# ronawho/distributed-lsb

Hardware: AMD Instinct MI355X
Metric: Melem/s (16-byte elems) at 1/2/4/8 GPUs; per-pass HBM GB/s vs roofline (higher is better)
Workload: dtype u64

## Files before the change

distributed-lsb_amd/csrc/lsb_abi.cpp:

```cpp
#include "lsb_rt.h"

using namespace lsb_rt;


extern "C" {

int64_t lsb_per_rank(int64_t n_total, int num_ranks) {
  return (num_ranks > 0 && n_total >= 0) ? div_ceil(n_total, num_ranks) : 0;
}

int64_t lsb_here(int64_t n_total, int num_ranks, int rank) {
  if (num_ranks <= 0 || n_total < 0 || rank < 0 || rank >= num_ranks) return 0;
  return here_of(n_total, num_ranks, rank);
}

const char* lsb_strerror(int code) {
  switch (code) {
    case LSB_OK: return "ok";
    case LSB_ERR_INVALID: return "invalid argument";
    case LSB_ERR_HIP: return last_error().empty() ? "HIP error" : last_error().c_str();
    case LSB_ERR_RCCL: return last_error().empty() ? "RCCL error" : last_error().c_str();
    case LSB_ERR_NOMEM: return "out of memory";
    case LSB_ERR_VERIFY: return "verification failed";
    case LSB_ERR_UNSUPPORTED: return "unsupported";
// ... 122 lines not shown
    else {
      ncclResult_t nr = ncclCommInitRank(&c->comm, num_ranks, uid, rank);
      if (nr != ncclSuccess) {
        c->comm = nullptr;
        rc = fail(LSB_ERR_RCCL, "ncclCommInitRank", ncclGetErrorString(nr));
      }
    }
  }
  if (rc != LSB_OK) {
    lsb_destroy(c);
    return rc;
  }
  *out = c;
  return LSB_OK;
}

int lsb_create_rank_ops(lsb_ctx_t** out, int64_t n_total, int num_ranks, int rank, int dev_id,
                        int radix_bits, const lsb_comm_ops_t* ops) {
  if (!out) return fail(LSB_ERR_INVALID, "lsb_create_rank_ops", "null out");
  *out = nullptr;
  if (n_total < 0 || num_ranks < 1 || num_ranks > 64 || rank < 0 || rank >= num_ranks || !ops ||
      !ops->allgather || !ops->alltoallv || !ops->allreduce_min_i64 || !ops->barrier)
    return fail(LSB_ERR_INVALID, "lsb_create_rank_ops", "n, P, rank or ops");
  if (radix_bits != 8 && radix_bits != 16 && radix_bits != 64)
    return fail(LSB_ERR_UNSUPPORTED, "lsb_create_rank_ops", "radix_bits must be 8, 16 or 64");
  lsb_ctx* c = new_ctx(n_total, num_ranks, radix_bits);
  if (!c) return LSB_ERR_NOMEM;
  c->mode = Mode::kOps;
  c->ops = *ops;
  c->first_rank = rank;
  c->ranks.resize(1);
  const int rc = init_rank(c, c->ranks[0], rank, dev_id);
  if (rc != LSB_OK) {
    lsb_destroy(c);
    return rc;
  }
  *out = c;
  return LSB_OK;
}

void lsb_destroy(lsb_ctx_t* c) {
  if (!c) return;
  (void)resolve_timing(c);
#ifdef LSB_OS_PROFILE
  (void)lsb_sync(c);
  os_profile_report();
#endif
#ifdef LSB_DEBUG
  const bool legacy = getenv("LSB_TEARDOWN_LEGACY") != nullptr;
#else
  const bool legacy = false;
#endif
  for (Rank& r : c->ranks) {
    if (legacy) break;
    (void)hipSetDevice(r.dev);
    if (r.stream) (void)hipStreamSynchronize(r.stream);
    if (r.pstream) (void)hipStreamSynchronize(r.pstream);
    if (r.xstream) (void)hipStreamSynchronize(r.xstream);
  }
  for (Rank& r : c->ranks) free_rank(r, c);
  for (auto& e : c->event_pool) (void)hipEventDestroy(e.second);
  if (c->comm) (void)ncclCommDestroy(c->comm);
  delete c;
}

int lsb_set_option(lsb_ctx_t* c, int option, int64_t value) {
  LSB_TRY(check_ctx(c));
  switch (option) {
    case LSB_OPT_TIMING:
      c->timing = value != 0;
      return LSB_OK;
    case LSB_OPT_FORCE_EXCHANGE:
      c->force_exchange = value != 0;
      return LSB_OK;
    case LSB_OPT_SKIP_CONSTANT_DIGITS:
      c->skip_constant = value != 0;
      return LSB_OK;
    case LSB_OPT_ONESWEEP:
      c->onesweep = value != 0;
      return LSB_OK;
    case LSB_OPT_REGION_FIRST:
      c->region = value != 0;
      return LSB_OK;
    case LSB_OPT_EXCHANGE_PEER:
      c->peer = value != 0;
      return LSB_OK;
    case LSB_OPT_EXCHANGE_P2P:
      c->p2p = value != 0;
      return LSB_OK;
    case LSB_OPT_EXCHANGE_SELF:
      c->self_coll = value != 0;
      return LSB_OK;
    case LSB_OPT_EXCHANGE_GATHER:
      c->gather = value != 0;
      return LSB_OK;
    case LSB_OPT_FAIL_ONESWEEP:
      if (value < 0 || value > (1 << 30)) return fail(LSB_ERR_INVALID, "lsb_set_option", "fail count");
      c->fail_onesweep = (int)value;
      return LSB_OK;
    case LSB_OPT_HYBRID:
      if (value < 0 || value > 2) return fail(LSB_ERR_INVALID, "lsb_set_option", "hybrid must be 0, 1 or 2");
      c->hybrid = (int)value;
      return LSB_OK;
    case LSB_OPT_ONESWEEP_SPLIT:
      if (value < 0 || value > 2) return fail(LSB_ERR_INVALID, "lsb_set_option", "split must be 0..2");
      c->os_split = (int)value;
      return LSB_OK;
    case LSB_OPT_EXCHANGE_CHUNKS:
      if (value != 0 && value != 2 && value != 4 && value != 8)
        return fail(LSB_ERR_INVALID, "lsb_set_option", "exchange chunks must be 0, 2, 4 or 8");
      c->xchunks = (int)value;
      return LSB_OK;
    case LSB_OPT_EXCHANGE_SLICES:
      if (value < 1 || value > 64)
        return fail(LSB_ERR_INVALID, "lsb_set_option", "exchange slices must be 1..64");
      c->slices = (int)value;
      return LSB_OK;
    default:
      return fail(LSB_ERR_INVALID, "lsb_set_option", "unknown option");
  }
}

int lsb_local_ranks(const lsb_ctx_t* c, int* first_rank, int* num_local) {
  LSB_TRY(check_ctx(c));
  if (first_rank) *first_rank = c->first_rank;
  if (num_local) *num_local = (int)c->ranks.size();
  return LSB_OK;
}

int lsb_generate_ex(lsb_ctx_t* c, int dist, double param) {
  LSB_TRY(check_ctx(c));
  lsb::KeyGen g;
  if (dist == LSB_DIST_UNIFORM) {
    g.dist = lsb::kDistUniform;
  } else if (dist == LSB_DIST_ZIPF) {
    if (!(param > 0.0) || param > 16.0) return fail(LSB_ERR_INVALID, "lsb_generate_ex", "zipf s");
    g.dist = lsb::kDistZipf;
    g.zipf_s = param;
    g.zipf_n = 1ull << 30;
  } else {
    return fail(LSB_ERR_INVALID, "lsb_generate_ex", "dist");
  }
  c->keygen = g;
  for (Rank& r : c->ranks) {
    HIP_TRY(hipSetDevice(r.dev));
    HIP_TRY(lsb::launch_pcg_fill(r.A, c->per, (uint64_t)r.rank, (uint64_t)r.rank * c->per, g,
                                 r.stream));
  }
  return lsb_sync(c);
}

int lsb_generate(lsb_ctx_t* c) { return lsb_generate_ex(c, LSB_DIST_UNIFORM, 0.0); }

int lsb_copy_in(lsb_ctx_t* c, int rank, int64_t off, int64_t cnt, const lsb_elem_t* host) {
  LSB_TRY(check_ctx(c));
  Rank* r = local_rank(c, rank);
  if (!r || off < 0 || cnt < 0 || off + cnt > c->per || (cnt > 0 && !host))
    return fail(LSB_ERR_INVALID, "lsb_copy_in", "rank or range");
  if (cnt == 0) return LSB_OK;
  HIP_TRY(hipSetDevice(r->dev));
  HIP_TRY(hipStreamSynchronize(r->stream));
  HIP_TRY(hipMemcpy(r->A + off, host, (size_t)cnt * sizeof(Elem), hipMemcpyHostToDevice));
  return LSB_OK;
}

int lsb_copy_out(lsb_ctx_t* c, int rank, int64_t off, int64_t cnt, lsb_elem_t* host) {
  LSB_TRY(check_ctx(c));
  Rank* r = local_rank(c, rank);
  if (!r || off < 0 || cnt < 0 || off + cnt > c->per || (cnt > 0 && !host))
    return fail(LSB_ERR_INVALID, "lsb_copy_out", "rank or range");
  if (cnt == 0) return LSB_OK;
  HIP_TRY(hipSetDevice(r->dev));
  HIP_TRY(hipStreamSynchronize(r->stream));
  HIP_TRY(hipMemcpy(host, r->A + off, (size_t)cnt * sizeof(Elem), hipMemcpyDeviceToHost));
  return LSB_OK;
}

namespace {

void quiesce(lsb_ctx* c) {
  for (Rank& r : c->ranks) {
    (void)hipSetDevice(r.dev);
    for (hipStream_t s : {r.stream, r.pstream, r.xstream})
      if (s) (void)hipStreamSynchronize(s);
  }
}

}

int lsb_pass(lsb_ctx_t* c, int digit) {
  LSB_TRY(check_ctx(c));
  if (digit < 0 || digit >= 64 / c->bits) return fail(LSB_ERR_INVALID, "lsb_pass", "digit");
  c->pass_cursor = c->bits == 64 ? 0 : digit * (c->bits / lsb::kDigitBits);
  const int rc = do_pass(c, digit);
  if (rc != LSB_OK) quiesce(c);
  return rc;
}

namespace {

int sort_body(lsb_ctx* c) {
  std::vector<Timer> sort_timers;
  sort_timers.reserve(c->ranks.size());
  for (Rank& r : c->ranks) sort_timers.emplace_back(c, &r, LSB_K_SORT);
  const int passes = 64 / c->bits;
  c->last_local_passes = c->last_exchanges = 0;
  c->last_varying = ~0ull;
  c->last_first = LSB_FIRST_COUNT;
  c->pass_cursor = 0;
  c->cur_pass = 0;
  if (c->bits == 64 && exchanging(c)) {
    LSB_TRY(merge_sort(c));
  } else if (onesweep_applies(c)) {
    LSB_TRY(sort_onesweep(c));
  } else if (exchange_onesweep_applies(c)) {
    LSB_TRY(sort_exchange_onesweep(c));
  } else if (!c->skip_constant) {
    for (int d = 0; d < passes; ++d) LSB_TRY(do_pass(c, d));
  } else {
    for (Rank& r : c->ranks) {
      HIP_TRY(hipSetDevice(r.dev));
      HIP_TRY(hipMemsetAsync(r.span, 0, 2 * sizeof(uint64_t), r.stream));
    }
    LSB_TRY(do_pass(c, 0, ~0ull, true));
    uint64_t kor = 0, knor = 0;
    LSB_TRY(gather_span(c, &kor, &knor));
    c->last_varying = kor & knor;
    const uint64_t digit_mask = (1ull << c->bits) - 1;
    for (int d = 1; d < passes; ++d) {
      if (((c->last_varying >> (d * c->bits)) & digit_mask) == 0) continue;
      LSB_TRY(do_pass(c, d, c->last_varying));
    }
  }
  for (Timer& t : sort_timers) t.stop();
  return LSB_OK;
}

}

int lsb_sort(lsb_ctx_t* c) {
  LSB_TRY(check_ctx(c));
  const int rc = sort_body(c);
  if (rc != LSB_OK) quiesce(c);
  return rc;
}

int lsb_get_last_sort(lsb_ctx_t* c, int* local_passes, int* exchanges, uint64_t* varying_bits) {
  LSB_TRY(check_ctx(c));
  if (local_passes) *local_passes = c->last_local_passes;
  if (exchanges) *exchanges = c->last_exchanges;
  if (varying_bits) *varying_bits = c->last_varying;
  return LSB_OK;
}

int lsb_get_first_pass(lsb_ctx_t* c, int* form) {
  LSB_TRY(check_ctx(c));
  if (!form) return fail(LSB_ERR_INVALID, "lsb_get_first_pass", "null");
  *form = c->last_first;
  return LSB_OK;
}

int lsb_sync(lsb_ctx_t* c) {
  LSB_TRY(check_ctx(c));
  for (Rank& r : c->ranks) {
    HIP_TRY(hipSetDevice(r.dev));
    HIP_TRY(hipStreamSynchronize(r.stream));
    LSB_TRY(onesweep_check(r));
  }
  return LSB_OK;
}

int lsb_barrier(lsb_ctx_t* c) {
  LSB_TRY(lsb_sync(c));
  if (c->mode == Mode::kLoopback) return LSB_OK;
  if (c->mode == Mode::kOps)
    return c->ops.barrier(c->ops.user) == 0 ? LSB_OK : ops_fail("barrier");
  Rank& r = c->ranks[0];
  HIP_TRY(hipSetDevice(r.dev));
  RCCL_TRY(ncclAllReduce(r.check, r.check, 1, ncclUint64, ncclSum, c->comm, r.stream));
  HIP_TRY(hipStreamSynchronize(r.stream));
  return LSB_OK;
}

int lsb_verify(lsb_ctx_t* c, int64_t* first_bad) {
  LSB_TRY(check_ctx(c));
  int64_t bad = INT64_MAX;
  for (Rank& r : c->ranks) {
    HIP_TRY(hipSetDevice(r.dev));
    HIP_TRY(hipMemsetAsync(r.check, 0xff, sizeof(unsigned long long), r.stream));
    HIP_TRY(lsb::launch_verify(r.A, r.here, (int64_t)r.rank * c->per, c->n, c->per, c->keygen,
                               r.check, r.stream));
    unsigned long long h = ~0ull;
    HIP_TRY(hipMemcpyAsync(&h, r.check, sizeof h, hipMemcpyDeviceToHost, r.stream));
    HIP_TRY(hipStreamSynchronize(r.stream));
    if (h != ~0ull && (int64_t)h < bad) bad = (int64_t)h;
  }
  std::vector<uint64_t> bnd;
  LSB_TRY(gather_boundaries(c, bnd));
  int prev = -1;
  for (int s = 0; s < c->P; ++s) {
    if (here_of(c->n, c->P, s) == 0) continue;
    if (prev >= 0) {
      const uint64_t lk = bnd[(size_t)prev * 4 + 2], lv = bnd[(size_t)prev * 4 + 3];
      const uint64_t fk = bnd[(size_t)s * 4 + 0], fv = bnd[(size_t)s * 4 + 1];
      if (!(lk < fk || (lk == fk && lv < fv))) {
        const int64_t idx = (int64_t)prev * c->per + here_of(c->n, c->P, prev) - 1;
        if (idx < bad) bad = idx;
      }
    }
    prev = s;
  }
  LSB_TRY(allreduce_min_i64(c, &bad));
  if (first_bad) *first_bad = bad == INT64_MAX ? -1 : bad;
  return bad == INT64_MAX ? LSB_OK : LSB_ERR_VERIFY;
}

int lsb_check_sorted(lsb_ctx_t* c, int* sorted) {
  LSB_TRY(check_ctx(c));
  int local_ok = 1;
  for (Rank& r : c->ranks) {
    HIP_TRY(hipSetDevice(r.dev));
    HIP_TRY(hipMemsetAsync(r.check, 0, sizeof(unsigned int), r.stream));
    HIP_TRY(lsb::launch_check_sorted(r.A, r.here, reinterpret_cast<unsigned int*>(r.check),
                                     r.stream));
    unsigned int h = 0;
    HIP_TRY(hipMemcpyAsync(&h, r.check, sizeof h, hipMemcpyDeviceToHost, r.stream));
    HIP_TRY(hipStreamSynchronize(r.stream));
    if (h) local_ok = 0;
  }
  std::vector<uint64_t> bnd;
  LSB_TRY(gather_boundaries(c, bnd));
  int prev = -1;
  int bounds_ok = 1;
  for (int s = 0; s < c->P; ++s) {
    if (here_of(c->n, c->P, s) == 0) continue;
    if (prev >= 0 && bnd[(size_t)s * 4 + 0] < bnd[(size_t)prev * 4 + 2]) bounds_ok = 0;
    prev = s;
  }
  int64_t ok = (local_ok && bounds_ok) ? 1 : 0;
  LSB_TRY(allreduce_min_i64(c, &ok));
  if (sorted) *sorted = (int)ok;
// ... 249 lines not shown
```

distributed-lsb_amd/csrc/lsb_context.cpp:

```cpp
#include "lsb_rt.h"

namespace lsb_rt {

thread_local std::string g_last_error;

const std::string& last_error() { return g_last_error; }

int fail(int code, const char* what, const char* detail) {
  char buf[512];
  snprintf(buf, sizeof buf, "%s: %s", what, detail ? detail : "");
  g_last_error = buf;
  if (getenv("LSB_DEBUG")) fprintf(stderr, "[lsb] %s\n", buf);
  return code;
}
hipEvent_t take_event(lsb_ctx* c) {
  int dev = 0;
  (void)hipGetDevice(&dev);
  for (size_t i = c->event_pool.size(); i-- > 0;)
    if (c->event_pool[i].first == dev) {
      hipEvent_t e = c->event_pool[i].second;
      c->event_pool.erase(c->event_pool.begin() + (long)i);
      return e;
    }
  hipEvent_t e = nullptr;
// ... 219 lines not shown
  if (k > 1) {
    std::vector<size_t> sc1(P), sd1(P), rc1(P), rd1(P);
    auto cut = [&](size_t n, size_t i) { return (size_t)((unsigned __int128)n * i / k); };
    for (size_t i = 0; i < k; ++i) {
      for (int q = 0; q < P; ++q) {
        sd1[q] = sd[q] + cut(sc[q], i);
        sc1[q] = cut(sc[q], i + 1) - cut(sc[q], i);
        rd1[q] = rd[q] + cut(rc[q], i);
        rc1[q] = cut(rc[q], i + 1) - cut(rc[q], i);
      }
      LSB_TRY(coll_alltoallv_u64(c, r, send, sc1.data(), sd1.data(), recv, rc1.data(), rd1.data(), 0, st));
    }
    return LSB_OK;
  }
  int64_t call_bytes = 0;
  for (int q = 0; q < P; ++q) call_bytes += (int64_t)sc[q] * 8;
  c->coll_calls += 1;
  c->coll_bytes += call_bytes;
  c->coll_max = std::max(c->coll_max, call_bytes);
  c->xs_calls += 1;
  for (int q = 0; q < P && q < LSB_MAX_RANKS; ++q) {
    c->xs_sent[q] += (int64_t)sc[q] * 8;
    c->xs_recv[q] += (int64_t)rc[q] * 8;
  }
  if (c->cur_pass >= 0 && c->cur_pass < LSB_MAX_PASSES) c->pass_xbytes[c->cur_pass] += call_bytes;
  if (c->mode == Mode::kRccl) {
    static const bool dsync = [] { const char* e = getenv("LSB_RCCL_SYNC"); return e && atoi(e); }();
    if (dsync) HIP_TRY(hipDeviceSynchronize());
    if (!c->p2p) {
      RCCL_TRY(ncclAllToAllv(send, sc, sd, recv, rc, rd, ncclUint64, c->comm, st));
    } else {
      RCCL_TRY(ncclGroupStart());
      for (int q = 0; q < P; ++q) {
        if (sc[q] > 0) RCCL_TRY(ncclSend(send + sd[q], sc[q], ncclUint64, q, c->comm, st));
        if (rc[q] > 0) RCCL_TRY(ncclRecv(recv + rd[q], rc[q], ncclUint64, q, c->comm, st));
      }
      RCCL_TRY(ncclGroupEnd());
    }
    if (dsync) HIP_TRY(hipDeviceSynchronize());
    return LSB_OK;
  }
  size_t send_end = 0, recv_end = 0;
  for (int q = 0; q < P; ++q) {
    if (sc[q]) send_end = std::max(send_end, sd[q] + sc[q]);
    if (rc[q]) recv_end = std::max(recv_end, rd[q] + rc[q]);
  }
  std::vector<uint64_t> hs(std::max<size_t>(send_end, 1)), hr(std::max<size_t>(recv_end, 1));
  std::vector<size_t> sb(P), sdb(P), rb(P), rdb(P);
  for (int q = 0; q < P; ++q) {
    if (sc[q])
      HIP_TRY(hipMemcpyAsync(hs.data() + sd[q], send + sd[q], sc[q] * 8, hipMemcpyDeviceToHost,
                             r.stream));
    sb[q] = sc[q] * 8;
    sdb[q] = sd[q] * 8;
    rb[q] = rc[q] * 8;
    rdb[q] = rd[q] * 8;
  }
  HIP_TRY(hipStreamSynchronize(r.stream));
  if (c->ops.alltoallv(c->ops.user, hs.data(), sb.data(), sdb.data(), hr.data(), rb.data(),
                       rdb.data()) != 0)
    return ops_fail("alltoallv");
  for (int q = 0; q < P; ++q)
    if (rc[q])
      HIP_TRY(hipMemcpyAsync(recv + rd[q], hr.data() + rd[q], rc[q] * 8, hipMemcpyHostToDevice,
                             r.stream));
  HIP_TRY(hipStreamSynchronize(r.stream));
  return LSB_OK;
}

int check_ctx(const lsb_ctx* c) {
  if (!c) return fail(LSB_ERR_INVALID, "lsb", "null context");
  return LSB_OK;
}

lsb_ctx* new_ctx(int64_t n_total, int num_ranks, int radix_bits) {
  lsb_ctx* c = new (std::nothrow) lsb_ctx();
  if (!c) return nullptr;
  c->n = n_total;
  c->P = num_ranks;
  c->per = div_ceil(n_total, num_ranks);
  c->bits = radix_bits;
  c->nb = radix_bits == 64 ? lsb::kBuckets : 1 << radix_bits;
  if (const char* e = getenv("LSB_REGION_FIRST")) c->region = atoi(e) != 0;
  if (const char* e = getenv("LSB_EXCHANGE_CHUNKS")) {
    const int v = atoi(e);
    c->xchunks = v == 2 || v == 4 || v == 8 ? v : 0;
  }
  if (const char* e = getenv("LSB_XCHUNK_RESERVE")) c->xchunk_reserve = std::max(0, atoi(e));
  return c;
}

int gather_boundaries(lsb_ctx* c, std::vector<uint64_t>& bnd) {
  const int P = c->P;
  bnd.assign((size_t)P * 4, 0);
  if (c->mode == Mode::kLoopback) {
    for (Rank& r : c->ranks) {
      if (r.here == 0) continue;
      HIP_TRY(hipSetDevice(r.dev));
      HIP_TRY(hipStreamSynchronize(r.stream));
      HIP_TRY(hipMemcpy(&bnd[(size_t)r.rank * 4], r.A, 16, hipMemcpyDeviceToHost));
      HIP_TRY(hipMemcpy(&bnd[(size_t)r.rank * 4 + 2], r.A + (r.here - 1), 16, hipMemcpyDeviceToHost));
    }
    return LSB_OK;
  }
  Rank& r = c->ranks[0];
  HIP_TRY(hipSetDevice(r.dev));
  uint64_t* d = r.gather;
  HIP_TRY(hipMemsetAsync(d, 0, sizeof(uint64_t) * 4 * P, r.stream));
  if (r.here > 0) {
    HIP_TRY(hipMemcpyAsync(d + (size_t)r.rank * 4, r.A, 16, hipMemcpyDeviceToDevice, r.stream));
    HIP_TRY(hipMemcpyAsync(d + (size_t)r.rank * 4 + 2, r.A + (r.here - 1), 16,
                           hipMemcpyDeviceToDevice, r.stream));
  }
  LSB_TRY(coll_allgather_u64(c, r, d + (size_t)r.rank * 4, d, 4));
  HIP_TRY(hipMemcpyAsync(bnd.data(), d, sizeof(uint64_t) * 4 * P, hipMemcpyDeviceToHost, r.stream));
  HIP_TRY(hipStreamSynchronize(r.stream));
  return LSB_OK;
}

int allreduce_min_i64(lsb_ctx* c, int64_t* v) {
  if (c->mode == Mode::kLoopback) return LSB_OK;
  if (c->mode == Mode::kOps)
    return c->ops.allreduce_min_i64(c->ops.user, v) == 0 ? LSB_OK : ops_fail("allreduce_min_i64");
  Rank& r = c->ranks[0];
  HIP_TRY(hipSetDevice(r.dev));
  int64_t* d = reinterpret_cast<int64_t*>(r.check);
  HIP_TRY(hipMemcpyAsync(d, v, sizeof(int64_t), hipMemcpyHostToDevice, r.stream));
  RCCL_TRY(ncclAllReduce(d, d, 1, ncclInt64, ncclMin, c->comm, r.stream));
  HIP_TRY(hipMemcpyAsync(v, d, sizeof(int64_t), hipMemcpyDeviceToHost, r.stream));
  HIP_TRY(hipStreamSynchronize(r.stream));
  return LSB_OK;
}

int gather_span(lsb_ctx* c, uint64_t* kor, uint64_t* knor) {
  *kor = *knor = 0;
  if (c->mode != Mode::kLoopback) {
    Rank& r = c->ranks[0];
    HIP_TRY(hipSetDevice(r.dev));
    LSB_TRY(coll_allgather_u64(c, r, r.span, r.span_gather, 2));
    HIP_TRY(hipMemcpyAsync(r.span_h, r.span_gather, sizeof(uint64_t) * 2 * c->P,
                           hipMemcpyDeviceToHost, r.stream));
    HIP_TRY(hipStreamSynchronize(r.stream));
    for (int q = 0; q < c->P; ++q) {
      *kor |= r.span_h[2 * q];
      *knor |= r.span_h[2 * q + 1];
    }
    return LSB_OK;
  }
  for (Rank& r : c->ranks) {
    HIP_TRY(hipSetDevice(r.dev));
    HIP_TRY(hipMemcpyAsync(r.span_h, r.span, sizeof(uint64_t) * 2, hipMemcpyDeviceToHost, r.stream));
  }
  for (Rank& r : c->ranks) {
    HIP_TRY(hipSetDevice(r.dev));
    HIP_TRY(hipStreamSynchronize(r.stream));
    *kor |= r.span_h[0];
    *knor |= r.span_h[1];
  }
  return LSB_OK;
}

}
```

distributed-lsb_amd/csrc/lsb_kernels.h:

```cpp
#pragma once

#include <hip/hip_runtime.h>
#include <stdint.h>

namespace lsb {

struct alignas(16) Elem {
  uint64_t key;
  uint64_t val;
};
static_assert(sizeof(Elem) == 16, "16-byte records");

constexpr int kDigitBits = 8;
constexpr int kBuckets = 1 << kDigitBits;
#ifndef LSB_SCATTER_BLOCK
#define LSB_SCATTER_BLOCK 256
#define LSB_SCATTER_IPT 16
#endif
constexpr int kScatterBlock = LSB_SCATTER_BLOCK;
constexpr int kScatterIpt = LSB_SCATTER_IPT;
constexpr int kTile = kScatterBlock * kScatterIpt;
#ifndef LSB_OS_BLOCK
#define LSB_OS_BLOCK 512
#endif
constexpr int kOsBlock = LSB_OS_BLOCK;
constexpr int kOsIpt = kTile / kOsBlock;
#ifndef LSB_OS_SPLIT_BLOCK
#define LSB_OS_SPLIT_BLOCK 256
#endif
constexpr int kOsSplitBlock = LSB_OS_SPLIT_BLOCK;
constexpr int kOsSplitIpt = kTile / kOsSplitBlock;
static_assert(kOsBlock % kBuckets == 0 && kOsBlock * kOsIpt == kTile, "onesweep tile shape");
constexpr int kMaxChunks = 65536;

struct Chunking {
  int64_t chunk_elems = 0;
  int num_chunks = 0;
};
Chunking make_chunking(int64_t m, int max_chunks);

constexpr int kDistUniform = 0;
constexpr int kDistZipf = 1;
struct KeyGen {
  int dist = kDistUniform;
  double zipf_s = 1.1;
  uint64_t zipf_n = 1ull << 30;
};

hipError_t launch_pcg_fill(Elem* A, int64_t count, uint64_t seed, uint64_t val0, KeyGen gen,
                           hipStream_t s);

hipError_t launch_digit16_counts(const Elem* A, int64_t m, int shift, int64_t* first,
                                 uint64_t* counts, hipStream_t s);

hipError_t launch_upsweep(const Elem* A, int64_t m, int shift, Chunking ch,
                          uint32_t* chunk_hist, uint64_t* span, hipStream_t s);

hipError_t launch_scan(const uint32_t* chunk_hist, int G, uint64_t* chunk_off,
                       uint64_t* totals, hipStream_t s);

hipError_t launch_scatter(const Elem* in, Elem* out, int64_t m, int shift, Chunking ch,
                          const uint64_t* chunk_off, const uint64_t* totals, int64_t* first16,
                          hipStream_t s);
hipError_t launch_starts_reset(int64_t* first16, hipStream_t s);
hipError_t launch_starts_to_counts(const int64_t* first16, int64_t m, uint64_t* counts,
                                   hipStream_t s);

constexpr int kOnesweepSubs = 8;
constexpr int64_t kOnesweepMaxElems = (int64_t(1) << 33) - (int64_t(1) << 16);
inline int64_t onesweep_tiles(int64_t m) { return (m + kTile - 1) / kTile; }
hipError_t launch_subhist(const Elem* A, int64_t m, int shift, int grid, uint32_t* sub_hist,
                          uint64_t* span, hipStream_t s);
hipError_t onesweep_profile(unsigned long long* out10, bool reset);
constexpr int kSegCap = 256;
struct SegPass {
  uint64_t pmask = 0;
  uint64_t rmask = 0;
  int64_t* base = nullptr;
  uint32_t* err = nullptr;
};
constexpr int kDescPieces = 4;
constexpr int kDescOverflow = 0xFF;
struct alignas(16) TileDesc {
  int32_t n, e0, e1, sel;
  int32_t start[kDescPieces];
  int64_t adj[kDescPieces];
};
constexpr int kMaxExchangeChunks = 8;
struct GatherSrc {
  const Elem* R = nullptr;
  const Elem* A = nullptr;
  int64_t self_adj[kMaxExchangeChunks] = {};
  int chunk_shift = 8;
  const int64_t* place = nullptr;
  const int64_t* gstart = nullptr;
  const int64_t* gadj = nullptr;
  const TileDesc* desc = nullptr;
  int P = 1, nb = 256, me = 0, self_in_a = 1;
  int64_t a_len = 0, r_len = 0;
};
hipError_t launch_gather_desc(const GatherSrc& g, int64_t m, TileDesc* desc, hipStream_t s);
hipError_t launch_count16_chunks(const Elem* B, int64_t m, int shift16, const uint32_t* lo_hist, int cshift,
                                 int grid, uint64_t* count16, uint32_t* chunk_hist, hipStream_t s);
constexpr int64_t kRegionMin = int64_t(1) << 27;
constexpr int kRegions = kBuckets * kOnesweepSubs;
inline int64_t region_mean(int64_t m) { return (m + kRegions - 1) / kRegions; }
#ifndef LSB_REGION_SIGMA
#define LSB_REGION_SIGMA 6
#endif
#ifndef LSB_REGION_DIV
#define LSB_REGION_DIV 64
#endif
inline int64_t region_cap(int64_t m, int64_t min_m = kRegionMin) {
  if (m < min_m || m <= 0) return 0;
  const int64_t mu = region_mean(m);
  int64_t sd = 1;
  while (sd * sd < mu) ++sd;
  const int64_t a = mu / LSB_REGION_DIV, b = LSB_REGION_SIGMA * sd;
  const int64_t slack = a > b ? a : b;
  return (mu + slack + kTile - 1) / kTile * kTile;
}
#ifndef LSB_REGION_STAGGER
#define LSB_REGION_STAGGER 0
#endif
__host__ __device__ inline int64_t region_stride(int64_t cap) { return cap + (LSB_REGION_STAGGER ? kTile : 0); }
__host__ __device__ inline int64_t region_base(int64_t r, int64_t cap) {
  return r * region_stride(cap) + (LSB_REGION_STAGGER ? ((r * 37) & 15) * 256 : 0);
}
inline int64_t region_slots(int64_t m, int64_t min_m = kRegionMin) {
  return region_stride(region_cap(m, min_m)) * kRegions;
}
struct RegionPass {
  int64_t cap = 0;
  uint32_t* counts = nullptr;
  uint32_t* ovf = nullptr;
};
hipError_t launch_sample(const Elem* A, int64_t m, int shift, uint32_t* hist, uint64_t* span,
                         hipStream_t s);
struct OnesweepExtra {
  uint64_t* totals = nullptr;
  uint64_t* count16 = nullptr;
  int halves = 1;
  const SegPass* seg = nullptr;
  const GatherSrc* gather = nullptr;
  bool probe = false;
  const RegionPass* region = nullptr;
  int region_mode = 0;
};
int onesweep_halves_for(const uint32_t* sub_hist_host, int64_t m);
hipError_t launch_onesweep(const Elem* in, Elem* out, int64_t m, int shift, int next_shift,
                           const uint32_t* sub_hist, uint32_t* next_hist, uint32_t* status,
                           uint32_t* tile_ctr, uint32_t epoch, uint32_t* err, int grid,
                           hipStream_t s, OnesweepExtra extra = OnesweepExtra());

constexpr int kSegMax = 64;
hipError_t launch_segsort(const Elem* in, Elem* out, int64_t m, uint64_t pmask, uint32_t* err,
                          int grid, hipStream_t s);
hipError_t launch_segfix(const Elem* in, Elem* out, int64_t m, int shift, const uint32_t* status,
                         const SegPass& seg, int grid, hipStream_t s);

hipError_t launch_place(const Elem* src, Elem* out, int64_t out_len, int64_t k0, int64_t count,
                        int shift, int nbuckets, const int64_t* off_row, hipStream_t s,
                        int next_shift = -1, uint32_t* next_hist = nullptr, bool store = true,
                        bool skew = false);

hipError_t launch_peer_exchange(const Elem* src, int64_t m, int shift, int nbuckets,
                                const uint64_t* hist, int P, int me, int64_t per,
                                Elem* const* dst, int64_t* base, hipStream_t s);
hipError_t launch_system_acquire(hipStream_t s);

hipError_t launch_plan(const uint64_t* hist, int P, int nb, int me, int64_t n, int64_t* work,
                       int64_t* total, int64_t* place, int64_t* counts, hipStream_t s,
                       int64_t* gstart = nullptr, int cshift = 8, int64_t* chunk_counts = nullptr);

constexpr int kSplitCands = 256;
constexpr int kSplitRounds = 8;
constexpr int kMergeMaxCuts = 512;
hipError_t launch_split_init(uint64_t* state, int Q, hipStream_t s);
hipError_t launch_split_cands(const Elem* A, int64_t m, const uint64_t* state, int Q, uint64_t* cnt,
                              hipStream_t s);
hipError_t launch_split_update(const uint64_t* gathered, int P, int Q, const int64_t* targets,
                               uint64_t* state, hipStream_t s);
hipError_t launch_split_final(const Elem* A, int64_t m, const uint64_t* state, int Q, uint64_t* out,
                              hipStream_t s);
constexpr int kMergeTile = 2048;
constexpr int kMergeMaxPairs = 32;
struct MergePair {
  const Elem* a;
  const Elem* b;
  Elem* out;
  int64_t na, nb, tile0;
};
struct MergeLevel {
  MergePair p[kMergeMaxPairs];
  int npairs;
  int64_t tiles;
};
inline int64_t merge_tiles(int64_t n) { return (n + kMergeTile - 1) / kMergeTile; }
hipError_t launch_merge_level(const MergeLevel& level, int64_t* path, int grid, hipStream_t s);

hipError_t launch_copy_records(Elem* dst, const Elem* src, int64_t cnt, hipStream_t s);
hipError_t launch_verify(const Elem* A, int64_t here, int64_t gbase, int64_t n, int64_t per,
                         KeyGen gen, unsigned long long* first_bad, hipStream_t s);

hipError_t launch_check_sorted(const Elem* A, int64_t here, unsigned int* unsorted, hipStream_t s);

}
```

distributed-lsb_amd/csrc/lsb_kernels.hip:

```cpp
#include "lsb_device.h"
#include <type_traits>

#ifdef LSB_DEBUG
#include <cassert>
#define LSB_DASSERT(c) assert(c)
#else
#define LSB_DASSERT(c) ((void)0)
#endif

namespace lsb {
namespace {

typedef unsigned __int128 u128;

constexpr u128 kPcgMult = ((u128)0x2360ED051FC65DA4ULL << 64) | (u128)0x4385DF649FCCF645ULL;
constexpr u128 kPcgInc = ((u128)0x5851F42D4C957F2DULL << 64) | (u128)0x14057B7EF767814FULL;

struct JumpTable {
  uint64_t mul_lo[64], mul_hi[64], add_lo[64], add_hi[64];
};

constexpr JumpTable make_jump_table() {
  JumpTable t{};
  u128 m = kPcgMult, a = kPcgInc;
  for (int k = 0; k < 64; ++k) {
    t.mul_lo[k] = (uint64_t)m;
    t.mul_hi[k] = (uint64_t)(m >> 64);
    t.add_lo[k] = (uint64_t)a;
    t.add_hi[k] = (uint64_t)(a >> 64);
    a = a * (m + 1);
    m = m * m;
  }
  return t;
}

__constant__ JumpTable kJump = make_jump_table();

__device__ __forceinline__ uint64_t pcg_output(u128 s) {
  const uint64_t x = (uint64_t)(s >> 64) ^ (uint64_t)s;
  const unsigned rot = (unsigned)(s >> 122);
  return (x >> rot) | (x << ((64u - rot) & 63u));
}

__device__ __forceinline__ u128 pcg_seed(uint64_t seed) {
  return ((u128)seed + kPcgInc) * kPcgMult + kPcgInc;
}

__device__ __forceinline__ u128 pcg_jump(u128 s, uint64_t delta) {
  while (delta) {
    const int k = __builtin_ctzll(delta);
    const u128 m = ((u128)kJump.mul_hi[k] << 64) | kJump.mul_lo[k];
    const u128 a = ((u128)kJump.add_hi[k] << 64) | kJump.add_lo[k];
    s = s * m + a;
    delta &= delta - 1;
  }
  return s;
}

__device__ __forceinline__ uint32_t lane_id() { return __lane_id(); }

__device__ __forceinline__ uint32_t mbcnt(uint64_t mask) {
  return __builtin_amdgcn_mbcnt_hi((uint32_t)(mask >> 32),
                                   __builtin_amdgcn_mbcnt_lo((uint32_t)mask, 0u));
}

__device__ __forceinline__ uint64_t match_digit8(uint32_t d, uint64_t active) {
  uint32_t lo = (uint32_t)active, hi = (uint32_t)(active >> 32);
#pragma unroll
  for (int bit = 0; bit < 8; ++bit) {
    const uint32_t t = (uint32_t)__builtin_amdgcn_sbfe((int)d, bit, 1);
    const uint64_t bal = __builtin_amdgcn_uicmp(t, 0u, 33);
    lo = __builtin_amdgcn_bitop3_b32(lo, (uint32_t)bal, t, 0x90);
    hi = __builtin_amdgcn_bitop3_b32(hi, (uint32_t)(bal >> 32), t, 0x90);
  }
  return ((uint64_t)hi << 32) | lo;
}

__device__ __forceinline__ Elem load_elem(const Elem* p) {
  const ulonglong2 v = *reinterpret_cast<const ulonglong2*>(p);
  return Elem{v.x, v.y};
}

__device__ __forceinline__ Elem load_elem_nt(const Elem* p) {
  typedef unsigned long long u64x2 __attribute__((ext_vector_type(2)));
  const u64x2 v = __builtin_nontemporal_load(reinterpret_cast<const u64x2*>(p));
  return Elem{v.x, v.y};
}

__device__ __forceinline__ void store_elem(Elem* p, const Elem& e) {
  *reinterpret_cast<ulonglong2*>(p) = make_ulonglong2(e.key, e.val);
}

template <typename T>
__device__ __forceinline__ T wave_inclusive_scan(T v) {
  const uint32_t lane = lane_id();
#pragma unroll
  for (int off = 1; off < 64; off <<= 1) {
    const T u = __shfl_up(v, off, 64);
    if (lane >= (uint32_t)off) v += u;
  }
  return v;
}

template <>
__device__ __forceinline__ uint32_t wave_inclusive_scan<uint32_t>(uint32_t v) {
  const uint32_t lane = lane_id(), rl = lane & 15u;
  uint32_t t;
  t = (uint32_t)__builtin_amdgcn_mov_dpp((int)v, 0x111, 0xf, 0xf, false);
  if (rl >= 1) v += t;
  t = (uint32_t)__builtin_amdgcn_mov_dpp((int)v, 0x112, 0xf, 0xf, false);
  if (rl >= 2) v += t;
  t = (uint32_t)__builtin_amdgcn_mov_dpp((int)v, 0x114, 0xf, 0xf, false);
  if (rl >= 4) v += t;
  t = (uint32_t)__builtin_amdgcn_mov_dpp((int)v, 0x118, 0xf, 0xf, false);
  if (rl >= 8) v += t;
  t = (uint32_t)__builtin_amdgcn_mov_dpp((int)v, 0x142, 0xf, 0xf, false);
  if ((lane & 31u) >= 16) v += t;
  t = (uint32_t)__builtin_amdgcn_mov_dpp((int)v, 0x143, 0xf, 0xf, false);
  if (lane >= 32) v += t;
  return v;
}

__device__ __forceinline__ uint32_t pair_swap(uint32_t v) {
  return (uint32_t)__builtin_amdgcn_mov_dpp((int)v, 0xB1, 0xf, 0xf, false);
}

template <int BLOCK, typename T>
__device__ __forceinline__ T block_exclusive_scan(T v, T* tmp, T* total) {
  constexpr int W = BLOCK / 64;
  const int w = threadIdx.x >> 6;
  const T inc = wave_inclusive_scan(v);
  if (lane_id() == 63) tmp[w] = inc;
  __syncthreads();
  T pre = 0, tot = 0;
#pragma unroll
  for (int i = 0; i < W; ++i) {
    const T x = tmp[i];
    pre += (i < w) ? x : T(0);
    tot += x;
  }
  __syncthreads();
  *total = tot;
  return pre + inc - v;
}

constexpr int kFillPerThread = 16;

__device__ __forceinline__ uint64_t mix64(uint64_t z) {
  z = (z ^ (z >> 30)) * 0xBF58476D1CE4E5B9ull;
  z = (z ^ (z >> 27)) * 0x94D049BB133111EBull;
  return z ^ (z >> 31);
}

__device__ __forceinline__ uint64_t make_key(uint64_t draw, const KeyGen& g) {
  if (g.dist == kDistUniform) return draw;
  const double u = (double)(draw >> 11) * 0x1.0p-53;
  const double n1 = (double)g.zipf_n + 1.0;
  double x;
  if (g.zipf_s == 1.0) {
    x = exp(u * log(n1));
  } else {
    const double e = 1.0 - g.zipf_s;
    x = pow(1.0 - u * (1.0 - pow(n1, e)), 1.0 / e);
  }
  uint64_t k = (uint64_t)x;
  if (k < 1) k = 1;
  if (k > g.zipf_n) k = g.zipf_n;
  return mix64(k);
}

__global__ __launch_bounds__(256) void k_pcg_fill(Elem* __restrict__ A, int64_t count,
                                                  uint64_t seed, uint64_t val0, KeyGen g) {
  const int64_t first = ((int64_t)blockIdx.x * 256 + threadIdx.x) * kFillPerThread;
// ... 419 lines not shown
  __syncthreads();
  if (t <= C) {
    int64_t a = 0;
    for (int l = 0; l < (t << cshift) && l < kBuckets; ++l) a += tot[l];
    cstart[t] = a;
  }
  __syncthreads();
  const uint64_t* __restrict__ keys = reinterpret_cast<const uint64_t*>(B);
  const int64_t TT = (m + T - 1) / T;
  const int64_t t0 = (int64_t)blockIdx.x * tiles_per_wg;
  const int64_t t1 = t0 + tiles_per_wg < TT ? t0 + tiles_per_wg : TT;
  auto target = [&](int64_t p, uint32_t l) -> uint32_t {
    const uint32_t k = l >> cshift;
    const int64_t len = cstart[k + 1] - cstart[k];
    const int64_t TTk = (len + T - 1) / T;
    return k * kSub + (uint32_t)sub_of_tile((p - cstart[k]) / T, TTk);
  };
  uint32_t cur_l = 0xFFFFFFFFu, cur_s = 0xFFFFFFFFu;
  uint32_t acc_l = 0, acc_s = 0;
  auto flush_l = [&]() {
    if (cur_l != 0xFFFFFFFFu && acc_l) atomicAdd(&count16[((uint32_t)t << 8) | cur_l], (unsigned long long)acc_l);
    acc_l = 0;
  };
  auto flush_s = [&]() {
    if (cur_s != 0xFFFFFFFFu && acc_s) atomicAdd(&chunk_hist[cur_s * kBuckets + t], acc_s);
    acc_s = 0;
  };
  for (int64_t tile = t0; tile < t1; ++tile) {
    const int64_t tb = tile * T;
    const int64_t end = tb + T < m ? tb + T : m;
    const uint32_t lf = (uint32_t)(keys[2 * tb] >> shift16) & 0xFFu;
    const uint32_t ll = (uint32_t)(keys[2 * (end - 1)] >> shift16) & 0xFFu;
    const uint32_t sf = target(tb, lf), sl = target(end - 1, ll);
    const bool uniform = lf == ll && sf == sl;
    uint64_t k[IPT];
#pragma unroll
    for (int i = 0; i < IPT; ++i) {
      const int64_t idx = tb + (int64_t)i * BLOCK + t;
      k[i] = idx < end ? __builtin_nontemporal_load(keys + 2 * idx) : 0ull;
    }
    if (uniform) {
#pragma unroll
      for (int i = 0; i < IPT; ++i) {
        const int64_t idx = tb + (int64_t)i * BLOCK + t;
        if (idx < end) atomicAdd(&th[w][(uint32_t)(k[i] >> (shift16 + 8)) & 0xFFu], 1u);
      }
      __syncthreads();
      uint32_t v = 0;
#pragma unroll
      for (int ww = 0; ww < W; ++ww) {
        v += th[ww][t];
        th[ww][t] = 0;
      }
      if (lf != cur_l) {
        flush_l();
        cur_l = lf;
      }
      if (sf != cur_s) {
        flush_s();
        cur_s = sf;
      }
      acc_l += v;
      acc_s += v;
      __syncthreads();
    } else {
#pragma unroll
      for (int i = 0; i < IPT; ++i) {
        const int64_t idx = tb + (int64_t)i * BLOCK + t;
        if (idx >= end) continue;
        const uint32_t l = (uint32_t)(k[i] >> shift16) & 0xFFu, h = (uint32_t)(k[i] >> (shift16 + 8)) & 0xFFu;
        atomicAdd(&count16[(h << 8) | l], 1ull);
        atomicAdd(&chunk_hist[target(idx, l) * kBuckets + h], 1u);
      }
    }
  }
  flush_l();
  flush_s();
}

constexpr int kSampleBlock = 256;
constexpr int kSampleTiles = 256;
__global__ __launch_bounds__(kSampleBlock) void k_sample(const Elem* __restrict__ A, int64_t m, int shift,
                                                         uint32_t* __restrict__ hist,
                                                         unsigned long long* __restrict__ span) {
  constexpr int IPT = kTile / kSampleBlock;
  __shared__ uint32_t h[kBuckets];
  h[threadIdx.x] = 0;
  __syncthreads();
  const int64_t TT = (m + kTile - 1) / kTile;
  const int64_t tb = (int64_t)blockIdx.x * TT / gridDim.x * kTile;
  const uint64_t* __restrict__ keys = reinterpret_cast<const uint64_t*>(A);
  uint64_t kor = 0, knor = 0;
#pragma unroll
  for (int i = 0; i < IPT; ++i) {
    const int64_t idx = tb + (int64_t)i * kSampleBlock + threadIdx.x;
    if (idx < m) {
      const uint64_t k = __builtin_nontemporal_load(keys + 2 * idx);
      kor |= k;
      knor |= ~k;
      atomicAdd(&h[(uint32_t)(k >> shift) & (kBuckets - 1)], 1u);
    }
  }
#pragma unroll
  for (int off = 32; off > 0; off >>= 1) {
    kor |= __shfl_xor(kor, off, 64);
    knor |= __shfl_xor(knor, off, 64);
  }
  if (lane_id() == 0) {
    atomicOr(&span[0], (unsigned long long)kor);
    atomicOr(&span[1], (unsigned long long)knor);
  }
  __syncthreads();
  if (h[threadIdx.x]) atomicAdd(&hist[threadIdx.x], h[threadIdx.x]);
}

#ifdef LSB_OS_PROFILE
__device__ unsigned long long g_os_prof[10];
#define OS_MARK(k)                                                       \
  do {                                                                   \
    if (t == 0) {                                                        \
      const uint64_t now = __builtin_amdgcn_s_memtime();                 \
      prof[k] += now - prof_last;                                        \
      prof_last = now;                                                   \
    }                                                                    \
  } while (0)
#else
#define OS_MARK(k) ((void)0)
#endif

#ifndef LSB_SEG_WIN
#define LSB_SEG_WIN 2
#endif
constexpr int kSegWin = LSB_SEG_WIN;
#ifndef LSB_SEG_LDSNB
#define LSB_SEG_LDSNB 0
#endif
#ifndef LSB_SEG_BATCH
#define LSB_SEG_BATCH 4
#endif
#ifndef LSB_GATHER_PF
#define LSB_GATHER_PF 64
#endif

template <int BLOCK, int IPT, bool NEXT, bool C16, int HALVES, bool SEG, bool GATHER, int RG>
__device__ __forceinline__ void onesweep_body(
    const Elem* __restrict__ in, Elem* __restrict__ out, int64_t m, int shift, int next_shift,
    const uint32_t* __restrict__ sub_hist, uint32_t* __restrict__ next_hist,
    uint32_t* __restrict__ status, uint32_t* __restrict__ tile_ctr, uint32_t epoch,
    uint32_t* __restrict__ err, uint64_t* __restrict__ totals,
    unsigned long long* __restrict__ count16, SegPass seg, GatherSrc gs, RegionPass rg) {
  constexpr int W = BLOCK / 64;
  constexpr int T = BLOCK * IPT;
  static_assert(!SEG || (!NEXT && !C16 && HALVES == 1), "the segment pass: last pass, whole stage");
  static_assert(RG == 0 || (!C16 && HALVES == 1 && !SEG && !GATHER), "regional passes: plain whole stage");
  static_assert(RG != 1 || NEXT, "the regional first pass counts the next digit");
  static_assert(BLOCK % kBuckets == 0, "bucket threads");
  using WC = typename std::conditional<(W > 4), uint16_t, uint32_t>::type;

  constexpr int HT = T / HALVES;
  __shared__ Elem stage[HT];
  __shared__ WC wcnt[W][kBuckets];
  __shared__ int64_t delta[kBuckets];
  __shared__ uint32_t cut[NEXT ? kBuckets : 1];
  __shared__ uint32_t nh[NEXT ? kSub * kBuckets : 1];
  __shared__ uint64_t scan64[W];
  __shared__ uint32_t scan32[W];
  __shared__ int32_t s_tile, s_sub;
  __shared__ uint32_t tile_lo[2];
  __shared__ TileDesc s_desc;

  const int t = threadIdx.x;
  const bool bkt = BLOCK == kBuckets || t < kBuckets;
  const int w = t >> 6;
  const uint32_t lane = lane_id();
  const int64_t TT = RG == 2 ? rg.cap / T * kRegions : (m + T - 1) / T;
  const int64_t TTn = RG == 1 ? rg.cap / T * kRegions : (m + T - 1) / T;
  const int64_t mcap = RG == 1 ? region_stride(rg.cap) * kRegions : m;
  uint32_t racc = 0;
  constexpr uint32_t kValMask = kStatusValMask, kPreBit = 1u << 30;
  const uint32_t tag_agg = (epoch & 1u) << 31, tag_pre = tag_agg | kPreBit;
  const int shift16 = shift - 8;
  uint32_t acc_lo = 0xFFFFFFFFu;
  uint64_t acc = 0;
  auto c16_flush = [&]() {
    if (acc) atomicAdd(count16 + (((uint32_t)t << 8) | acc_lo), (unsigned long long)acc);
    acc = 0;
  };

  uint32_t col[HALVES == 1 ? kSub : 1];
  uint64_t tot = 0;
#pragma unroll
  for (int x = 0; x < kSub; ++x) {
    const uint32_t v = bkt && RG != 1 ? sub_hist[x * kBuckets + t] : 0u;
    if (HALVES == 1) col[x] = v;
    tot += v;
  }
  uint64_t all;
  const uint64_t bstart = block_exclusive_scan<BLOCK>(tot, scan64, &all);
  if (totals != nullptr && blockIdx.x == 0 && bkt) totals[t] = tot;
  if (SEG && blockIdx.x == 0 && bkt) {
    uint64_t pre = bstart;
#pragma unroll
    for (int x = 0; x < kSub; ++x) {
      seg.base[x * kBuckets + t] = (int64_t)pre;
      pre += col[x];
    }
  }
  const bool skewed = NEXT && __syncthreads_or(tot > (uint64_t)(m >> 5)) != 0;
  if (NEXT)
    for (int i = t; i < kSub * kBuckets; i += BLOCK) nh[i] = 0;

#ifdef LSB_OS_PROFILE
  uint64_t prof[10] = {};
  uint64_t prof_last = __builtin_amdgcn_s_memtime();
#endif
  int sub = (int)(blockIdx.x % kSub);
  int tries = 0;
  int cur_sub = -1;
  uint64_t base = 0;
  auto grab = [&](int& tile_out, int& sub_out) {
    int tile = -1;
    while (tries < kSub) {
      const int64_t f0 = sub_first_tile(sub, TT), f1 = sub_first_tile(sub + 1, TT);
      if (f1 > f0) {
        const uint32_t jj = atomicAdd(&tile_ctr[sub], 1u);
        if ((int64_t)jj < f1 - f0) {
          tile = (int)(f0 + jj);
          break;
        }
      }
      sub = sub + 1 == kSub ? 0 : sub + 1;
      ++tries;
    }
    tile_out = tile;
    sub_out = sub;
  };
  int nxt_tile = -1, nxt_sub = 0;
  if (t == 0) grab(nxt_tile, nxt_sub);
  uint4 dreg = make_uint4(0u, 0u, 0u, 0u);
  auto fetch_desc = [&]() {
    if (GATHER && w == 0) {
      const int nt = __builtin_amdgcn_readfirstlane(nxt_tile);
      if (nt >= 0 && lane < 4) dreg = reinterpret_cast<const uint4*>(gs.desc + nt)[lane];
    }
  };
  fetch_desc();

  for (;;) {
    if (t == 0) {
      s_tile = nxt_tile;
      s_sub = nxt_sub;
    }
    if (GATHER && w == 0 && lane < 4) {
      uint32_t l;
      asm volatile("v_mbcnt_lo_u32_b32 %0, -1, 0" : "=v"(l));
      *reinterpret_cast<uint4*>(reinterpret_cast<char*>(&s_desc) + l * 16u) = dreg;
    }
#pragma unroll
    for (int j = 0; j < kBuckets / 64; ++j) wcnt[w][lane + 64 * j] = 0;
    __syncthreads();
    OS_MARK(0);
    const int tile = s_tile;
    if (tile < 0) break;
    const int x = s_sub;
    if (x != cur_sub) {
      if (RG == 1) {
        if (bkt && cur_sub >= 0 && racc) atomicAdd(&rg.counts[t * kSub + cur_sub], racc);
        racc = 0;
        base = (uint64_t)region_base((bkt ? t : 0) * kSub + x, rg.cap);
      } else {
        uint64_t pre = 0;
#pragma unroll
        for (int xx = 0; xx < kSub; ++xx)
          pre += xx < x ? (HALVES == 1 ? col[xx] : (bkt ? sub_hist[xx * kBuckets + t] : 0u)) : 0u;
        base = bstart + pre;
      }
      cur_sub = x;
    }
    int64_t tb = (int64_t)tile * T;
    int nvalid = (int)((m - tb) < T ? (m - tb) : T);
    uint32_t rg_reg = 0, rg_k = 0;
    if (RG == 2) {
      const uint32_t tu = (uint32_t)__builtin_amdgcn_readfirstlane(tile);
      const uint32_t ct = (uint32_t)(rg.cap / T);
      rg_reg = tu / ct;
      rg_k = tu - rg_reg * ct;
      tb = region_base(rg_reg, rg.cap) + (int64_t)rg_k * T;
    }

    Elem e[IPT];
    const int wbase = w * 64 * IPT + (int)lane;
    if (GATHER) {
      const int dn = __builtin_amdgcn_readfirstlane(s_desc.n);
      if (dn != kDescOverflow) {
        const uint32_t sel = (uint32_t)__builtin_amdgcn_readfirstlane(s_desc.sel);
        const Elem* pb[kDescPieces];
        int st[kDescPieces];
#pragma unroll
        for (int k = 0; k < kDescPieces; ++k) {
          st[k] = __builtin_amdgcn_readfirstlane(s_desc.start[k]);
          const uint64_t a = s_desc.adj[k];
          const int64_t adj = (int64_t)(((uint64_t)(uint32_t)__builtin_amdgcn_readfirstlane((int)(a >> 32)) << 32) |
                                        (uint32_t)__builtin_amdgcn_readfirstlane((int)(uint32_t)a));
          pb[k] = ((sel >> k) & 1u ? gs.A : gs.R) + (tb + adj);
        }
        const int wu = __builtin_amdgcn_readfirstlane(w);
#pragma unroll
        for (int i = 0; i < IPT; ++i) {
          const int li = wbase + i * 64;
          const int g0 = wu * 64 * IPT + i * 64;
          int ka = 0, kb = 0;
#pragma unroll
          for (int k = 1; k < kDescPieces; ++k) {
            ka += g0 >= st[k] ? 1 : 0;
            kb += g0 + 63 >= st[k] ? 1 : 0;
          }
          const Elem* src = pb[0];
          if (ka == kb) {
#pragma unroll
            for (int k = 1; k < kDescPieces; ++k) src = ka >= k ? pb[k] : src;
          } else {
#pragma unroll
            for (int k = 1; k < kDescPieces; ++k) src = li >= st[k] ? pb[k] : src;
          }
          LSB_DASSERT(li >= nvalid || gather_in(gs, src + li));
          e[i] = li < nvalid ? load_elem_nt(src + li) : Elem{0ull, 0ull};
        }
      } else {
        const int e0 = s_desc.e0, e1 = s_desc.e1;
#pragma unroll
        for (int i = 0; i < IPT; ++i) {
          const int li = wbase + i * 64;
          LSB_DASSERT(li >= nvalid || gather_in(gs, gather_search(gs, e0, e1, tb + li)));
          e[i] = li < nvalid ? load_elem_nt(gather_search(gs, e0, e1, tb + li)) : Elem{0ull, 0ull};
          __builtin_amdgcn_sched_barrier(0);
        }
      }
#if LSB_GATHER_PF
      if (w == 1 && lane == 0) {
        const int pf = tile + LSB_GATHER_PF;
        if (pf < sub_first_tile(x + 1, TT))
          (void)__hip_atomic_load(const_cast<int32_t*>(&gs.desc[pf].n), __ATOMIC_RELAXED, __HIP_MEMORY_SCOPE_AGENT);
      }
#endif
    } else {
#pragma unroll
      for (int i = 0; i < IPT; ++i) {
        const int li = wbase + i * 64;
        e[i] = RG == 2 || li < nvalid ? load_elem_nt(in + tb + li) : Elem{0ull, 0ull};
      }
      if (RG == 2) {
        __builtin_amdgcn_sched_barrier(0);
        const int64_t v = (int64_t)rg.counts[rg_reg] - (int64_t)rg_k * T;
        nvalid = (int)(v < 0 ? 0 : (v < T ? v : T));
      }
    }
#ifdef LSB_OS_PROFILE
    asm volatile("s_waitcnt vmcnt(0)" ::: "memory");
    OS_MARK(6);
#endif
    const int64_t first = sub_first_tile(x, TT);
    const int64_t last = sub_first_tile(x + 1, TT);
    const bool head = tile == first;
    const bool even = (lane & 1u) == 0;
    const __amdgpu_buffer_rsrc_t rs = __builtin_amdgcn_make_buffer_rsrc(
        status + first * kBuckets, 0, (int)((last - first) * kBuckets * 4), 0x00020000);
    constexpr uint32_t kRowBytes = kBuckets * 4;
    const uint32_t my_off = (uint32_t)(tile - first) * kRowBytes + (uint32_t)t * 4u;
    uint32_t prow = (uint32_t)(tile - first) - 1u;
    v2u g[kLookW];
    auto load_window = [&]() {
#pragma unroll
      for (int r = 0; r < kLookW; ++r)
        g[r] = __builtin_amdgcn_raw_buffer_load_b64(rs, (prow - (uint32_t)r) * kRowBytes + (uint32_t)t * 4u, 0, 16);
    };
    uint32_t cnt = 0, lstart;
    uint32_t rk[IPT];
#pragma unroll
    for (int i = 0; i < IPT; ++i) {
      const bool valid = wbase + i * 64 < nvalid;
      const uint32_t d = (uint32_t)(e[i].key >> shift) & (kBuckets - 1);
      const uint64_t mt = match_digit8(d, __ballot(valid));
      const uint32_t below = mbcnt(mt);
      const uint32_t pre = wcnt[w][d];
      rk[i] = pre + below;
      if (valid && below == 0) wcnt[w][d] = (WC)(pre + (uint32_t)__popcll(mt));
      if (C16) {
        const int li = wbase + i * 64;
        if (li == 0) tile_lo[0] = (uint32_t)(e[i].key >> shift16) & 0xFFu;
        if (li == nvalid - 1) tile_lo[1] = (uint32_t)(e[i].key >> shift16) & 0xFFu;
      }
    }
    __syncthreads();
    OS_MARK(1);
    if (bkt) {
#pragma unroll
      for (int ww = 0; ww < W; ++ww) {
        const uint32_t v = wcnt[ww][t];
        wcnt[ww][t] = (WC)cnt;
        cnt += v;
      }
      if (RG == 1) racc += cnt;
    }
    bool mixed16 = false;
    if (C16) {
      const uint32_t l0 = tile_lo[0];
      mixed16 = l0 != tile_lo[1];
      if (!mixed16 && cnt > 0) {
        if (l0 != acc_lo) {
          c16_flush();
          acc_lo = l0;
        }
        acc += cnt;
      }
    }
    const uint32_t cnt_b = pair_swap(cnt);
    if (even && bkt) {
      const uint32_t tg = head ? tag_pre : tag_agg;
      __builtin_amdgcn_raw_buffer_store_b64(v2u{cnt | tg, cnt_b | tg}, rs, my_off, 0, kStPol);
      if (!head) load_window();
    }
    {
      uint32_t tile_total;
      lstart = block_exclusive_scan<BLOCK>(cnt, scan32, &tile_total);
      if (bkt) {
#pragma unroll
        for (int ww = 0; ww < W; ++ww) wcnt[ww][t] = (WC)(wcnt[ww][t] + lstart);
      }
    }
    __syncthreads();
    OS_MARK(2);
    auto stage_half = [&](int h) {
#pragma unroll
      for (int i = 0; i < IPT; ++i) {
        if (wbase + i * 64 < nvalid) {
          const uint32_t d = (uint32_t)(e[i].key >> shift) & (kBuckets - 1);
          if (HALVES == 1) {
            stage[wcnt[w][d] + rk[i]] = e[i];
          } else {
            if (h == 0) rk[i] += wcnt[w][d];
            if ((int)(rk[i] / HT) == h) stage[rk[i] - h * HT] = e[i];
          }
        }
      }
    };
    stage_half(0);

    OS_MARK(3);
    uint32_t ea = 0, eb = 0;
    if (even && bkt && !head) {
      uint32_t spins = 0;
      for (;;) {
        uint32_t used = 0;
        bool done = false;
#pragma unroll
        for (int r = 0; r < kLookW; ++r) {
          if (done || used != (uint32_t)r) continue;
          if (((g[r].x ^ g[r].y) >> 30) == 0 && (g[r].x & ~kValMask & ~kPreBit) == tag_agg) {
            ea += g[r].x & kValMask;
            eb += g[r].y & kValMask;
            ++used;
            done = (g[r].x & kPreBit) != 0;
          }
        }
#ifdef LSB_OS_PROFILE
        if (t == 0) prof[7] += used;
#endif
        if (done) break;
        if (used == 0) {
          __builtin_amdgcn_s_sleep(kPollSleep);
          if ((++spins & 1023u) == 0 &&
              (spins > kSpinLimit ||
               __hip_atomic_load((gu32*)err, __ATOMIC_RELAXED, __HIP_MEMORY_SCOPE_AGENT) != 0)) {
            atomicOr(err, 1u);
            break;
          }
        }
        prow -= used;
        load_window();
      }
      __builtin_amdgcn_raw_buffer_store_b64(v2u{(ea + cnt) | tag_pre, (eb + cnt_b) | tag_pre}, rs,
                                            my_off, 0, kStPol);
    }
    const uint32_t eb_left = pair_swap(eb);
    const uint64_t excl = even ? ea : eb_left;
    int64_t R = (int64_t)(base + excl);
    if (RG == 1 && bkt && excl + cnt > (uint64_t)rg.cap) {
      atomicOr(rg.ovf, 1u);
      R = R < mcap - (int64_t)cnt ? R : mcap - (int64_t)cnt;
    }
    if (bkt) delta[t] = R - (int64_t)lstart;
    if (NEXT && bkt) {
      uint32_t c = 0xFFFFu;
      if (RG == 1) {
        c = 0xFFFFu | ((uint32_t)(t >> 5) << 16) | ((uint32_t)(t >> 5) << 24);
      } else if (cnt > 0) {
        const int x0 = sub_of_tile(R / T, TTn);
        const int64_t bnd = x0 + 1 < kSub ? sub_first_tile(x0 + 1, TTn) * T : mcap;
        if (R + cnt > bnd) {
          const int x1 = sub_of_tile(bnd / T, TTn);
          c = (uint32_t)(lstart + (bnd - R)) | ((uint32_t)x0 << 16) | ((uint32_t)x1 << 24);
        } else {
          c = 0xFFFFu | ((uint32_t)x0 << 16) | ((uint32_t)x0 << 24);
        }
      }
      cut[t] = c;
    }
    __syncthreads();
    OS_MARK(5);
#ifdef LSB_OS_PROFILE
    if (t == 0) ++prof[8];
#endif
    if (t == 0) {
      grab(nxt_tile, nxt_sub);
    }

    auto emit = [&](auto skew_tag, const Elem& v, int j, int64_t g, uint32_t c) {
      constexpr bool kSkew = decltype(skew_tag)::value;
      LSB_DASSERT(g >= 0 && g < mcap);
      const uint64_t gs = (uint64_t)g < (uint64_t)(mcap - 1) ? (uint64_t)g : (uint64_t)(mcap - 1);
      store_elem(out + gs, v);
      if (NEXT) {
        const uint32_t xs = (uint32_t)j >= (c & 0xFFFFu) ? (c >> 24) : ((c >> 16) & 0xFFu);
        const uint32_t dn = (uint32_t)(v.key >> next_shift) & (kBuckets - 1);
        const uint32_t slot = xs * kBuckets + dn;
        if (kSkew) {
          const uint64_t act = __ballot(1);
          const uint32_t prev =
              (uint32_t)__builtin_amdgcn_update_dpp((int)~slot, (int)slot, 0x138, 0xf, 0xf, false);
          const bool head = prev != slot;
          const uint64_t heads = __ballot(head);
          if (head) {
            const uint64_t above = heads & ~((2ull << lane) - 1ull);
            const uint32_t end = above ? (uint32_t)__builtin_ctzll(above) : (uint32_t)__popcll(act);
            atomicAdd(&nh[slot], end - lane);
          }
        } else {
          atomicAdd(&nh[slot], 1u);
        }
      }
    };
    auto seg_pos = [&](const Elem& v, int j, int jend) -> int {
      int pos = j;
#if LSB_SEG_LDSNB
      const uint64_t pv = j > 0 ? stage[j - 1].key : ~v.key;
      const uint64_t nx = j + 1 < nvalid ? stage[j + 1].key : ~v.key;
#else
      const uint32_t kl = (uint32_t)v.key, kh = (uint32_t)(v.key >> 32);
      uint64_t pv = ((uint64_t)(uint32_t)__builtin_amdgcn_update_dpp(0, (int)kh, 0x138, 0xf, 0xf, false) << 32) |
                    (uint32_t)__builtin_amdgcn_update_dpp(0, (int)kl, 0x138, 0xf, 0xf, false);
      uint64_t nx = ((uint64_t)(uint32_t)__builtin_amdgcn_update_dpp(0, (int)kh, 0x130, 0xf, 0xf, false) << 32) |
                    (uint32_t)__builtin_amdgcn_update_dpp(0, (int)kl, 0x130, 0xf, 0xf, false);
      if (lane == 0 && j > 0) pv = stage[j - 1].key;
      if ((lane == 63 || j + 1 == jend) && j + 1 < nvalid) nx = stage[j + 1].key;
#endif
      const uint64_t pk = v.key & seg.pmask;
      const bool sp = j > 0 && (pv & seg.pmask) == pk;
      const bool sn = j + 1 < nvalid && (nx & seg.pmask) == pk;
      if (sp || sn) {
        uint32_t less = 0, eqb = 0;
        const int klo = j - kSegMax > 0 ? j - kSegMax : 0;
        const int khi = j + 1 + kSegMax < nvalid ? j + 1 + kSegMax : nvalid;
        uint64_t wb[kSegWin > 0 ? kSegWin : 1], wf[kSegWin > 0 ? kSegWin : 1];
#pragma unroll
        for (int q = 0; q < kSegWin; ++q) {
          wb[q] = q == 0 && j - 1 >= klo ? pv : j - 1 - q >= klo ? stage[j - 1 - q].key : ~v.key;
          wf[q] = q == 0 && j + 1 < khi ? nx : j + 1 + q < khi ? stage[j + 1 + q].key : ~v.key;
        }
        int k = j - 1;
        bool on = true;
#pragma unroll
        for (int q = 0; q < kSegWin; ++q) {
          on = on && (wb[q] & seg.pmask) == pk;
          if (on) {
            less += wb[q] < v.key ? 1u : 0u;
            eqb += wb[q] == v.key ? 1u : 0u;
            --k;
          }
        }
        while (on && k >= klo) {
          const uint64_t kk = stage[k].key;
          if ((kk & seg.pmask) != pk) break;
          less += kk < v.key ? 1u : 0u;
          eqb += kk == v.key ? 1u : 0u;
          --k;
        }
        const int sfirst = k + 1;
        bool too_long = k < klo && klo > 0;
        k = j + 1;
        on = true;
#pragma unroll
        for (int q = 0; q < kSegWin; ++q) {
          on = on && (wf[q] & seg.pmask) == pk;
          if (on) {
            less += wf[q] < v.key ? 1u : 0u;
            ++k;
          }
        }
        while (on && k < khi) {
          const uint64_t kk = stage[k].key;
          if ((kk & seg.pmask) != pk) break;
          less += kk < v.key ? 1u : 0u;
          ++k;
        }
        too_long |= k == khi && khi < nvalid;
        if (too_long) atomicOr(seg.err, 2u);
        pos = sfirst + (int)(less + eqb);
      }
      return pos;
    };
    auto write_out = [&](auto skew_tag, int h) {
      const int jend = HALVES == 1 || (h + 1) * HT >= nvalid ? nvalid : (h + 1) * HT;
      if ((!SEG || LSB_SEG_BATCH) && HALVES == 1 && !C16 && !GATHER && jend == HT) {
        constexpr int G = SEG && LSB_SEG_BATCH > 0 && LSB_SEG_BATCH < HT / BLOCK ? LSB_SEG_BATCH : HT / BLOCK;
#pragma unroll
        for (int k0 = 0; k0 < HT / BLOCK; k0 += G) {
          Elem v[G];
          int64_t dl[G];
          uint32_t ct[G];
#pragma unroll
          for (int k = 0; k < G; ++k) v[k] = stage[(k0 + k) * BLOCK + t];
#pragma unroll
          for (int k = 0; k < G; ++k) {
            const uint32_t d = (uint32_t)(v[k].key >> shift) & (kBuckets - 1);
            dl[k] = delta[d];
            ct[k] = NEXT ? cut[d] : 0u;
          }
#pragma unroll
          for (int k = 0; k < G; ++k) {
            const int j = (k0 + k) * BLOCK + t;
            emit(skew_tag, v[k], j, dl[k] + (SEG ? seg_pos(v[k], j, jend) : j), ct[k]);
          }
        }
        return;
      }
      for (int j = h * HT + t; j < jend; j += BLOCK) {
        const Elem v = stage[j - h * HT];
        int pos = j;
        if (SEG) pos = seg_pos(v, j, jend);
        const uint32_t d = (uint32_t)(v.key >> shift) & (kBuckets - 1);
        emit(skew_tag, v, j, delta[d] + pos, NEXT ? cut[d] : 0u);
        if (C16 && mixed16) {
          const uint32_t s16 = (d << 8) | ((uint32_t)(v.key >> shift16) & 0xFFu);
          const uint64_t act = __ballot(1);
          const uint32_t prev = (uint32_t)__builtin_amdgcn_update_dpp((int)~s16, (int)s16, 0x138, 0xf, 0xf, false);
          const bool head = prev != s16;
          const uint64_t heads = __ballot(head);
          if (head) {
            const uint64_t above = heads & ~((2ull << lane) - 1ull);
            const uint32_t end = above ? (uint32_t)__builtin_ctzll(above) : (uint32_t)__popcll(act);
            atomicAdd(count16 + s16, (unsigned long long)(end - lane));
          }
        }
      }
    };
    for (int h = 0; h < HALVES; ++h) {
      if (h > 0) {
        stage_half(h);
        __syncthreads();
      }
      if (skewed) write_out(std::true_type{}, h);
      else write_out(std::false_type{}, h);
      if (h == HALVES - 1) fetch_desc();
      __syncthreads();
    }
    OS_MARK(4);
  }
  if (C16) c16_flush();
#ifdef LSB_OS_PROFILE
  if (t == 0)
    for (int k = 0; k < 10; ++k) atomicAdd(&g_os_prof[k], (unsigned long long)prof[k]);
#endif
  if (NEXT) {
    for (int i = t; i < kSub * kBuckets; i += BLOCK)
      if (nh[i]) atomicAdd(&next_hist[i], nh[i]);
  }
  if (RG == 1 && bkt && cur_sub >= 0 && racc) atomicAdd(&rg.counts[t * kSub + cur_sub], racc);
}

template <int BLOCK, int IPT, bool NEXT, bool C16, int HALVES, bool SEG = false, bool GATHER = false, int RG = 0>
__global__ __launch_bounds__(BLOCK, (HALVES == 1 ? 2 : 3) * BLOCK / 256) void k_onesweep(
    const Elem* __restrict__ in, Elem* __restrict__ out, int64_t m, int shift, int next_shift,
    const uint32_t* __restrict__ sub_hist, uint32_t* __restrict__ next_hist,
    uint32_t* __restrict__ status, uint32_t* __restrict__ tile_ctr, uint32_t epoch,
    uint32_t* __restrict__ err, uint64_t* __restrict__ totals,
    unsigned long long* __restrict__ count16, SegPass seg, GatherSrc gs, RegionPass rg) {
  onesweep_body<BLOCK, IPT, NEXT, C16, HALVES, SEG, GATHER, RG>(in, out, m, shift, next_shift, sub_hist,
                                                                next_hist, status, tile_ctr, epoch, err, totals,
                                                                count16, seg, gs, rg);
}

__global__ __launch_bounds__(kOsBlock, 2 * kOsBlock / 256) void k_onesweep_probe(
    const Elem* __restrict__ in, Elem* __restrict__ out, int64_t m, int shift, int next_shift,
    const uint32_t* __restrict__ sub_hist, uint32_t* __restrict__ next_hist,
    uint32_t* __restrict__ status, uint32_t* __restrict__ tile_ctr, uint32_t epoch,
    uint32_t* __restrict__ err, uint64_t* __restrict__ totals,
    unsigned long long* __restrict__ count16, SegPass seg, GatherSrc gs) {
  onesweep_body<kOsBlock, kOsIpt, true, false, 1, false, false, 0>(in, out, m, shift, next_shift, sub_hist,
                                                                   next_hist, status, tile_ctr, epoch, err,
                                                                   totals, count16, seg, gs, RegionPass());
}

constexpr int kPlaceBlock = 256;
constexpr int kPlaceIpt = 8;
constexpr int kPlaceLdsBuckets = 4096;
constexpr int kPlaceNextGrid = 1024;

template <bool kLds, bool kNext, bool kStore = true>
__global__ __launch_bounds__(kPlaceBlock) void k_place(const Elem* __restrict__ src,
                                                       Elem* __restrict__ out, int64_t k0,
                                                       int64_t count, int shift, uint32_t mask,
                                                       const int64_t* __restrict__ off_row,
                                                       int64_t out_len, int next_shift,
                                                       uint32_t* __restrict__ next_hist, uint32_t skew) {
  __shared__ int64_t lds_off[kLds ? kPlaceLdsBuckets : 1];
  __shared__ uint32_t nh[kNext ? kSub * kBuckets : 1];
  const int nb = (int)mask + 1;
  const int64_t* off = off_row;
  const int64_t TT = (out_len + kTile - 1) / kTile;
  if (kNext)
    for (int i = threadIdx.x; i < kSub * kBuckets; i += kPlaceBlock) nh[i] = 0;
  if (kLds) {
    for (int i = threadIdx.x; i < nb; i += kPlaceBlock) lds_off[i] = off_row[i];
    off = lds_off;
  }
  if (kLds || kNext) __syncthreads();
  const int64_t step = (int64_t)gridDim.x * kPlaceBlock * kPlaceIpt;
  for (int64_t base = (int64_t)blockIdx.x * kPlaceBlock * kPlaceIpt + threadIdx.x; base < count;
       base += step) {
    Elem x[kPlaceIpt];
#pragma unroll
    for (int i = 0; i < kPlaceIpt; ++i) {
      const int64_t k = base + (int64_t)i * kPlaceBlock;
      x[i] = k < count ? load_elem(src + k) : Elem{0ull, 0ull};
    }
#pragma unroll
    for (int i = 0; i < kPlaceIpt; ++i) {
      const int64_t k = base + (int64_t)i * kPlaceBlock;
      if (k < count) {
        const uint32_t d = (uint32_t)(x[i].key >> shift) & mask;
        const int64_t g = off[d] + k0 + k;
        LSB_DASSERT(g >= 0 && g < out_len);
        if (kStore) store_elem(out + g, x[i]);
        if (kNext) {
          const uint32_t xs = (uint32_t)sub_of_tile(g / kTile, TT);
          const uint32_t slot = xs * kBuckets + ((uint32_t)(x[i].key >> next_shift) & (kBuckets - 1));
          if (skew) {
            const uint64_t act = __ballot(1);
            const uint32_t lane = lane_id();
            const uint32_t prev =
                (uint32_t)__builtin_amdgcn_update_dpp((int)~slot, (int)slot, 0x138, 0xf, 0xf, false);
            const bool head = prev != slot;
            const uint64_t heads = __ballot(head);
            if (head) {
              const uint64_t above = heads & ~((2ull << lane) - 1ull);
              const uint32_t end = above ? (uint32_t)__builtin_ctzll(above) : (uint32_t)__popcll(act);
              atomicAdd(&nh[slot], end - lane);
            }
          } else {
            atomicAdd(&nh[slot], 1u);
          }
        }
      }
    }
  }
  if (kNext) {
    __syncthreads();
    for (int i = threadIdx.x; i < kSub * kBuckets; i += kPlaceBlock)
      if (nh[i]) atomicAdd(&next_hist[i], nh[i]);
  }
}

struct PeerDests {
  Elem* dst[64];
};

constexpr int kPeerBaseBlock = 1024;
constexpr int kWaitVmcnt0 = 0x0F70;

__global__ __launch_bounds__(kPeerBaseBlock) void k_peer_base(const uint64_t* __restrict__ hist,
                                                              int P, int nb, int me,
                                                              int64_t* __restrict__ base) {
  __shared__ uint64_t tmp_t[kPeerBaseBlock / 64], tmp_m[kPeerBaseBlock / 64];
// ... 238 lines not shown
      return (h << 8) | l;
    });
    __syncthreads();
    const int C = kBuckets >> cshift;
    if ((int)threadIdx.x < C) {
      const int k = threadIdx.x;
      const int64_t a = row[k << cshift];
      const int64_t e = k + 1 < C ? row[(k + 1) << cshift] : tot;
      chunk_recv[(int64_t)s * C + k] = e - a;
    }
  }
  if (threadIdx.x == 0) recv_counts[s] = tot;
}

__global__ __launch_bounds__(256) void k_plan_finish(int P, int nb, int64_t lo,
                                                     const int64_t* __restrict__ work,
                                                     const int64_t* __restrict__ recv_counts,
                                                     int64_t* __restrict__ place) {
  const int64_t i = (int64_t)blockIdx.x * 256 + threadIdx.x;
  if (i < P) {
    int64_t acc = 0;
    for (int s = 0; s <= (int)i; ++s) acc += recv_counts[s];
    place[(int64_t)P * nb + i] = acc;
  }
  if (i >= (int64_t)P * nb) return;
  const int s = (int)(i / nb);
  int64_t displ = 0;
  for (int q = 0; q < s; ++q) displ += recv_counts[q];
  place[i] = (place[i] - lo) - (displ + work[i]);
}

__global__ __launch_bounds__(256) void k_gather_adj(GatherSrc g, int64_t* __restrict__ gadj) {
  const int64_t e = (int64_t)blockIdx.x * 256 + threadIdx.x;
  if (e < (int64_t)g.P * g.nb) gadj[e] = gather_adj(g, (int)e);
}

__global__ __launch_bounds__(256) void k_gather_desc(GatherSrc g, int64_t m, int64_t TT,
                                                     TileDesc* __restrict__ desc) {
  const int64_t t = (int64_t)blockIdx.x * 256 + threadIdx.x;
  if (t >= TT) return;
  const int cells = g.P * g.nb;
  const int64_t tb = t * kTile;
  const int64_t te = (tb + kTile < m ? tb + kTile : m) - 1;
  const int e0 = gather_piece(g, 0, cells - 1, tb);
  const int e1 = gather_piece(g, e0, cells - 1, te);
  TileDesc d;
  d.e0 = e0;
  d.e1 = e1;
  d.sel = 0;
  int n = 0;
#pragma unroll
  for (int k = 0; k < kDescPieces; ++k) {
    d.start[k] = 0x7FFFFFFF;
    d.adj[k] = 0;
  }
  if (e1 - e0 < 64) {
    for (int e = e0; e <= e1; ++e) {
      const int64_t st = g.gstart[e], en = e + 1 < cells ? g.gstart[e + 1] : m;
      if (en <= st) continue;
      if (n == kDescPieces) {
        n = kDescOverflow;
        break;
      }
      const int64_t v = gather_adj(g, e);
      d.start[n] = st > tb ? (int32_t)(st - tb) : 0;
      d.adj[n] = v >> 1;
      d.sel |= (int)(v & 1) << n;
      ++n;
    }
  } else {
    n = kDescOverflow;
  }
  d.n = n;
  desc[t] = d;
}

__global__ __launch_bounds__(256) void k_copy_records(Elem* __restrict__ dst, const Elem* __restrict__ src,
                                                      int64_t cnt) {
  const int64_t stride = (int64_t)gridDim.x * 256;
  for (int64_t i = (int64_t)blockIdx.x * 256 + threadIdx.x; i < cnt; i += stride)
    store_elem(dst + i, load_elem_nt(src + i));
}

__global__ __launch_bounds__(256) void k_verify(const Elem* __restrict__ A, int64_t here,
                                                int64_t gbase, int64_t n, int64_t per, KeyGen gen,
                                                unsigned long long* first_bad) {
  const int64_t stride = (int64_t)gridDim.x * 256;
  for (int64_t i = (int64_t)blockIdx.x * 256 + threadIdx.x; i < here; i += stride) {
    const Elem x = load_elem(A + i);
    bool bad = x.val >= (uint64_t)n;
    if (!bad) {
      const uint64_t r = x.val / (uint64_t)per;
      const uint64_t idx = x.val - r * (uint64_t)per;
      bad = make_key(pcg_output(pcg_jump(pcg_seed(r), idx + 1)), gen) != x.key;
    }
    if (i + 1 < here) {
      const Elem y = load_elem(A + i + 1);
      bad |= !(x.key < y.key || (x.key == y.key && x.val < y.val));
    }
    if (bad) atomicMin(first_bad, (unsigned long long)(gbase + i));
  }
}

__global__ __launch_bounds__(256) void k_check_sorted(const Elem* __restrict__ A, int64_t here,
                                                      unsigned int* unsorted) {
  const int64_t stride = (int64_t)gridDim.x * 256;
  for (int64_t i = (int64_t)blockIdx.x * 256 + threadIdx.x; i + 1 < here; i += stride) {
    if (A[i + 1].key < A[i].key) *unsorted = 1u;
  }
}

int grid_for(int64_t work, int block, int cap) {
  const int64_t g = (work + block - 1) / block;
  return (int)(g < 1 ? 1 : (g > cap ? cap : g));
}

}

Chunking make_chunking(int64_t m, int max_chunks) {
  Chunking ch;
  if (m <= 0) return ch;
  if (max_chunks > kMaxChunks) max_chunks = kMaxChunks;
  if (max_chunks < 1) max_chunks = 1;
  const int64_t tiles = (m + kTile - 1) / kTile;
  const int64_t tiles_per_chunk = (tiles + max_chunks - 1) / max_chunks;
  ch.chunk_elems = tiles_per_chunk * kTile;
  ch.num_chunks = (int)((m + ch.chunk_elems - 1) / ch.chunk_elems);
  return ch;
}

hipError_t launch_pcg_fill(Elem* A, int64_t count, uint64_t seed, uint64_t val0, KeyGen gen,
                           hipStream_t s) {
  if (count <= 0) return hipSuccess;
  const int64_t threads = (count + kFillPerThread - 1) / kFillPerThread;
  const int64_t blocks = (threads + 255) / 256;
  hipLaunchKernelGGL(k_pcg_fill, dim3((unsigned)blocks), dim3(256), 0, s, A, count, seed, val0,
                     gen);
  return hipGetLastError();
}

hipError_t launch_digit16_counts(const Elem* A, int64_t m, int shift, int64_t* first,
                                 uint64_t* counts, hipStream_t s) {
  hipError_t e = hipMemsetAsync(first, 0xff, sizeof(int64_t) * 65536, s);
  if (e != hipSuccess) return e;
  if (m > 0)
    hipLaunchKernelGGL(k_digit_starts, dim3(grid_for(m, 256, 8192)), dim3(256), 0, s, A, m, shift,
                       first);
  hipLaunchKernelGGL(k_starts_to_counts, dim3(1), dim3(kStartsBlock), 0, s, first, m, counts);
  return hipGetLastError();
}

hipError_t launch_starts_reset(int64_t* first, hipStream_t s) {
  return hipMemsetAsync(first, 0x7f, sizeof(int64_t) * 65536, s);
}

hipError_t launch_starts_to_counts(const int64_t* first, int64_t m, uint64_t* counts,
                                   hipStream_t s) {
  hipLaunchKernelGGL(k_starts_to_counts, dim3(1), dim3(kStartsBlock), 0, s, first, m, counts);
  return hipGetLastError();
}

hipError_t launch_upsweep(const Elem* A, int64_t m, int shift, Chunking ch, uint32_t* chunk_hist,
                          uint64_t* span, hipStream_t s) {
  if (m <= 0) return hipSuccess;
  if (span)
    hipLaunchKernelGGL((k_upsweep<256, 16, true>), dim3(ch.num_chunks), dim3(256), 0, s, A, m,
                       shift, ch.chunk_elems, ch.num_chunks, chunk_hist,
                       reinterpret_cast<unsigned long long*>(span));
  else
    hipLaunchKernelGGL((k_upsweep<256, 16, false>), dim3(ch.num_chunks), dim3(256), 0, s, A, m,
                       shift, ch.chunk_elems, ch.num_chunks, chunk_hist, nullptr);
  return hipGetLastError();
}

hipError_t launch_scan(const uint32_t* chunk_hist, int G, uint64_t* chunk_off, uint64_t* totals,
                       hipStream_t s) {
  if (G <= 0) return hipSuccess;
  if (G > kMaxChunks) return hipErrorInvalidValue;
  hipLaunchKernelGGL(k_scan, dim3(kBuckets), dim3(kScanBlock), 0, s, chunk_hist, G, chunk_off,
                     totals);
  return hipGetLastError();
}

hipError_t launch_scatter(const Elem* in, Elem* out, int64_t m, int shift, Chunking ch,
                          const uint64_t* chunk_off, const uint64_t* totals, int64_t* first16,
                          hipStream_t s) {
  if (m <= 0) return hipSuccess;
  if (first16) {
    if (shift < 8) return hipErrorInvalidValue;
    hipLaunchKernelGGL((k_scatter<kScatterBlock, kScatterIpt, true>), dim3(ch.num_chunks),
                       dim3(kScatterBlock), 0, s, in, out, m, shift, ch.chunk_elems, ch.num_chunks,
                       chunk_off, totals, reinterpret_cast<long long*>(first16));
  } else {
    hipLaunchKernelGGL((k_scatter<kScatterBlock, kScatterIpt, false>), dim3(ch.num_chunks),
                       dim3(kScatterBlock), 0, s, in, out, m, shift, ch.chunk_elems, ch.num_chunks,
                       chunk_off, totals, nullptr);
  }
  return hipGetLastError();
}

hipError_t onesweep_profile(unsigned long long* out10, bool reset) {
#ifdef LSB_OS_PROFILE
  hipError_t e = hipMemcpyFromSymbol(out10, HIP_SYMBOL(g_os_prof), 10 * sizeof(unsigned long long));
  if (e != hipSuccess || !reset) return e;
  const unsigned long long z[10] = {};
  return hipMemcpyToSymbol(HIP_SYMBOL(g_os_prof), z, sizeof z);
#else
  for (int k = 0; k < 10; ++k) out10[k] = 0;
  (void)reset;
  return hipErrorNotSupported;
#endif
}

hipError_t launch_subhist(const Elem* A, int64_t m, int shift, int grid, uint32_t* sub_hist,
                          uint64_t* span, hipStream_t s) {
  hipError_t e = hipMemsetAsync(sub_hist, 0, sizeof(uint32_t) * kSub * kBuckets, s);
  if (e != hipSuccess || m <= 0) return e;
  const int64_t TT = (m + kTile - 1) / kTile;
  if (grid < 1) grid = 1;
  const int64_t tpw = (TT + grid - 1) / grid;
  const dim3 g((unsigned)((TT + tpw - 1) / tpw));
  if (span)
    hipLaunchKernelGGL((k_subhist<kScatterBlock, kScatterIpt, true>), g, dim3(kScatterBlock), 0, s,
                       A, m, shift, tpw, sub_hist, reinterpret_cast<unsigned long long*>(span));
  else
    hipLaunchKernelGGL((k_subhist<kScatterBlock, kScatterIpt, false>), g, dim3(kScatterBlock), 0, s,
                       A, m, shift, tpw, sub_hist, nullptr);
  return hipGetLastError();
}

hipError_t launch_count16_chunks(const Elem* B, int64_t m, int shift16, const uint32_t* lo_hist, int cshift,
                                 int grid, uint64_t* count16, uint32_t* chunk_hist, hipStream_t s) {
  if (shift16 < 0 || shift16 > 48 || cshift < 5 || cshift > 7 || !lo_hist) return hipErrorInvalidValue;
  hipError_t e = hipMemsetAsync(count16, 0, sizeof(uint64_t) * 65536, s);
  if (e == hipSuccess)
    e = hipMemsetAsync(chunk_hist, 0, sizeof(uint32_t) * (kBuckets >> cshift) * kSub * kBuckets, s);
  if (e != hipSuccess || m <= 0) return e;
  const int64_t TT = (m + kTile - 1) / kTile;
  if (grid < 1) grid = 1;
  const int64_t tpw = (TT + grid - 1) / grid;
  hipLaunchKernelGGL((k_count16c<kScatterBlock, kScatterIpt>), dim3((unsigned)((TT + tpw - 1) / tpw)),
                     dim3(kScatterBlock), 0, s, B, m, shift16, lo_hist, cshift, tpw,
                     reinterpret_cast<unsigned long long*>(count16), chunk_hist);
  return hipGetLastError();
}

hipError_t launch_sample(const Elem* A, int64_t m, int shift, uint32_t* hist, uint64_t* span, hipStream_t s) {
  if (shift < 0 || shift > 56) return hipErrorInvalidValue;
  hipError_t e = hipMemsetAsync(hist, 0, sizeof(uint32_t) * kBuckets, s);
  if (e == hipSuccess) e = hipMemsetAsync(span, 0, 2 * sizeof(uint64_t), s);
  if (e != hipSuccess || m <= 0) return e;
  const int64_t TT = (m + kTile - 1) / kTile;
  const unsigned g = (unsigned)(TT < kSampleTiles ? TT : kSampleTiles);
  hipLaunchKernelGGL(k_sample, dim3(g), dim3(kSampleBlock), 0, s, A, m, shift, hist,
                     reinterpret_cast<unsigned long long*>(span));
  return hipGetLastError();
}

int onesweep_halves_for(const uint32_t* h, int64_t m) {
  for (int b = 0; b < kBuckets; ++b) {
    uint64_t tot = 0;
    for (int x = 0; x < kSub; ++x) tot += h[x * kBuckets + b];
    if (tot > (uint64_t)(m >> 5) && tot < (uint64_t)m) return 2;
  }
  return 1;
}

hipError_t launch_onesweep(const Elem* in, Elem* out, int64_t m, int shift, int next_shift,
                           const uint32_t* sub_hist, uint32_t* next_hist, uint32_t* status,
                           uint32_t* tile_ctr, uint32_t epoch, uint32_t* err, int grid,
                           hipStream_t s, OnesweepExtra extra) {
  if (m <= 0) return hipSuccess;
  if (m > kOnesweepMaxElems || epoch == 0 || epoch >= (1u << 31) || shift < 0 || shift > 56 ||
      next_shift > 56 || (extra.halves != 1 && extra.halves != 2))
    return hipErrorInvalidValue;
  hipError_t e = hipMemsetAsync(tile_ctr, 0, sizeof(uint32_t) * kSub, s);
  if (e != hipSuccess) return e;
  const int rm = extra.region_mode;
  const RegionPass rp = extra.region ? *extra.region : RegionPass();
  if (rm < 0 || rm > 2 || (rm != 0 && (!extra.region || rp.cap <= 0 || rp.cap % kTile != 0 ||
                                       rp.cap * kRegions < m || !rp.counts)))
    return hipErrorInvalidValue;
  const int64_t TT = rm == 2 ? rp.cap / kTile * kRegions : (m + kTile - 1) / kTile;
  auto* c16 = reinterpret_cast<unsigned long long*>(extra.count16);
  const bool gat = extra.gather != nullptr;
  if (extra.halves == 2 && gat) return hipErrorInvalidValue;
  const bool split = extra.halves == 2 && c16 == nullptr;
  int64_t g = split ? (int64_t)grid * 3 / 2 : grid;
  if (g < kSub) g = kSub;
  if (g > (TT + kSub - 1) / kSub * kSub) g = (TT + kSub - 1) / kSub * kSub;
  const dim3 gd((unsigned)g), bd(split ? kOsSplitBlock : kOsBlock);
  uint32_t* st = status;
  const GatherSrc gsrc = extra.gather ? *extra.gather : GatherSrc();
  auto go = [&](auto kplain, auto kgather, int nshift, uint32_t* nhist, unsigned long long* cnt16,
                SegPass sp) {
    hipLaunchKernelGGL(gat ? kgather : kplain, gd, bd, 0, s, in, out, m, shift, nshift, sub_hist, nhist,
                       st, tile_ctr, epoch, err, extra.totals, cnt16, sp, gsrc, RegionPass());
  };
  if (rm != 0) {
    if (c16 || extra.halves != 1 || extra.seg || gat || extra.probe || extra.totals) return hipErrorInvalidValue;
    if (rm == 1 && (next_shift < 0 || !rp.ovf)) return hipErrorInvalidValue;
    if (next_shift >= 0) {
      e = hipMemsetAsync(next_hist, 0, sizeof(uint32_t) * kSub * kBuckets, s);
      if (e != hipSuccess) return e;
    }
    if (rm == 1) {
      e = hipMemsetAsync(rp.counts, 0, sizeof(uint32_t) * kRegions, s);
      if (e == hipSuccess) e = hipMemsetAsync(rp.ovf, 0, sizeof(uint32_t), s);
      if (e != hipSuccess) return e;
      hipLaunchKernelGGL((k_onesweep<kOsBlock, kOsIpt, true, false, 1, false, false, 1>), gd, bd, 0, s, in, out,
                         m, shift, next_shift, sub_hist, next_hist, st, tile_ctr, epoch, err, nullptr, nullptr,
                         SegPass(), gsrc, rp);
    } else if (next_shift >= 0) {
      hipLaunchKernelGGL((k_onesweep<kOsBlock, kOsIpt, true, false, 1, false, false, 2>), gd, bd, 0, s, in, out,
                         m, shift, next_shift, sub_hist, next_hist, st, tile_ctr, epoch, err, nullptr, nullptr,
                         SegPass(), gsrc, rp);
    } else {
      hipLaunchKernelGGL((k_onesweep<kOsBlock, kOsIpt, false, false, 1, false, false, 2>), gd, bd, 0, s, in, out,
                         m, shift, 0, sub_hist, nullptr, st, tile_ctr, epoch, err, nullptr, nullptr, SegPass(),
                         gsrc, rp);
    }
  } else if (extra.probe) {
    if (next_shift < 0 || !next_hist || c16 || extra.halves != 1 || extra.seg || gat) return hipErrorInvalidValue;
    e = hipMemsetAsync(next_hist, 0, sizeof(uint32_t) * kSub * kBuckets, s);
    if (e != hipSuccess) return e;
    hipLaunchKernelGGL(k_onesweep_probe, gd, bd, 0, s, in, out, m, shift, next_shift, sub_hist, next_hist, st,
                       tile_ctr, epoch, err, nullptr, nullptr, SegPass(), gsrc);
  } else if (extra.seg) {
    if (next_shift >= 0 || c16 || extra.halves != 1 || !extra.seg->base ||
        !extra.seg->err || gat)
      return hipErrorInvalidValue;
    hipLaunchKernelGGL((k_onesweep<kOsBlock, kOsIpt, false, false, 1, true>), gd, bd, 0, s, in, out, m,
                       shift, 0, sub_hist, nullptr, st, tile_ctr, epoch, err, extra.totals, nullptr,
                       *extra.seg, gsrc, RegionPass());
  } else if (c16) {
    if (shift < 8 || next_shift >= 0) return hipErrorInvalidValue;
    e = hipMemsetAsync(c16, 0, sizeof(uint64_t) * 65536, s);
    if (e != hipSuccess) return e;
    go(k_onesweep<kOsBlock, kOsIpt, false, true, 1>, k_onesweep<kOsBlock, kOsIpt, false, true, 1, false, true>,
       0, nullptr, c16, SegPass());
  } else if (next_shift >= 0) {
    e = hipMemsetAsync(next_hist, 0, sizeof(uint32_t) * kSub * kBuckets, s);
    if (e != hipSuccess) return e;
    if (split)
      go(k_onesweep<kOsSplitBlock, kOsSplitIpt, true, false, 2>,
         k_onesweep<kOsSplitBlock, kOsSplitIpt, true, false, 2>, next_shift, next_hist, nullptr, SegPass());
    else
      go(k_onesweep<kOsBlock, kOsIpt, true, false, 1>, k_onesweep<kOsBlock, kOsIpt, true, false, 1, false, true>,
         next_shift, next_hist, nullptr, SegPass());
  } else if (split) {
    go(k_onesweep<kOsSplitBlock, kOsSplitIpt, false, false, 2>,
       k_onesweep<kOsSplitBlock, kOsSplitIpt, false, false, 2>, 0, nullptr, nullptr, SegPass());
  } else {
    go(k_onesweep<kOsBlock, kOsIpt, false, false, 1>, k_onesweep<kOsBlock, kOsIpt, false, false, 1, false, true>,
       0, nullptr, nullptr, SegPass());
  }
  return hipGetLastError();
}

hipError_t launch_place(const Elem* src, Elem* out, int64_t out_len, int64_t k0, int64_t count,
                        int shift, int nbuckets, const int64_t* off_row, hipStream_t s,
                        int next_shift, uint32_t* next_hist, bool store, bool skew) {
  if (count <= 0) return hipSuccess;
  if (nbuckets != 256 && nbuckets != 65536) return hipErrorInvalidValue;
  if (k0 < 0 || k0 + count > out_len) return hipErrorInvalidValue;
  const uint32_t mask = (uint32_t)nbuckets - 1;
  const bool lds = nbuckets <= kPlaceLdsBuckets;
  if (next_shift >= 0) {
    if (next_shift > 56 || !next_hist || out_len > kOnesweepMaxElems) return hipErrorInvalidValue;
    const dim3 grid(grid_for(count, kPlaceBlock * kPlaceIpt, kPlaceNextGrid));
    if (!store) {
      if (lds)
        hipLaunchKernelGGL((k_place<true, true, false>), grid, dim3(kPlaceBlock), 0, s, src, out, k0,
                           count, shift, mask, off_row, out_len, next_shift, next_hist, skew ? 1u : 0u);
      else
        hipLaunchKernelGGL((k_place<false, true, false>), grid, dim3(kPlaceBlock), 0, s, src, out, k0,
                           count, shift, mask, off_row, out_len, next_shift, next_hist, skew ? 1u : 0u);
      return hipGetLastError();
    }
    if (lds)
      hipLaunchKernelGGL((k_place<true, true>), grid, dim3(kPlaceBlock), 0, s, src, out, k0, count,
                         shift, mask, off_row, out_len, next_shift, next_hist, skew ? 1u : 0u);
    else
      hipLaunchKernelGGL((k_place<false, true>), grid, dim3(kPlaceBlock), 0, s, src, out, k0, count,
                         shift, mask, off_row, out_len, next_shift, next_hist, skew ? 1u : 0u);
    return hipGetLastError();
  }
  if (!store) return hipErrorInvalidValue;
  const dim3 grid(grid_for(count, kPlaceBlock * kPlaceIpt, 4096));
  if (lds)
    hipLaunchKernelGGL((k_place<true, false>), grid, dim3(kPlaceBlock), 0, s, src, out, k0, count,
                       shift, mask, off_row, out_len, 0, nullptr, 0u);
  else
    hipLaunchKernelGGL((k_place<false, false>), grid, dim3(kPlaceBlock), 0, s, src, out, k0, count,
                       shift, mask, off_row, out_len, 0, nullptr, 0u);
  return hipGetLastError();
}

hipError_t launch_peer_exchange(const Elem* src, int64_t m, int shift, int nbuckets,
                                const uint64_t* hist, int P, int me, int64_t per,
                                Elem* const* dst, int64_t* base, hipStream_t s) {
  if (P < 1 || P > 64 || me < 0 || me >= P || (nbuckets != 256 && nbuckets != 65536))
    return hipErrorInvalidValue;
  hipLaunchKernelGGL(k_peer_base, dim3(1), dim3(kPeerBaseBlock), 0, s, hist, P, nbuckets, me, base);
  if (m <= 0) return hipGetLastError();
  PeerDests d{};
  for (int q = 0; q < P; ++q) d.dst[q] = dst[q];
  const dim3 grid(grid_for(m, kPlaceBlock * kPlaceIpt, 4096));
  const uint32_t mask = (uint32_t)nbuckets - 1;
  if (nbuckets <= kPlaceLdsBuckets)
    hipLaunchKernelGGL(k_peer_scatter<true>, grid, dim3(kPlaceBlock), 0, s, src, m, shift, mask,
                       base, per, P, d);
  else
    hipLaunchKernelGGL(k_peer_scatter<false>, grid, dim3(kPlaceBlock), 0, s, src, m, shift, mask,
                       base, per, P, d);
  return hipGetLastError();
}

hipError_t launch_system_acquire(hipStream_t s) {
  hipLaunchKernelGGL(k_system_acquire, dim3(64), dim3(64), 0, s);
  return hipGetLastError();
}

hipError_t launch_plan(const uint64_t* hist, int P, int nb, int me, int64_t n, int64_t* work,
                       int64_t* total, int64_t* place, int64_t* counts, hipStream_t s,
                       int64_t* gstart, int cshift, int64_t* chunk_counts) {
  if (P < 1 || me < 0 || me >= P || nb < 1 || n < 0) return hipErrorInvalidValue;
  if (cshift < 8 && (nb != 65536 || cshift < 5 || !chunk_counts || P > 64)) return hipErrorInvalidValue;
  const int C = cshift < 8 ? kBuckets >> cshift : 1;
  if (cshift < 8) {
    hipError_t e = hipMemsetAsync(chunk_counts, 0, sizeof(int64_t) * 2 * P * C, s);
    if (e != hipSuccess) return e;
  }
  const int64_t per = (n + P - 1) / P;
  const int64_t lo = (int64_t)me * per;
  int64_t here = n - lo;
  if (here > per) here = per;
  if (here < 0) here = 0;
  const int64_t hi = lo + here;
  hipError_t e = hipMemsetAsync(counts, 0, sizeof(int64_t) * 2 * P, s);
  if (e != hipSuccess) return e;
  const int64_t cells = (int64_t)P * nb;
  hipLaunchKernelGGL(k_plan_cols, dim3((nb + 255) / 256), dim3(256), 0, s, hist, P, nb, work, total);
  hipLaunchKernelGGL(k_plan_base, dim3(1), dim3(kPlanScanBlock), 0, s, total, nb);
  hipLaunchKernelGGL(k_plan_pieces, dim3((unsigned)((cells + 255) / 256)), dim3(256), 0, s, hist, P,
                     nb, me, per, lo, hi, total, work, place,
                     reinterpret_cast<unsigned long long*>(counts), gstart, cshift < 8 ? cshift : 8,
                     cshift < 8 ? reinterpret_cast<unsigned long long*>(chunk_counts) : nullptr);
  hipLaunchKernelGGL(k_plan_rows, dim3(P), dim3(kPlanScanBlock), 0, s, work, nb, counts + P, cshift < 8 ? cshift : 8,
                     cshift < 8 ? chunk_counts + (size_t)P * C : nullptr);
  hipLaunchKernelGGL(k_plan_finish, dim3((unsigned)((cells + 255) / 256)), dim3(256), 0, s, P, nb,
                     lo, work, counts + P, place);
  return hipGetLastError();
}

hipError_t launch_gather_desc(const GatherSrc& g, int64_t m, TileDesc* desc, hipStream_t s) {
  if (m <= 0) return hipSuccess;
  if (!g.R || !g.A || !g.place || !g.gstart || !g.gadj || !desc || g.P < 1 || g.me < 0 || g.me >= g.P ||
      (g.nb != 256 && g.nb != 65536) || (int64_t)g.P * g.nb > (int64_t(1) << 30))
    return hipErrorInvalidValue;
  const int64_t TT = (m + kTile - 1) / kTile;
  const int64_t cells = (int64_t)g.P * g.nb;
  hipLaunchKernelGGL(k_gather_adj, dim3((unsigned)((cells + 255) / 256)), dim3(256), 0, s, g,
                     const_cast<int64_t*>(g.gadj));
  hipLaunchKernelGGL(k_gather_desc, dim3((unsigned)((TT + 255) / 256)), dim3(256), 0, s, g, m, TT, desc);
  return hipGetLastError();
}

hipError_t launch_copy_records(Elem* dst, const Elem* src, int64_t cnt, hipStream_t s) {
  if (cnt <= 0) return hipSuccess;
  hipLaunchKernelGGL(k_copy_records, dim3(grid_for(cnt, 256, 8192)), dim3(256), 0, s, dst, src, cnt);
  return hipGetLastError();
}

hipError_t launch_verify(const Elem* A, int64_t here, int64_t gbase, int64_t n, int64_t per,
                         KeyGen gen, unsigned long long* first_bad, hipStream_t s) {
  if (here <= 0) return hipSuccess;
  hipLaunchKernelGGL(k_verify, dim3(grid_for(here, 256, 8192)), dim3(256), 0, s, A, here, gbase, n,
                     per, gen, first_bad);
  return hipGetLastError();
}

hipError_t launch_check_sorted(const Elem* A, int64_t here, unsigned int* unsorted, hipStream_t s) {
  if (here <= 1) return hipSuccess;
  hipLaunchKernelGGL(k_check_sorted, dim3(grid_for(here, 256, 8192)), dim3(256), 0, s, A, here,
                     unsorted);
  return hipGetLastError();
}

}
```

distributed-lsb_amd/csrc/lsb_passes.cpp:

```cpp
#include "lsb_rt.h"

#include <cmath>

#include <deque>

namespace lsb_rt {

int local_pass(lsb_ctx* c, Rank& r, int shift, bool want_span, bool starts16) {
  HIP_TRY(hipSetDevice(r.dev));
  r.starts_fused = starts16;
  if (r.here == 0) {
    HIP_TRY(hipMemsetAsync(r.totals, 0, sizeof(uint64_t) * lsb::kBuckets, r.stream));
    return LSB_OK;
  }
  if (starts16) HIP_TRY(lsb::launch_starts_reset(r.first16, r.stream));
  const lsb::Chunking& ch = r.chunking;
  {
    Timer t(c, &r, LSB_K_UPSWEEP);
    HIP_TRY(lsb::launch_upsweep(r.A, r.here, shift, ch, r.chunk_hist,
                                want_span ? r.span : nullptr, r.stream));
  }
  {
    Timer t(c, &r, LSB_K_SCAN);
    HIP_TRY(lsb::launch_scan(r.chunk_hist, ch.num_chunks, r.chunk_off, r.totals, r.stream));
  }
  {
    Timer t(c, &r, LSB_K_SCATTER);
    HIP_TRY(lsb::launch_scatter(r.A, r.B, r.here, shift, ch, r.chunk_off, r.totals,
                                starts16 ? r.first16 : nullptr, r.stream));
    count_pass_elems(c, r.here);
  }
  std::swap(r.A, r.B);
  return LSB_OK;
}


int do_pass(lsb_ctx* c, int digit, uint64_t varying, bool want_span) {
  if (c->bits == 64 && exchanging(c)) return merge_sort(c);
  for (Rank& r : c->ranks) r.starts_fused = false;
  const int subs = c->bits / lsb::kDigitBits;
  for (int sub = 0; sub < subs; ++sub) {
    const int shift = digit * c->bits + sub * lsb::kDigitBits;
    if (!want_span && ((varying >> shift) & (lsb::kBuckets - 1)) == 0) continue;
    const bool starts16 = exchanging(c) && subs == 2 && sub == 1;
    begin_pass(c, shift);
    for (Rank& r : c->ranks) LSB_TRY(local_pass(c, r, shift, want_span && sub == 0, starts16));
    ++c->last_local_passes;
  }
  if (!exchanging(c)) return LSB_OK;
  ++c->last_exchanges;
  return exchange_digit(c, digit);
}

bool onesweep_applies(const lsb_ctx* c) {
  return c->onesweep && !exchanging(c) && c->ranks.size() == 1 && c->ranks[0].here > 0 &&
         c->ranks[0].here <= lsb::kOnesweepMaxElems;
}

constexpr int kRgCounts = 0, kRgHist = lsb::kRegions, kRgOvf = kRgHist + lsb::kBuckets,
              kRgSpan = kRgOvf + 2, kRgWords = kRgSpan + 4;

int onesweep_ensure(Rank& r) {
  if (r.os_status) return LSB_OK;
  const size_t tiles = (size_t)lsb::onesweep_tiles(r.here);
  LSB_TRY(dev_alloc(&r.os_status, tiles * lsb::kBuckets));
  LSB_TRY(dev_alloc(&r.os_hist, 2 * lsb::kOnesweepSubs * lsb::kBuckets));
  LSB_TRY(dev_alloc(&r.os_ctr, 2 * lsb::kOnesweepSubs));
  LSB_TRY(host_alloc(&r.os_err_h, 2));
  r.os_err_h[0] = r.os_err_h[1] = 0;
  LSB_TRY(host_alloc(&r.os_hist_h, (size_t)lsb::kOnesweepSubs * lsb::kBuckets));
  HIP_TRY(hipMemsetAsync(r.os_status, 0, tiles * lsb::kBuckets * sizeof(uint32_t), r.stream));
  HIP_TRY(hipMemsetAsync(r.os_ctr, 0, 2 * lsb::kOnesweepSubs * sizeof(uint32_t), r.stream));
  r.os_epoch = 0;
  r.os_grid = max_chunks_for_device(r.dev);
  if (r.rg_cap > 0) {
    const size_t rows = (size_t)lsb::onesweep_tiles(r.rg_cap * lsb::kRegions) * lsb::kBuckets;
    LSB_TRY(dev_alloc(&r.rg_buf, (size_t)kRgWords));
    LSB_TRY(host_alloc(&r.rg_h, (size_t)kRgWords));
    LSB_TRY(dev_alloc(&r.os_status2, rows));
    HIP_TRY(hipMemsetAsync(r.os_status2, 0, rows * sizeof(uint32_t), r.stream));
    r.os_epoch2 = 0;
  }
  return LSB_OK;
}

void zero_status(Rank& r) {
  (void)hipMemsetAsync(r.os_status, 0, (size_t)lsb::onesweep_tiles(r.here) * lsb::kBuckets * sizeof(uint32_t),
                       r.stream);
  if (r.os_status2)
    (void)hipMemsetAsync(r.os_status2, 0,
                         (size_t)lsb::onesweep_tiles(r.rg_cap * lsb::kRegions) * lsb::kBuckets * sizeof(uint32_t),
                         r.stream);
  r.os_epoch = 0;
  r.os_epoch2 = 0;
}

int onesweep_launch(lsb_ctx* c, Rank& r, int shift, int next, const uint32_t* hist,
                    uint32_t* next_hist, lsb::OnesweepExtra x) {
  if (r.os_dirty) {
    zero_status(r);
    HIP_TRY(hipGetLastError());
    r.os_dirty = false;
  }
  const bool track2 = x.region_mode == 2;
  uint32_t* status = track2 ? r.os_status2 : r.os_status;
  uint32_t& last_epoch = track2 ? r.os_epoch2 : r.os_epoch;
  if (!status) return fail(LSB_ERR_INVALID, "onesweep_launch", "regional layout's look-back rows");
  uint32_t epoch = last_epoch + 1;
  if (epoch >= (1u << 30)) epoch = 2;
  hipError_t e;
  if (c->fail_onesweep > 0 && --c->fail_onesweep == 0) {
    r.os_dirty = true;
    return fail(LSB_ERR_HIP, "launch_onesweep", "injected launch failure (LSB_OPT_FAIL_ONESWEEP)");
  }
  {
    Timer t(c, &r, LSB_K_SCATTER);
    e = lsb::launch_onesweep(r.A, r.B, r.here, shift, next, hist, next_hist, status, r.os_ctr,
                             epoch, r.os_ctr + lsb::kOnesweepSubs, r.os_grid, r.stream, x);
  }
  if (e != hipSuccess) {
    (void)hipGetLastError();
    r.os_dirty = true;
    return fail(LSB_ERR_HIP, "launch_onesweep", hipGetErrorString(e));
  }
  last_epoch = epoch;
  count_pass_elems(c, r.here);
  std::swap(r.A, r.B);
  return LSB_OK;
}

int queue_halves(lsb_ctx* c, Rank& r, const uint32_t* hist) {
  if (c->os_split != 0 || r.here == 0) return LSB_OK;
  HIP_TRY(hipMemcpyAsync(r.os_hist_h, hist, sizeof(uint32_t) * lsb::kOnesweepSubs * lsb::kBuckets,
                         hipMemcpyDeviceToHost, r.stream));
  return LSB_OK;
}

int choose_halves(lsb_ctx* c, Rank& r, bool synced) {
  if (c->os_split != 0 || r.here == 0) {
    r.os_halves = c->os_split == 2 ? 2 : 1;
    return LSB_OK;
  }
  if (!synced) HIP_TRY(hipStreamSynchronize(r.stream));
  r.os_halves = lsb::onesweep_halves_for(r.os_hist_h, r.here);
  return LSB_OK;
}

int count_byte(lsb_ctx* c, Rank& r, int byte, bool span) {
  Timer t(c, &r, LSB_K_UPSWEEP);
  HIP_TRY(lsb::launch_subhist(r.A, r.here, byte * lsb::kDigitBits, r.os_grid, r.os_hist,
                              span ? r.span : nullptr, r.stream));
  return LSB_OK;
}

std::vector<int> varying_bytes(uint64_t varying) {
  std::vector<int> d;
  for (int b = 0; b < 64 / lsb::kDigitBits; ++b)
    if (((varying >> (b * lsb::kDigitBits)) & (lsb::kBuckets - 1)) != 0) d.push_back(b);
  return d;
}

int onesweep_digits(lsb_ctx* c, Rank& r, const std::vector<int>& digits, int* passes, size_t from = 0,
                    const lsb::RegionPass* rp = nullptr, bool* disarm = nullptr) {
  uint32_t* hist[2] = {r.os_hist, r.os_hist + lsb::kOnesweepSubs * lsb::kBuckets};
  for (size_t i = from; i < digits.size(); ++i) {
    const int shift = digits[i] * lsb::kDigitBits;
    const int next = i + 1 < digits.size() ? digits[i + 1] * lsb::kDigitBits : -1;
    begin_pass(c, shift);
    lsb::OnesweepExtra x;
    x.halves = r.os_halves;
    if (rp && i == from) {
      x.region = rp;
      x.region_mode = 2;
    }
    LSB_TRY(onesweep_launch(c, r, shift, next, hist[i & 1], hist[(i + 1) & 1], x));
    ++*passes;
    if (disarm) *disarm = false;
  }
  return LSB_OK;
}


bool region_applies(const lsb_ctx* c, const Rank& r) {
  return c->region && !exchanging(c) && c->onesweep && c->os_split == 0 && r.rg_cap > 0 &&
         r.here == c->per && r.cap >= lsb::region_stride(r.rg_cap) * lsb::kRegions &&
         r.here <= lsb::kOnesweepMaxElems;
}

lsb::RegionPass region_pass(Rank& r) {
  lsb::RegionPass rp;
  rp.cap = r.rg_cap;
  rp.counts = r.rg_buf + kRgCounts;
  rp.ovf = r.rg_buf + kRgOvf;
  return rp;
}

int region_sample(lsb_ctx* c, Rank& r, int byte, bool* go, uint64_t* seen) {
  *go = false;
  if (!r.os_status2) return LSB_OK;
  {
    Timer t(c, &r, LSB_K_UPSWEEP);
    HIP_TRY(lsb::launch_sample(r.A, r.here, byte * lsb::kDigitBits, r.rg_buf + kRgHist,
                               reinterpret_cast<uint64_t*>(r.rg_buf + kRgSpan), r.stream));
  }
  HIP_TRY(hipMemcpyAsync(r.rg_h + kRgHist, r.rg_buf + kRgHist, (size_t)(kRgWords - kRgHist) * sizeof(uint32_t),
                         hipMemcpyDeviceToHost, r.stream));
  HIP_TRY(hipStreamSynchronize(r.stream));
  uint64_t S = 0, top = 0;
  for (int b = 0; b < lsb::kBuckets; ++b) {
    S += r.rg_h[kRgHist + b];
    top = std::max<uint64_t>(top, r.rg_h[kRgHist + b]);
  }
  uint64_t sp[2];
  memcpy(sp, r.rg_h + kRgSpan, sizeof sp);
  *seen = sp[0] & sp[1];
  bool every_byte = true;
  for (int b = 0; b < 64 / lsb::kDigitBits; ++b)
    every_byte = every_byte && ((*seen >> (b * lsb::kDigitBits)) & (lsb::kBuckets - 1)) != 0;
  const double mean = (double)S / lsb::kBuckets, sd = std::sqrt(mean);
  const double slack = (double)r.rg_cap / (double)lsb::region_mean(r.here);
  const double gate = std::min(mean + std::max(0.1 * mean, 6.0 * sd), mean * slack + 4.0 * sd);
  *go = every_byte && S > 0 && (double)top <= gate;
  return LSB_OK;
}

int region_first(lsb_ctx* c, Rank& r, int shift, int next_shift, int* passes) {
  const lsb::RegionPass rp = region_pass(r);
  begin_pass(c, shift);
  lsb::OnesweepExtra x;
  x.region = &rp;
  x.region_mode = 1;
  LSB_TRY(onesweep_launch(c, r, shift, next_shift, nullptr, r.os_hist + lsb::kOnesweepSubs * lsb::kBuckets, x));
  ++*passes;
  HIP_TRY(hipMemcpyAsync(r.rg_h + kRgOvf, r.rg_buf + kRgOvf, sizeof(uint32_t), hipMemcpyDeviceToHost, r.stream));
  return LSB_OK;
}

std::vector<int> hybrid_bytes(uint64_t varying, int64_t m) {
  int need = 0;
  while ((int64_t(1) << need) < m) ++need;
  std::vector<int> top;
  int bits = 0;
  for (int b = 64 / lsb::kDigitBits - 1; b >= 0 && bits < need; --b) {
    const uint64_t v = (varying >> (b * lsb::kDigitBits)) & (lsb::kBuckets - 1);
    if (!v) continue;
    top.insert(top.begin(), b);
    bits += __builtin_popcountll(v);
  }
  return top;
}

namespace {

struct LocalSort {
  lsb_ctx* c;
  Rank& r;
  int passes = 0;
  uint64_t varying = 0;
  enum Kind { kDone, kLsd, kHybrid } kind = kDone;
  int cursor = 0, cur = 0;
  int counted = -1;
  bool hist_queued = false;
  std::vector<int> digits, msd;
  bool fuse = false;
  bool region = false;
  Elem *X0 = nullptr, *X1 = nullptr, *X2 = nullptr;
  bool armed = false;
  uint64_t pmask = 0;
  lsb::SegPass sp;
  const Elem* seg_in = nullptr;
  uint32_t* err = nullptr;

  LocalSort(lsb_ctx* c_, Rank& r_) : c(c_), r(r_) {}
  LocalSort(const LocalSort&) = delete;
  ~LocalSort() {
    if (armed) {
      r.A = X0;
      r.B = X1;
      r.R = X2;
    }
  }
  struct Step {
    LocalSort& s;
    explicit Step(LocalSort& s_) : s(s_) {
      s.c->pass_cursor = s.cursor;
      s.c->cur_pass = s.cur;
    }
    ~Step() {
      s.cursor = s.c->pass_cursor;
      s.cur = s.c->cur_pass;
    }
  };

  int begin();
  int queue();
  int finish();
  int hybrid_passes(size_t from);
  int classic();
  int first_hist(int byte, bool* skewed, bool* constant);
  int queue_err_word() {
    HIP_TRY(hipMemcpyAsync(r.os_err_h, r.os_ctr + lsb::kOnesweepSubs, sizeof(uint32_t),
                           hipMemcpyDeviceToHost, r.stream));
    return LSB_OK;
  }
};

int LocalSort::classic() {
  HIP_TRY(hipMemsetAsync(r.span, 0, 2 * sizeof(uint64_t), r.stream));
  c->pass_cursor = 0;
  begin_pass(c, 0);
  LSB_TRY(local_pass(c, r, 0, c->skip_constant));
  passes = 1;
  varying = ~0ull;
  if (c->skip_constant) {
    HIP_TRY(hipMemcpyAsync(r.span_h, r.span, 2 * sizeof(uint64_t), hipMemcpyDeviceToHost, r.stream));
    HIP_TRY(hipStreamSynchronize(r.stream));
    varying = r.span_h[0] & r.span_h[1];
  }
  for (int d = 1; d < 64 / lsb::kDigitBits; ++d) {
    if (((varying >> (d * lsb::kDigitBits)) & (lsb::kBuckets - 1)) == 0) continue;
    begin_pass(c, d * lsb::kDigitBits);
    LSB_TRY(local_pass(c, r, d * lsb::kDigitBits));
    ++passes;
  }
  return LSB_OK;
}

int LocalSort::begin() {
  Step step(*this);
  kind = kDone;
  if (r.here == 0) return LSB_OK;
  HIP_TRY(hipSetDevice(r.dev));
  if (!c->onesweep || r.here > lsb::kOnesweepMaxElems) return classic();
  LSB_TRY(onesweep_ensure(r));
  c->pass_cursor = 0;
  c->cur_pass = 0;
  varying = ~0ull;
  HIP_TRY(hipMemsetAsync(r.span, 0, 2 * sizeof(uint64_t), r.stream));
  if (c->hybrid) {
    kind = kHybrid;
    LSB_TRY(ensure_recv(c, r));
    const std::vector<int> guess = hybrid_bytes(~0ull, r.here);
    region = false;
    if (guess.size() >= 3 && region_applies(c, r)) LSB_TRY(region_sample(c, r, guess[0], &region, &varying));
    if (region) {
      c->last_first = LSB_FIRST_REGIONAL;
      msd = guess;
      X0 = r.A;
      X1 = r.B;
      X2 = r.R;
      armed = true;
      LSB_TRY(region_first(c, r, guess[0] * lsb::kDigitBits, guess[1] * lsb::kDigitBits, &passes));
      r.B = X2;
      r.R = X0;
      return LSB_OK;
    }
    varying = ~0ull;
    counted = guess.empty() ? 0 : guess[0];
    LSB_TRY(count_byte(c, r, counted, c->skip_constant));
    HIP_TRY(hipMemcpyAsync(r.os_hist_h, r.os_hist, sizeof(uint32_t) * lsb::kOnesweepSubs * lsb::kBuckets,
                           hipMemcpyDeviceToHost, r.stream));
    hist_queued = true;
  } else {
    kind = kLsd;
    region = false;
    if (region_applies(c, r)) LSB_TRY(region_sample(c, r, 0, &region, &varying));
    if (region) {
      c->last_first = LSB_FIRST_REGIONAL;
      X0 = r.A;
      X1 = r.B;
      X2 = r.R;
      armed = true;
      return region_first(c, r, 0, lsb::kDigitBits, &passes);
    }
    varying = ~0ull;
    LSB_TRY(count_byte(c, r, 0, c->skip_constant));
    LSB_TRY(queue_halves(c, r, r.os_hist));
  }
  if (c->skip_constant)
    HIP_TRY(hipMemcpyAsync(r.span_h, r.span, 2 * sizeof(uint64_t), hipMemcpyDeviceToHost, r.stream));
  return LSB_OK;
}

int LocalSort::first_hist(int byte, bool* skewed, bool* constant) {
  if (byte != counted) {
    LSB_TRY(count_byte(c, r, byte, false));
    counted = byte;
    hist_queued = false;
  }
  if (!hist_queued)
    HIP_TRY(hipMemcpyAsync(r.os_hist_h, r.os_hist, sizeof(uint32_t) * lsb::kOnesweepSubs * lsb::kBuckets,
                           hipMemcpyDeviceToHost, r.stream));
  hist_queued = false;
  HIP_TRY(hipStreamSynchronize(r.stream));
  const int64_t m = r.here;
  const int h = lsb::onesweep_halves_for(r.os_hist_h, m);
  r.os_halves = c->os_split == 0 ? h : (c->os_split == 2 ? 2 : 1);
  *skewed = h == 2;
  *constant = false;
  for (int b = 0; b < lsb::kBuckets && !*constant; ++b) {
    uint64_t tot = 0;
    for (int x = 0; x < lsb::kOnesweepSubs; ++x) tot += r.os_hist_h[x * lsb::kBuckets + b];
    *constant = tot == (uint64_t)m;
  }
  return LSB_OK;
}

int LocalSort::queue() {
  if (kind == kDone) return LSB_OK;
  Step step(*this);
  HIP_TRY(hipSetDevice(r.dev));
  const int64_t m = r.here;
  if (kind == kLsd && region) {
    region = false;
    HIP_TRY(hipStreamSynchronize(r.stream));
    digits = varying_bytes(~0ull);
    if (r.rg_h[kRgOvf] == 0) {
      r.os_halves = 1;
      const lsb::RegionPass rp = region_pass(r);
      LSB_TRY(onesweep_digits(c, r, digits, &passes, 1, &rp, &armed));
      kind = kDone;
      return queue_err_word();
    }
    c->last_first = LSB_FIRST_REGIONAL_REDONE;
    std::swap(r.A, r.B);
    armed = false;
    passes = 0;
    c->pass_cursor = 0;
    c->cur_pass = 0;
    HIP_TRY(hipMemsetAsync(r.span, 0, 2 * sizeof(uint64_t), r.stream));
    LSB_TRY(count_byte(c, r, 0, c->skip_constant));
    LSB_TRY(queue_halves(c, r, r.os_hist));
    HIP_TRY(hipMemcpyAsync(r.span_h, r.span, 2 * sizeof(uint64_t), hipMemcpyDeviceToHost, r.stream));
    HIP_TRY(hipStreamSynchronize(r.stream));
    varying = c->skip_constant ? r.span_h[0] & r.span_h[1] : ~0ull;
    digits = varying_bytes(varying);
    LSB_TRY(choose_halves(c, r, true));
    LSB_TRY(onesweep_digits(c, r, digits, &passes));
    kind = kDone;
    return queue_err_word();
  }
  if (kind == kHybrid && region) {
    region = false;
    HIP_TRY(hipStreamSynchronize(r.stream));
    if (r.rg_h[kRgOvf] == 0) {
      digits = varying_bytes(~0ull);
      r.os_halves = 1;
      return hybrid_passes(1);
    }
    r.A = X0;
    r.B = X1;
    r.R = X2;
    armed = false;
    passes = 0;
    c->pass_cursor = 0;
    c->cur_pass = 0;
    c->last_first = LSB_FIRST_REGIONAL_REDONE;
    HIP_TRY(hipMemsetAsync(r.span, 0, 2 * sizeof(uint64_t), r.stream));
    counted = msd[0];
    LSB_TRY(count_byte(c, r, counted, c->skip_constant));
    HIP_TRY(hipMemcpyAsync(r.os_hist_h, r.os_hist, sizeof(uint32_t) * lsb::kOnesweepSubs * lsb::kBuckets,
                           hipMemcpyDeviceToHost, r.stream));
    hist_queued = true;
    if (c->skip_constant)
      HIP_TRY(hipMemcpyAsync(r.span_h, r.span, 2 * sizeof(uint64_t), hipMemcpyDeviceToHost, r.stream));
    varying = ~0ull;
  }
  if (c->skip_constant) HIP_TRY(hipStreamSynchronize(r.stream));
  if (c->skip_constant) varying = r.span_h[0] & r.span_h[1];
  digits = varying_bytes(varying);
  if (kind == kLsd) {
    if (!digits.empty() && digits[0] != 0) {
      LSB_TRY(count_byte(c, r, digits[0], false));
      LSB_TRY(queue_halves(c, r, r.os_hist));
      LSB_TRY(choose_halves(c, r, false));
    } else {
      LSB_TRY(choose_halves(c, r, c->skip_constant));
    }
    LSB_TRY(onesweep_digits(c, r, digits, &passes));
    kind = kDone;
    return queue_err_word();
  }
  msd = hybrid_bytes(c->skip_constant ? varying : ~0ull, m);
  bool hybrid = msd.size() < digits.size();
  bool skewed = false, constant = false;
  if (hybrid && !msd.empty()) {
    LSB_TRY(first_hist(msd[0], &skewed, &constant));
    if (skewed || constant) hybrid = false;
  }
  if (!hybrid) {
    if (!digits.empty()) LSB_TRY(first_hist(digits[0], &skewed, &constant));
    LSB_TRY(onesweep_digits(c, r, digits, &passes));
    kind = kDone;
    return queue_err_word();
  }
  return hybrid_passes(0);
}

int LocalSort::hybrid_passes(size_t from) {
  const int64_t m = r.here;
  if (from == 0) {
    X0 = r.A;
    X1 = r.B;
    X2 = r.R;
    armed = true;
  }
  for (int b : msd) pmask |= (uint64_t)(lsb::kBuckets - 1) << (b * lsb::kDigitBits);
  err = r.os_ctr + lsb::kOnesweepSubs + 1;
  fuse = c->hybrid == 1 && r.os_halves == 1 && !msd.empty();
  if (fuse) {
    if (!r.seg_base) LSB_TRY(dev_alloc(&r.seg_base, (size_t)lsb::kOnesweepSubs * lsb::kBuckets));
    sp.pmask = pmask;
    sp.rmask = pmask & ~((uint64_t)(lsb::kBuckets - 1) << (msd.back() * lsb::kDigitBits));
    sp.base = r.seg_base;
    sp.err = err;
  }
  HIP_TRY(hipMemsetAsync(err, 0, sizeof(uint32_t), r.stream));
  uint32_t* hist[2] = {r.os_hist, r.os_hist + lsb::kOnesweepSubs * lsb::kBuckets};
  const lsb::RegionPass rp = from == 1 ? region_pass(r) : lsb::RegionPass();
  for (size_t i = from; i < msd.size(); ++i) {
    const int shift = msd[i] * lsb::kDigitBits;
    const int next = i + 1 < msd.size() ? msd[i + 1] * lsb::kDigitBits : -1;
    begin_pass(c, shift);
    lsb::OnesweepExtra x;
    x.halves = r.os_halves;
    if (from == 1 && i == 1) {
      x.region = &rp;
      x.region_mode = 2;
    }
    if (fuse && i + 1 == msd.size()) {
      x.seg = &sp;
      seg_in = r.A;
    }
    LSB_TRY(onesweep_launch(c, r, shift, next, hist[i & 1], hist[(i + 1) & 1], x));
    ++passes;
    if (i == 0) {
      r.B = X2;
      r.R = X0;
    }
  }
  if (msd.empty()) {
    r.B = X1;
    r.R = X2;
  }
  if (fuse) {
    {
      Timer t(c, &r, LSB_K_SEGSORT);
      HIP_TRY(lsb::launch_segfix(seg_in, r.A, m, msd.back() * lsb::kDigitBits, r.os_status, sp,
                                 16 * r.os_grid, r.stream));
    }
    HIP_TRY(hipMemcpyAsync(r.os_err_h + 1, err, sizeof(uint32_t), hipMemcpyDeviceToHost, r.stream));
  }
  return LSB_OK;
}

int LocalSort::finish() {
  if (kind != kHybrid) return LSB_OK;
  Step step(*this);
  HIP_TRY(hipSetDevice(r.dev));
  auto sync_err = [&](uint32_t* v) -> int {
    HIP_TRY(hipStreamSynchronize(r.stream));
    *v = r.os_err_h[1];
    return LSB_OK;
  };
  bool sorted = false, a_valid = true;
  if (fuse) {
    uint32_t e = 0;
    LSB_TRY(sync_err(&e));
    sorted = e == 0;
    a_valid = (e & 2u) == 0;
  }
  if (!sorted && a_valid) {
    HIP_TRY(hipMemsetAsync(err, 0, sizeof(uint32_t), r.stream));
    begin_pass(c, 64);
    {
      Timer t(c, &r, LSB_K_SEGSORT);
      HIP_TRY(lsb::launch_segsort(r.A, r.B, r.here, pmask, err, 3 * r.os_grid / 2, r.stream));
    }
    count_pass_elems(c, r.here, false);
    ++passes;
    HIP_TRY(hipMemcpyAsync(r.os_err_h + 1, err, sizeof(uint32_t), hipMemcpyDeviceToHost, r.stream));
// ... 79 lines not shown
```

distributed-lsb_amd/csrc/lsb_rt.h:

```cpp
#pragma once
#include <hip/hip_runtime.h>
#include <rccl/rccl.h>

#include <algorithm>
#include <cstdio>
#include <cstdlib>
#include <cstring>
#include <new>
#include <string>
#include <vector>

#include "../../include/lsb.h"
#include "lsb_kernels.h"
#include "lsb_xgeom.h"

namespace lsb_rt {

using lsb::Elem;

enum class Mode { kLoopback, kRccl, kOps };

struct PendingEvent {
  int kid;
  int dev;
// ... 32 lines not shown
  int64_t* counts_h = nullptr;
  lsb::Chunking chunking;
  Elem* buf[2] = {nullptr, nullptr};
  std::vector<Elem*> peer0, peer1;
  std::vector<void*> ipc_opened;
  int64_t* peer_base = nullptr;
  uint32_t* os_status = nullptr;
  uint32_t* os_hist = nullptr;
  uint32_t* os_ctr = nullptr;
  uint32_t* os_err_h = nullptr;
  uint32_t* os_hist_h = nullptr;
  int os_halves = 1;
  uint32_t os_epoch = 0;
  bool os_dirty = false;
  int64_t* seg_base = nullptr;
  int os_grid = 0;
  int64_t cap = 0;
  int64_t rg_cap = 0;
  uint32_t* os_status2 = nullptr;
  uint32_t os_epoch2 = 0;
  uint32_t* rg_buf = nullptr;
  uint32_t* rg_h = nullptr;
  int os_cur = 0;
  int os_valid = -1;
  int place_next = -1;
  uint32_t* place_hist = nullptr;
  bool counts_ready = false;
  bool gather_next = false;
  bool gather_pending = false;
  int64_t* gstart = nullptr;
  lsb::TileDesc* gdesc = nullptr;
  lsb::GatherSrc gsrc;
  hipStream_t xstream = nullptr;
  hipEvent_t ck_hi[lsb::kMaxExchangeChunks] = {};
  hipEvent_t ck_wire[lsb::kMaxExchangeChunks] = {};
  hipEvent_t xdone = nullptr;
  uint32_t* ck_hist = nullptr;
  int64_t* ck_counts = nullptr;
  int64_t* ck_counts_h = nullptr;
  uint32_t* lo_hist_h = nullptr;
  uint64_t* split_state = nullptr;
  int64_t* split_targets = nullptr;
  uint64_t* split_cnt = nullptr;
  uint64_t* split_gather = nullptr;
  uint64_t* split_fin = nullptr;
  uint64_t* split_fin_gather = nullptr;
  uint64_t* split_h = nullptr;
  int64_t* merge_path = nullptr;
  int split_q = 0, split_S = 0;
  std::vector<int64_t> mcut;
  std::vector<int64_t> send_counts, send_displs, recv_counts, recv_displs;
};

}

struct lsb_ctx {
  lsb_rt::Mode mode = lsb_rt::Mode::kLoopback;
  int64_t n = 0;
  int64_t per = 0;
  int P = 1;
  int bits = 8;
  int nb = 256;
  int first_rank = 0;
  std::vector<lsb_rt::Rank> ranks;
  ncclComm_t comm = nullptr;
  lsb_comm_ops_t ops = {};
  bool timing = false;
  bool shared_device = false;
  std::vector<int> access_devs;
  bool force_exchange = false;
  bool skip_constant = true;
  int slices = 0;
  int xchunks = 0;
  int xchunk_reserve = 0;
  bool p2p = false;
  bool peer = false;
  bool peer_ready = false;
  bool onesweep = true;
  bool region = true;
  bool self_coll = false;
  bool gather = true;
  int os_split = 0;
  int fail_onesweep = 0;
  int hybrid = 0;
  int64_t coll_calls = 0, coll_bytes = 0, coll_max = 0;
  int last_local_passes = 0;
  int last_exchanges = 0;
  uint64_t last_varying = 0;
  int last_first = 0;
  lsb::KeyGen keygen;
  std::vector<lsb_rt::PendingEvent> pending;
  std::vector<std::pair<int, hipEvent_t>> event_pool;
  int64_t launches[LSB_K_COUNT] = {};
  double total_ms[LSB_K_COUNT] = {};
  int64_t scatter_elems = 0;
  int cur_pass = 0;
  int pass_cursor = 0;
  int pass_shift[LSB_MAX_PASSES] = {};
  int64_t pass_launches[LSB_MAX_PASSES][LSB_K_COUNT] = {};
  double pass_ms[LSB_MAX_PASSES][LSB_K_COUNT] = {};
  int64_t pass_elems[LSB_MAX_PASSES] = {};
  int64_t xs_exchanges = 0, xs_calls = 0;
  int64_t xs_sent[LSB_MAX_RANKS] = {}, xs_recv[LSB_MAX_RANKS] = {};
  int64_t xs_place_bytes = 0, xs_placed = 0, xs_counted = 0;
  int64_t pass_xbytes[LSB_MAX_PASSES] = {};
};

#define HIP_TRY(expr)                                                    \
  do {                                                                   \
    hipError_t _e = (expr);                                              \
    if (_e != hipSuccess) return fail(LSB_ERR_HIP, #expr, hipGetErrorString(_e)); \
  } while (0)

#define RCCL_TRY(expr)                                                   \
  do {                                                                   \
    ncclResult_t _r = (expr);                                            \
    if (_r != ncclSuccess) return fail(LSB_ERR_RCCL, #expr, ncclGetErrorString(_r)); \
  } while (0)

#define LSB_TRY(expr)              \
  do {                             \
    int _c = (expr);               \
    if (_c != LSB_OK) return _c;   \
  } while (0)

namespace lsb_rt {

const std::string& last_error();

inline int64_t div_ceil(int64_t x, int64_t y) { return (x + y - 1) / y; }

inline int64_t here_of(int64_t n, int P, int r) {
  const int64_t per = P > 0 ? div_ceil(n, P) : 0;
  int64_t h = per;
  if (per * r + h > n) h = n - per * r;
  return h < 0 ? 0 : h;
}

inline bool exchanging(const lsb_ctx* c) { return c->P > 1 || c->force_exchange; }

hipEvent_t take_event(lsb_ctx* c);

struct Timer {
  lsb_ctx* c;
  Rank* r;
  int kid;
  int pass;
  hipStream_t stream;
  hipEvent_t start = nullptr;
  Timer(lsb_ctx* c_, Rank* r_, int kid_, hipStream_t s = nullptr)
      : c(c_), r(r_), kid(kid_), pass(kid_ == LSB_K_SORT ? -1 : c_->cur_pass),
        stream(s ? s : r_->stream) {
    if (!c->timing) return;
    start = take_event(c);
    if (start) (void)hipEventRecord(start, stream);
  }
  void stop() {
    if (!start) return;
    hipEvent_t e = take_event(c);
    if (!e) return;
    (void)hipEventRecord(e, stream);
    c->pending.push_back({kid, r->dev, pass, start, e});
    start = nullptr;
  }
  ~Timer() { stop(); }
};

void begin_pass(lsb_ctx* c, int shift);
void count_pass_elems(lsb_ctx* c, int64_t m, bool scatter = true);
int resolve_timing(lsb_ctx* c);

template <typename T>
// ... 113 lines not shown
```

distributed-lsb_amd/lsbsort/__init__.py:

```python
from __future__ import annotations

import ctypes
import os
import sys
from typing import Optional, Sequence

import numpy as np

PKG_DIR = os.path.dirname(os.path.abspath(__file__))
ROOT_DIR = os.path.dirname(PKG_DIR)
LIB_PATH = os.environ.get("LSB_LIBRARY") or os.path.join(ROOT_DIR, "build", "liblsb.so")
HARNESS_PATH = os.path.join(ROOT_DIR, "build", "hip_lsbsort")
HEADER_PATH = os.path.join(os.path.dirname(ROOT_DIR), "include", "lsb.h")

ELEM_DTYPE = np.dtype([("key", "<u8"), ("val", "<u8")])
UNIQUE_ID_BYTES = 128

LSB_OK = 0
LSB_ERR_VERIFY = 5
DIST_UNIFORM, DIST_ZIPF = 0, 1
K_UPSWEEP, K_SCAN, K_SCATTER, K_EXCHANGE, K_PLACE, K_SORT, K_SEGSORT, K_WIRE, K_PLACE_TAIL = range(9)
KERNEL_NAMES = ("upsweep", "scan", "scatter", "exchange", "place", "sort", "segsort", "wire", "place_tail")
MAX_RANKS = 64
OPT_TIMING, OPT_FORCE_EXCHANGE, OPT_SKIP_CONSTANT_DIGITS, OPT_EXCHANGE_SLICES, OPT_EXCHANGE_P2P = 0, 1, 2, 3, 4
OPT_EXCHANGE_PEER = 5
OPT_ONESWEEP = 6
OPT_EXCHANGE_SELF = 7
OPT_ONESWEEP_SPLIT = 8
OPT_HYBRID = 9
OPT_EXCHANGE_GATHER = 10
OPT_FAIL_ONESWEEP = 11
OPT_REGION_FIRST = 12
OPT_EXCHANGE_CHUNKS = 13
FIRST_COUNT, FIRST_REGIONAL, FIRST_REGIONAL_REDONE = 0, 1, 2
MAX_PASSES = 16


class LsbError(RuntimeError):
    def __init__(self, code: int, where: str):
        msg = _lib().lsb_strerror(code).decode()
        super().__init__(f"{where}: lsb error {code}: {msg}")
        self.code = code


_L = None


_ALLGATHER = ctypes.CFUNCTYPE(ctypes.c_int, ctypes.c_void_p, ctypes.c_void_p, ctypes.c_void_p,
                              ctypes.c_size_t)
_ALLTOALLV = ctypes.CFUNCTYPE(ctypes.c_int, ctypes.c_void_p, ctypes.c_void_p,
                              ctypes.POINTER(ctypes.c_size_t), ctypes.POINTER(ctypes.c_size_t),
                              ctypes.c_void_p, ctypes.POINTER(ctypes.c_size_t),
                              ctypes.POINTER(ctypes.c_size_t))
_ALLREDUCE_MIN = ctypes.CFUNCTYPE(ctypes.c_int, ctypes.c_void_p, ctypes.POINTER(ctypes.c_int64))
_BARRIER = ctypes.CFUNCTYPE(ctypes.c_int, ctypes.c_void_p)


class ExchangeStats(ctypes.Structure):
    _fields_ = [("exchanges", ctypes.c_int64), ("calls", ctypes.c_int64),
                ("sent_bytes", ctypes.c_int64 * 64), ("recv_bytes", ctypes.c_int64 * 64),
                ("wire_ms", ctypes.c_double), ("plan_ms", ctypes.c_double), ("place_ms", ctypes.c_double),
                ("place_tail_ms", ctypes.c_double), ("place_bytes", ctypes.c_int64),
                ("placed_records", ctypes.c_int64), ("counted_records", ctypes.c_int64)]


class CommOps(ctypes.Structure):
    _fields_ = [("user", ctypes.c_void_p), ("allgather", _ALLGATHER), ("alltoallv", _ALLTOALLV),
                ("allreduce_min_i64", _ALLREDUCE_MIN), ("barrier", _BARRIER)]


def _bytes_at(ptr, n):
    if n == 0:
        return np.zeros(0, dtype=np.uint8)
    return np.ctypeslib.as_array((ctypes.c_uint8 * n).from_address(ptr))


def _make_comm_ops(comm, P):
    def guard(fn):
        def wrapped(*a):
            try:
                fn(*a)
                return 0
            except Exception as e:
                print(f"lsbsort comm callback failed: {e!r}", file=sys.stderr)
                return 1
        return wrapped

    def allgather(_u, send, recv, nbytes):
        _bytes_at(recv, nbytes * P)[:] = comm.allgather(_bytes_at(send, nbytes).copy())

    def alltoallv(_u, send, sc, sd, recv, rc, rd):
        scn = [sc[i] for i in range(P)]
        sdn = [sd[i] for i in range(P)]
        rcn = [rc[i] for i in range(P)]
        rdn = [rd[i] for i in range(P)]
        send_len = max([d + c for d, c in zip(sdn, scn) if c] or [0])
        recv_len = max([d + c for d, c in zip(rdn, rcn) if c] or [0])
        comm.alltoallv(_bytes_at(send, send_len), scn, sdn, _bytes_at(recv, recv_len), rcn, rdn)

    def allreduce_min(_u, v):
        v[0] = int(comm.allreduce_min(int(v[0])))

    def barrier(_u):
        comm.barrier()

    keep = (_ALLGATHER(guard(allgather)), _ALLTOALLV(guard(alltoallv)),
            _ALLREDUCE_MIN(guard(allreduce_min)), _BARRIER(guard(barrier)))
    ops = CommOps(None, *keep)
    return ops, keep


def _lib() -> ctypes.CDLL:
    global _L
    if _L is None:
        if not os.path.exists(LIB_PATH):
            raise RuntimeError(
                f"HIP library {LIB_PATH} is not built; run `make -C distributed-lsb_amd` "
                "(or __graft_entry__.build())")
        L = ctypes.CDLL(LIB_PATH)
        i64, i32, vp, cp = ctypes.c_int64, ctypes.c_int, ctypes.c_void_p, ctypes.c_char_p
        P64 = ctypes.POINTER(ctypes.c_int64)
        sig = {
            "lsb_per_rank": (i64, [i64, i32]),
            "lsb_here": (i64, [i64, i32, i32]),
            "lsb_create": (i32, [ctypes.POINTER(vp), i64, i32, ctypes.POINTER(ctypes.c_int), i32]),
            "lsb_get_unique_id": (i32, [ctypes.c_char_p]),
            "lsb_device_count": (i32, [ctypes.POINTER(ctypes.c_int)]),
            "lsb_create_rank": (i32, [ctypes.POINTER(vp), i64, i32, i32, i32, i32, ctypes.c_char_p]),
            "lsb_create_rank_ops": (i32, [ctypes.POINTER(vp), i64, i32, i32, i32, i32,
                                          ctypes.POINTER(CommOps)]),
            "lsb_destroy": (None, [vp]),
            "lsb_set_option": (i32, [vp, i32, i64]),
            "lsb_get_last_sort": (i32, [vp, vp, vp, vp]),
            "lsb_get_first_pass": (i32, [vp, vp]),
            "lsb_local_ranks": (i32, [vp, ctypes.POINTER(ctypes.c_int), ctypes.POINTER(ctypes.c_int)]),
            "lsb_generate": (i32, [vp]),
            "lsb_generate_ex": (i32, [vp, i32, ctypes.c_double]),
            "lsb_copy_in": (i32, [vp, i32, i64, i64, vp]),
            "lsb_copy_out": (i32, [vp, i32, i64, i64, vp]),
            "lsb_sort": (i32, [vp]),
            "lsb_pass": (i32, [vp, i32]),
            "lsb_sync": (i32, [vp]),
            "lsb_barrier": (i32, [vp]),
            "lsb_verify": (i32, [vp, P64]),
            "lsb_check_sorted": (i32, [vp, ctypes.POINTER(ctypes.c_int)]),
            "lsb_get_kernel_stats": (i32, [vp, i32, P64, ctypes.POINTER(ctypes.c_double)]),
            "lsb_reset_kernel_stats": (i32, [vp]),
            "lsb_get_scatter_elems": (i32, [vp, P64]),
            "lsb_get_pass_stats": (i32, [vp, i32, ctypes.POINTER(ctypes.c_int), P64, P64,
                                         ctypes.POINTER(ctypes.c_double), ctypes.POINTER(ctypes.c_double),
                                         ctypes.POINTER(ctypes.c_double), ctypes.POINTER(ctypes.c_double)]),
            "lsb_get_exchange_bytes": (i32, [vp, P64, P64, P64]),
            "lsb_get_exchange_stats": (i32, [vp, ctypes.POINTER(ExchangeStats)]),
            "lsb_get_placement": (i32, [vp, i32, ctypes.POINTER(ctypes.c_int), ctypes.POINTER(ctypes.c_double),
                                        ctypes.POINTER(ctypes.c_double), ctypes.POINTER(ctypes.c_double)]),
            "lsb_get_pass_exchange": (i32, [vp, i32, P64, ctypes.POINTER(ctypes.c_double),
                                            ctypes.POINTER(ctypes.c_double)]),
            "lsb_build_info": (cp, []),
            "lsb_rank_footprint": (i32, [i64, i32, i32, i32, P64, P64]),
            "lsb_device_memory": (i32, [i32, P64, P64]),
            "lsb_plan_exchange": (i32, [i64, i32, i32, i32, vp, vp, vp, vp, vp, vp]),
            "lsb_plan_exchange_device": (i32, [i32, i64, i32, i32, i32, vp, vp, vp, vp, vp, vp]),
            "lsb_plan_merge": (i32, [i64, i32, i32, vp, vp, vp, vp, vp, vp]),
            "lsb_strerror": (cp, [i32]),
        }
        for name, (res, args) in sig.items():
            fn = getattr(L, name)
            fn.restype = res
            fn.argtypes = args
        _L = L
    return _L


def _check(code: int, where: str) -> None:
    if code != LSB_OK:
        raise LsbError(code, where)


def per_rank(n: int, P: int) -> int:
    return int(_lib().lsb_per_rank(n, P))


def here(n: int, P: int, r: int) -> int:
    return int(_lib().lsb_here(n, P, r))


def rank_footprint(n: int, P: int, radix_bits: int = 8, with_recv: bool = False) -> dict:
    b, pb = ctypes.c_int64(), ctypes.c_int64()
    _check(_lib().lsb_rank_footprint(n, P, radix_bits, int(with_recv), ctypes.byref(b), ctypes.byref(pb)),
           "lsb_rank_footprint")
    return {"bytes": b.value, "probe_bytes": pb.value}


def device_memory(dev: int = 0) -> tuple:
    f, t = ctypes.c_int64(), ctypes.c_int64()
    _check(_lib().lsb_device_memory(dev, ctypes.byref(f), ctypes.byref(t)), "lsb_device_memory")
    return f.value, t.value


def build_info() -> dict:
    info = _lib().lsb_build_info().decode()
    return dict(kv.split("=", 1) for kv in info.split())


def source_files() -> list:
    import re
    mk = open(os.path.join(ROOT_DIR, "Makefile")).read()
    rt = re.search(r"^RT\s*:=\s*(.*)$", mk, re.M).group(1).split()
    files = []
    for tok in re.search(r"^SOURCES\s*:=\s*(.*)$", mk, re.M).group(1).split():
        if tok.startswith("$(RT:"):
            files += [f"csrc/{u}.cpp" for u in rt]
        else:
            files.append(tok)
    return files


# ... 124 lines not shown

    def copy_out(self, rank: int, off: int = 0, cnt: Optional[int] = None) -> np.ndarray:
        if cnt is None:
            cnt = self.here(rank) - off
        out = np.empty(cnt, dtype=ELEM_DTYPE)
        _check(_lib().lsb_copy_out(self._h, rank, off, cnt, out.ctypes.data if cnt else None),
               "lsb_copy_out")
        return out

    def scatter_global(self, arr: np.ndarray) -> None:
        arr = np.ascontiguousarray(arr, dtype=ELEM_DTYPE)
        if arr.size != self.n:
            raise ValueError("need exactly n records")
        for r in self.local_ranks:
            h = self.here(r)
            if h:
                self.copy_in(r, arr[r * self.per: r * self.per + h])

    def gather_global(self) -> np.ndarray:
        if len(self.local_ranks) != self.P:
            raise RuntimeError("gather_global needs all ranks in this process")
        parts = [self.copy_out(r) for r in range(self.P)]
        return np.concatenate(parts) if parts else np.empty(0, dtype=ELEM_DTYPE)

    def my_sort(self) -> None:
        _check(_lib().lsb_sort(self._h), "lsb_sort")

    def global_shuffle(self, digit: int) -> None:
        _check(_lib().lsb_pass(self._h, digit), "lsb_pass")

    mySort = my_sort
    globalShuffle = global_shuffle

    def sync(self) -> None:
        _check(_lib().lsb_sync(self._h), "lsb_sync")

    def barrier(self) -> None:
        _check(_lib().lsb_barrier(self._h), "lsb_barrier")

    def verify(self):
        bad = ctypes.c_int64(-1)
        rc = _lib().lsb_verify(self._h, ctypes.byref(bad))
        if rc not in (LSB_OK, LSB_ERR_VERIFY):
            _check(rc, "lsb_verify")
        return rc == LSB_OK, int(bad.value)

    def check_sorted(self) -> bool:
        s = ctypes.c_int(0)
        _check(_lib().lsb_check_sorted(self._h, ctypes.byref(s)), "lsb_check_sorted")
        return bool(s.value)

    checkSorted = check_sorted

    def print_lines(self, name: str = "A", n_per_rank: int = 10):
        lines = []
        if n_per_rank * self.P >= self.n:
            lines.append(f"{name}: displaying all {self.n} elements")
        else:
            lines.append(f"{name}: displaying first {n_per_rank} elements on each rank"
                         f" out of {self.n} elements")
        for r in self.local_ranks:
            h = self.here(r)
            k = min(n_per_rank, h)
            for i, e in enumerate(self.copy_out(r, 0, k)):
                lines.append(f"{name}[{r * self.per + i}] = ({int(e['key']):016x},{int(e['val'])})")
            if k < h:
                lines.append("...")
        return lines

    def set_timing(self, on: bool = True) -> None:
        self.set_option(OPT_TIMING, 1 if on else 0)

    def last_sort(self) -> tuple:
        lp, ex, vb = ctypes.c_int(), ctypes.c_int(), ctypes.c_uint64()
        _check(_lib().lsb_get_last_sort(self._h, ctypes.byref(lp), ctypes.byref(ex), ctypes.byref(vb)),
               "lsb_get_last_sort")
        return int(lp.value), int(ex.value), int(vb.value)

    def first_pass(self) -> int:
        f = ctypes.c_int()
        _check(_lib().lsb_get_first_pass(self._h, ctypes.byref(f)), "lsb_get_first_pass")
        return int(f.value)

    def kernel_stats(self) -> dict:
        out = {}
        for kid, name in enumerate(KERNEL_NAMES):
            n = ctypes.c_int64()
            ms = ctypes.c_double()
            _check(_lib().lsb_get_kernel_stats(self._h, kid, ctypes.byref(n), ctypes.byref(ms)),
                   "lsb_get_kernel_stats")
            out[name] = (int(n.value), float(ms.value))
        return out

    def pass_stats(self) -> list:
        out = []
        for p in range(MAX_PASSES):
            sh, la, el = ctypes.c_int(), ctypes.c_int64(), ctypes.c_int64()
            ms = [ctypes.c_double() for _ in range(4)]
            _check(_lib().lsb_get_pass_stats(self._h, p, ctypes.byref(sh), ctypes.byref(la), ctypes.byref(el),
                                             *[ctypes.byref(x) for x in ms]), "lsb_get_pass_stats")
            if sh.value < 0:
                continue
            xb, wire, tail = ctypes.c_int64(), ctypes.c_double(), ctypes.c_double()
            _check(_lib().lsb_get_pass_exchange(self._h, p, ctypes.byref(xb), ctypes.byref(wire),
                                                ctypes.byref(tail)), "lsb_get_pass_exchange")
            out.append({"pass": p, "shift": int(sh.value), "launches": int(la.value), "elems": int(el.value),
                        "ms_count": ms[0].value, "ms_scatter": ms[1].value, "ms_exchange": ms[2].value,
                        "ms_place": ms[3].value, "exchange_bytes": int(xb.value), "ms_wire": wire.value,
                        "ms_place_tail": tail.value})
        return out

    def placement(self, rank: Optional[int] = None) -> dict:
        r = self.local_ranks[0] if rank is None else rank
        k = ctypes.c_int()
        ms = [ctypes.c_double() for _ in range(3)]
        _check(_lib().lsb_get_placement(self._h, r, ctypes.byref(k), *[ctypes.byref(x) for x in ms]),
               "lsb_get_placement")
        return {"candidates": int(k.value), "chosen_ms": round(ms[0].value, 4),
                "first_pair_ms": round(ms[1].value, 4), "worst_ms": round(ms[2].value, 4)}

    def exchange_stats(self) -> dict:
        st = ExchangeStats()
        _check(_lib().lsb_get_exchange_stats(self._h, ctypes.byref(st)), "lsb_get_exchange_stats")
        return {"exchanges": int(st.exchanges), "calls": int(st.calls),
                "sent_bytes": [int(x) for x in st.sent_bytes[:self.P]],
                "recv_bytes": [int(x) for x in st.recv_bytes[:self.P]],
                "wire_ms": st.wire_ms, "plan_ms": st.plan_ms, "place_ms": st.place_ms,
                "place_tail_ms": st.place_tail_ms, "place_bytes": int(st.place_bytes),
                "placed_records": int(st.placed_records), "counted_records": int(st.counted_records)}

    def reset_kernel_stats(self) -> None:
        _check(_lib().lsb_reset_kernel_stats(self._h), "lsb_reset_kernel_stats")

    def scatter_elems(self) -> int:
        e = ctypes.c_int64()
        _check(_lib().lsb_get_scatter_elems(self._h, ctypes.byref(e)), "lsb_get_scatter_elems")
        return int(e.value)

    def exchange_bytes(self) -> tuple:
        c, b, mx = ctypes.c_int64(), ctypes.c_int64(), ctypes.c_int64()
        _check(_lib().lsb_get_exchange_bytes(self._h, ctypes.byref(c), ctypes.byref(b), ctypes.byref(mx)),
               "lsb_get_exchange_bytes")
        return int(c.value), int(b.value), int(mx.value)


def mySort(world: World) -> None:
    world.my_sort()


def globalShuffle(world: World, digit: int) -> None:
    world.global_shuffle(digit)
```

include/lsb.h:

```cpp
#ifndef LSB_H
#define LSB_H

#include <stddef.h>
#include <stdint.h>

#ifdef __cplusplus
extern "C" {
#endif

#define LSB_OK                 0
#define LSB_ERR_INVALID        1
#define LSB_ERR_HIP            2
#define LSB_ERR_RCCL           3
#define LSB_ERR_NOMEM          4
#define LSB_ERR_VERIFY         5
#define LSB_ERR_UNSUPPORTED    6
#define LSB_ERR_STATE          7

#define LSB_UNIQUE_ID_BYTES  128

typedef struct lsb_elem {
  uint64_t key;
  uint64_t val;
} lsb_elem_t;

typedef struct lsb_ctx lsb_ctx_t;

#define LSB_K_UPSWEEP   0
#define LSB_K_SCAN      1
#define LSB_K_SCATTER   2
#define LSB_K_EXCHANGE  3
#define LSB_K_PLACE     4
#define LSB_K_SORT      5
#define LSB_K_SEGSORT   6
#define LSB_K_WIRE      7
#define LSB_K_PLACE_TAIL 8
#define LSB_K_COUNT     9
#define LSB_MAX_RANKS  64

#define LSB_OPT_TIMING          0
#define LSB_OPT_FORCE_EXCHANGE  1
#define LSB_OPT_SKIP_CONSTANT_DIGITS 2
#define LSB_OPT_EXCHANGE_SLICES 3
#define LSB_OPT_EXCHANGE_P2P    4
#define LSB_OPT_EXCHANGE_PEER   5
#define LSB_OPT_ONESWEEP        6
#define LSB_OPT_EXCHANGE_SELF   7
#define LSB_OPT_ONESWEEP_SPLIT  8
#define LSB_OPT_HYBRID          9
#define LSB_OPT_EXCHANGE_GATHER 10
#define LSB_OPT_FAIL_ONESWEEP   11
#define LSB_OPT_REGION_FIRST    12
#define LSB_OPT_EXCHANGE_CHUNKS 13

int64_t lsb_per_rank(int64_t n_total, int num_ranks);
int64_t lsb_here(int64_t n_total, int num_ranks, int rank);

int  lsb_create(lsb_ctx_t** ctx, int64_t n_total, int num_ranks,
                const int* dev_ids, int radix_bits);
int  lsb_device_count(int* count);
int  lsb_get_unique_id(unsigned char id[LSB_UNIQUE_ID_BYTES]);
int  lsb_create_rank(lsb_ctx_t** ctx, int64_t n_total, int num_ranks, int rank,
                     int dev_id, int radix_bits,
                     const unsigned char id[LSB_UNIQUE_ID_BYTES]);
typedef struct lsb_comm_ops {
  void* user;
  int (*allgather)(void* user, const void* send, void* recv, size_t bytes);
  int (*alltoallv)(void* user, const void* send, const size_t* send_bytes,
                   const size_t* send_displs, void* recv, const size_t* recv_bytes,
                   const size_t* recv_displs);
  int (*allreduce_min_i64)(void* user, int64_t* value);
  int (*barrier)(void* user);
} lsb_comm_ops_t;
int  lsb_create_rank_ops(lsb_ctx_t** ctx, int64_t n_total, int num_ranks, int rank,
                         int dev_id, int radix_bits, const lsb_comm_ops_t* ops);
void lsb_destroy(lsb_ctx_t* ctx);
int  lsb_set_option(lsb_ctx_t* ctx, int option, int64_t value);
int  lsb_local_ranks(const lsb_ctx_t* ctx, int* first_rank, int* num_local);

int  lsb_generate(lsb_ctx_t* ctx);
#define LSB_DIST_UNIFORM 0
#define LSB_DIST_ZIPF    1
int  lsb_generate_ex(lsb_ctx_t* ctx, int dist, double param);
int  lsb_copy_in(lsb_ctx_t* ctx, int rank, int64_t off, int64_t cnt, const lsb_elem_t* host);
int  lsb_copy_out(lsb_ctx_t* ctx, int rank, int64_t off, int64_t cnt, lsb_elem_t* host);

int  lsb_sort(lsb_ctx_t* ctx);
int  lsb_get_last_sort(lsb_ctx_t* ctx, int* local_passes, int* exchanges,
                       uint64_t* varying_bits);
#define LSB_FIRST_COUNT           0
#define LSB_FIRST_REGIONAL        1
#define LSB_FIRST_REGIONAL_REDONE 2
int  lsb_get_first_pass(lsb_ctx_t* ctx, int* form);
int  lsb_pass(lsb_ctx_t* ctx, int digit);
int  lsb_sync(lsb_ctx_t* ctx);
int  lsb_barrier(lsb_ctx_t* ctx);

int  lsb_verify(lsb_ctx_t* ctx, int64_t* first_bad);
int  lsb_check_sorted(lsb_ctx_t* ctx, int* sorted);

int  lsb_get_kernel_stats(lsb_ctx_t* ctx, int kernel_id, int64_t* launches, double* total_ms);
int  lsb_reset_kernel_stats(lsb_ctx_t* ctx);
int  lsb_get_scatter_elems(lsb_ctx_t* ctx, int64_t* elems);
#define LSB_MAX_PASSES 16
int  lsb_get_pass_stats(lsb_ctx_t* ctx, int pass, int* shift, int64_t* launches, int64_t* elems,
                        double* ms_count, double* ms_scatter, double* ms_exchange, double* ms_place);
int  lsb_get_exchange_bytes(lsb_ctx_t* ctx, int64_t* calls, int64_t* bytes, int64_t* max_call_bytes);
typedef struct lsb_exchange_stats {
  int64_t exchanges;
  int64_t calls;
  int64_t sent_bytes[LSB_MAX_RANKS];
  int64_t recv_bytes[LSB_MAX_RANKS];
  double wire_ms, plan_ms, place_ms, place_tail_ms;
  int64_t place_bytes;
  int64_t placed_records;
  int64_t counted_records;
} lsb_exchange_stats_t;
int  lsb_get_exchange_stats(lsb_ctx_t* ctx, lsb_exchange_stats_t* out);
int  lsb_get_pass_exchange(lsb_ctx_t* ctx, int pass, int64_t* bytes, double* wire_ms,
                           double* place_tail_ms);

int  lsb_get_placement(lsb_ctx_t* ctx, int rank, int* candidates, double* chosen_ms,
                       double* first_pair_ms, double* worst_ms);

int  lsb_rank_footprint(int64_t n_total, int num_ranks, int radix_bits, int with_recv,
                        int64_t* bytes, int64_t* probe_bytes);

int  lsb_device_memory(int dev, int64_t* free_bytes, int64_t* total_bytes);

const char* lsb_build_info(void);

int  lsb_plan_exchange(int64_t n_total, int num_ranks, int rank, int nbuckets,
                       const int64_t* hist,
                       int64_t* send_counts, int64_t* send_displs,
                       int64_t* recv_counts, int64_t* recv_displs,
                       int64_t* place_off);

int  lsb_plan_exchange_device(int dev_id, int64_t n_total, int num_ranks, int rank, int nbuckets,
                              const int64_t* hist,
                              int64_t* send_counts, int64_t* send_displs,
                              int64_t* recv_counts, int64_t* recv_displs,
                              int64_t* place_off);

int  lsb_plan_merge(int64_t n_total, int num_ranks, int rank, const int64_t* below,
                    const int64_t* upto, int64_t* send_counts, int64_t* send_displs,
                    int64_t* recv_counts, int64_t* recv_displs);

const char* lsb_strerror(int code);

#ifdef __cplusplus
}
#endif

#endif
```

Before: 19970.

## Pack records to 12 bytes in intermediate onesweep passes when values fit 32 bits

The sample kernel and the first regional pass now check whether any value uses its high 32 bits. When none do (on by default with pack_values=1), the intermediate onesweep passes read and write 12-byte packed records instead of 16-byte ones, and the last pass unpacks back to full records. This is meant to cut HBM traffic per pass by about a quarter. In exchange it adds a wide-value detection path that falls back to a counted restart, recovery logic for failed packed passes, and a broken-state flag, all of which add complexity and risk.

```diff
diff --git a/distributed-lsb_amd/csrc/lsb_abi.cpp b/distributed-lsb_amd/csrc/lsb_abi.cpp
--- a/distributed-lsb_amd/csrc/lsb_abi.cpp
+++ b/distributed-lsb_amd/csrc/lsb_abi.cpp
@@ -228,6 +228,10 @@
     case LSB_OPT_REGION_FIRST:
       c->region = value != 0;
       return LSB_OK;
+    case LSB_OPT_PACK_VALUES:
+      if (value < 0 || value > 2) return fail(LSB_ERR_INVALID, "lsb_set_option", "pack values must be 0, 1 or 2");
+      c->pack_values = (int)value;
+      return LSB_OK;
     case LSB_OPT_EXCHANGE_PEER:
       c->peer = value != 0;
       return LSB_OK;
@@ -293,6 +297,7 @@
     HIP_TRY(lsb::launch_pcg_fill(r.A, c->per, (uint64_t)r.rank, (uint64_t)r.rank * c->per, g,
                                  r.stream));
   }
+  c->broken = false;
   return lsb_sync(c);
 }
 
@@ -353,6 +358,7 @@
   c->last_local_passes = c->last_exchanges = 0;
   c->last_varying = ~0ull;
   c->last_first = LSB_FIRST_COUNT;
+  c->last_records = LSB_RECORDS_FULL;
   c->pass_cursor = 0;
   c->cur_pass = 0;
   if (c->bits == 64 && exchanging(c)) {
@@ -386,6 +392,8 @@
 
 int lsb_sort(lsb_ctx_t* c) {
   LSB_TRY(check_ctx(c));
+  if (c->broken)
+    return fail(LSB_ERR_STATE, "lsb_sort", "an earlier sort failed and left packed records in A; load the input again");
   const int rc = sort_body(c);
   if (rc != LSB_OK) quiesce(c);
   return rc;
@@ -403,6 +411,13 @@
   LSB_TRY(check_ctx(c));
   if (!form) return fail(LSB_ERR_INVALID, "lsb_get_first_pass", "null");
   *form = c->last_first;
+  return LSB_OK;
+}
+
+int lsb_get_last_records(lsb_ctx_t* c, int* form) {
+  LSB_TRY(check_ctx(c));
+  if (!form) return fail(LSB_ERR_INVALID, "lsb_get_last_records", "null");
+  *form = c->last_records;
   return LSB_OK;
 }
 
diff --git a/distributed-lsb_amd/csrc/lsb_context.cpp b/distributed-lsb_amd/csrc/lsb_context.cpp
--- a/distributed-lsb_amd/csrc/lsb_context.cpp
+++ b/distributed-lsb_amd/csrc/lsb_context.cpp
@@ -325,6 +325,10 @@
   c->bits = radix_bits;
   c->nb = radix_bits == 64 ? lsb::kBuckets : 1 << radix_bits;
   if (const char* e = getenv("LSB_REGION_FIRST")) c->region = atoi(e) != 0;
+  if (const char* e = getenv("LSB_PACK_VALUES")) {
+    const int v = atoi(e);
+    if (v >= 0 && v <= 2) c->pack_values = v;
+  }
   if (const char* e = getenv("LSB_EXCHANGE_CHUNKS")) {
     const int v = atoi(e);
     c->xchunks = v == 2 || v == 4 || v == 8 ? v : 0;
diff --git a/distributed-lsb_amd/csrc/lsb_kernels.h b/distributed-lsb_amd/csrc/lsb_kernels.h
--- a/distributed-lsb_amd/csrc/lsb_kernels.h
+++ b/distributed-lsb_amd/csrc/lsb_kernels.h
@@ -10,6 +10,11 @@
   uint64_t val;
 };
 static_assert(sizeof(Elem) == 16, "16-byte records");
+struct alignas(4) Packed {
+  uint32_t klo, khi;
+  uint32_t val;
+};
+static_assert(sizeof(Packed) == 12, "12-byte packed records");
 
 constexpr int kDigitBits = 8;
 constexpr int kBuckets = 1 << kDigitBits;
@@ -134,8 +139,9 @@
   int64_t cap = 0;
   uint32_t* counts = nullptr;
   uint32_t* ovf = nullptr;
-};
-hipError_t launch_sample(const Elem* A, int64_t m, int shift, uint32_t* hist, uint64_t* span,
+  uint32_t* wide = nullptr;
+};
+hipError_t launch_sample(const Elem* A, int64_t m, int shift, uint32_t* hist, uint64_t* span, uint32_t* wide,
                          hipStream_t s);
 struct OnesweepExtra {
   uint64_t* totals = nullptr;
@@ -146,6 +152,7 @@
   bool probe = false;
   const RegionPass* region = nullptr;
   int region_mode = 0;
+  bool pack_in = false, pack_out = false;
 };
 int onesweep_halves_for(const uint32_t* sub_hist_host, int64_t m);
 hipError_t launch_onesweep(const Elem* in, Elem* out, int64_t m, int shift, int next_shift,
@@ -200,6 +207,7 @@
 hipError_t launch_merge_level(const MergeLevel& level, int64_t* path, int grid, hipStream_t s);
 
 hipError_t launch_copy_records(Elem* dst, const Elem* src, int64_t cnt, hipStream_t s);
+hipError_t launch_unpack(Elem* dst, const Packed* src, int64_t cnt, hipStream_t s);
 hipError_t launch_verify(const Elem* A, int64_t here, int64_t gbase, int64_t n, int64_t per,
                          KeyGen gen, unsigned long long* first_bad, hipStream_t s);
 
diff --git a/distributed-lsb_amd/csrc/lsb_kernels.hip b/distributed-lsb_amd/csrc/lsb_kernels.hip
--- a/distributed-lsb_amd/csrc/lsb_kernels.hip
+++ b/distributed-lsb_amd/csrc/lsb_kernels.hip
@@ -89,6 +89,28 @@
 
 __device__ __forceinline__ void store_elem(Elem* p, const Elem& e) {
   *reinterpret_cast<ulonglong2*>(p) = make_ulonglong2(e.key, e.val);
+}
+
+__device__ __forceinline__ Packed load_elem_nt(const Packed* p) {
+  const uint32_t* w = reinterpret_cast<const uint32_t*>(p);
+  return Packed{__builtin_nontemporal_load(w), __builtin_nontemporal_load(w + 1), __builtin_nontemporal_load(w + 2)};
+}
+
+__device__ __forceinline__ void store_elem(Packed* p, const Packed& e) { *p = e; }
+
+__device__ __forceinline__ uint64_t rec_key(const Elem& e) { return e.key; }
+__device__ __forceinline__ uint64_t rec_key(const Packed& e) { return ((uint64_t)e.khi << 32) | e.klo; }
+__device__ __forceinline__ uint64_t rec_val(const Elem& e) { return e.val; }
+__device__ __forceinline__ uint64_t rec_val(const Packed& e) { return e.val; }
+template <typename R>
+__device__ __forceinline__ R make_rec(uint64_t key, uint64_t val);
+template <>
+__device__ __forceinline__ Elem make_rec<Elem>(uint64_t key, uint64_t val) {
+  return Elem{key, val};
+}
+template <>
+__device__ __forceinline__ Packed make_rec<Packed>(uint64_t key, uint64_t val) {
+  return Packed{(uint32_t)key, (uint32_t)(key >> 32), (uint32_t)val};
 }
 
 template <typename T>
@@ -674,7 +696,8 @@
 constexpr int kSampleTiles = 256;
 __global__ __launch_bounds__(kSampleBlock) void k_sample(const Elem* __restrict__ A, int64_t m, int shift,
                                                          uint32_t* __restrict__ hist,
-                                                         unsigned long long* __restrict__ span) {
+                                                         unsigned long long* __restrict__ span,
+                                                         uint32_t* __restrict__ wide) {
   constexpr int IPT = kTile / kSampleBlock;
   __shared__ uint32_t h[kBuckets];
   h[threadIdx.x] = 0;
@@ -683,11 +706,13 @@
   const int64_t tb = (int64_t)blockIdx.x * TT / gridDim.x * kTile;
   const uint64_t* __restrict__ keys = reinterpret_cast<const uint64_t*>(A);
   uint64_t kor = 0, knor = 0;
+  uint32_t vhi = 0;
 #pragma unroll
   for (int i = 0; i < IPT; ++i) {
     const int64_t idx = tb + (int64_t)i * kSampleBlock + threadIdx.x;
     if (idx < m) {
       const uint64_t k = __builtin_nontemporal_load(keys + 2 * idx);
+      vhi |= (uint32_t)(__builtin_nontemporal_load(keys + 2 * idx + 1) >> 32);
       kor |= k;
       knor |= ~k;
       atomicAdd(&h[(uint32_t)(k >> shift) & (kBuckets - 1)], 1u);
@@ -702,6 +727,7 @@
     atomicOr(&span[0], (unsigned long long)kor);
     atomicOr(&span[1], (unsigned long long)knor);
   }
+  if (__ballot(vhi != 0) != 0 && lane_id() == 0) atomicOr(wide, 1u);
   __syncthreads();
   if (h[threadIdx.x]) atomicAdd(&hist[threadIdx.x], h[threadIdx.x]);
 }
@@ -734,9 +760,9 @@
 #define LSB_GATHER_PF 64
 #endif
 
-template <int BLOCK, int IPT, bool NEXT, bool C16, int HALVES, bool SEG, bool GATHER, int RG>
+template <int BLOCK, int IPT, bool NEXT, bool C16, int HALVES, bool SEG, bool GATHER, int RG, bool PIN, bool POUT>
 __device__ __forceinline__ void onesweep_body(
-    const Elem* __restrict__ in, Elem* __restrict__ out, int64_t m, int shift, int next_shift,
+    const Elem* __restrict__ in_, Elem* __restrict__ out_, int64_t m, int shift, int next_shift,
     const uint32_t* __restrict__ sub_hist, uint32_t* __restrict__ next_hist,
     uint32_t* __restrict__ status, uint32_t* __restrict__ tile_ctr, uint32_t epoch,
     uint32_t* __restrict__ err, uint64_t* __restrict__ totals,
@@ -746,11 +772,19 @@
   static_assert(!SEG || (!NEXT && !C16 && HALVES == 1), "the segment pass: last pass, whole stage");
   static_assert(RG == 0 || (!C16 && HALVES == 1 && !SEG && !GATHER), "regional passes: plain whole stage");
   static_assert(RG != 1 || NEXT, "the regional first pass counts the next digit");
+  static_assert(!(PIN || POUT) || (!C16 && HALVES == 1 && !SEG && !GATHER), "packed records: plain whole stage");
+  static_assert(!(RG == 1 && PIN) && !(RG == 2 && !PIN && POUT), "only the first pass packs");
+  using RIn = typename std::conditional<PIN, Packed, Elem>::type;
+  using ROut = typename std::conditional<POUT, Packed, Elem>::type;
+  const RIn* __restrict__ in = reinterpret_cast<const RIn*>(in_);
+  ROut* __restrict__ out = reinterpret_cast<ROut*>(out_);
   static_assert(BLOCK % kBuckets == 0, "bucket threads");
   using WC = typename std::conditional<(W > 4), uint16_t, uint32_t>::type;
 
   constexpr int HT = T / HALVES;
-  __shared__ Elem stage[HT];
+  __shared__ Elem stage[POUT ? 1 : HT];
+  __shared__ uint64_t skey[POUT ? HT : 1];
+  __shared__ uint32_t sval[POUT ? HT : 1];
   __shared__ WC wcnt[W][kBuckets];
   __shared__ int64_t delta[kBuckets];
   __shared__ uint32_t cut[NEXT ? kBuckets : 1];
@@ -769,6 +803,7 @@
   const int64_t TTn = RG == 1 ? rg.cap / T * kRegions : (m + T - 1) / T;
   const int64_t mcap = RG == 1 ? region_stride(rg.cap) * kRegions : m;
   uint32_t racc = 0;
+  uint32_t vhi = 0;
   constexpr uint32_t kValMask = kStatusValMask, kPreBit = 1u << 30;
   const uint32_t tag_agg = (epoch & 1u) << 31, tag_pre = tag_agg | kPreBit;
   const int shift16 = shift - 8;
@@ -880,7 +915,7 @@
       tb = region_base(rg_reg, rg.cap) + (int64_t)rg_k * T;
     }
 
-    Elem e[IPT];
+    RIn e[IPT];
     const int wbase = w * 64 * IPT + (int)lane;
     if (GATHER) {
       const int dn = __builtin_amdgcn_readfirstlane(s_desc.n);
@@ -916,7 +951,7 @@
             for (int k = 1; k < kDescPieces; ++k) src = li >= st[k] ? pb[k] : src;
           }
           LSB_DASSERT(li >= nvalid || gather_in(gs, src + li));
-          e[i] = li < nvalid ? load_elem_nt(src + li) : Elem{0ull, 0ull};
+          if constexpr (GATHER) e[i] = li < nvalid ? load_elem_nt(src + li) : Elem{0ull, 0ull};
         }
       } else {
         const int e0 = s_desc.e0, e1 = s_desc.e1;
@@ -924,7 +959,8 @@
         for (int i = 0; i < IPT; ++i) {
           const int li = wbase + i * 64;
           LSB_DASSERT(li >= nvalid || gather_in(gs, gather_search(gs, e0, e1, tb + li)));
-          e[i] = li < nvalid ? load_elem_nt(gather_search(gs, e0, e1, tb + li)) : Elem{0ull, 0ull};
+          if constexpr (GATHER)
+            e[i] = li < nvalid ? load_elem_nt(gather_search(gs, e0, e1, tb + li)) : Elem{0ull, 0ull};
           __builtin_amdgcn_sched_barrier(0);
         }
       }
@@ -939,7 +975,13 @@
 #pragma unroll
       for (int i = 0; i < IPT; ++i) {
         const int li = wbase + i * 64;
-        e[i] = RG == 2 || li < nvalid ? load_elem_nt(in + tb + li) : Elem{0ull, 0ull};
+        if (PIN && RG != 2) {
+          e[i] = load_elem_nt(in + tb + (li < nvalid ? li : nvalid - 1));
+          if (li >= nvalid) e[i] = RIn{};
+        } else {
+          e[i] = RG == 2 || li < nvalid ? load_elem_nt(in + tb + li) : RIn{};
+        }
+        if (!PIN && POUT) vhi |= (uint32_t)(rec_val(e[i]) >> 32);
       }
       if (RG == 2) {
         __builtin_amdgcn_sched_barrier(0);
@@ -971,7 +1013,7 @@
 #pragma unroll
     for (int i = 0; i < IPT; ++i) {
       const bool valid = wbase + i * 64 < nvalid;
-      const uint32_t d = (uint32_t)(e[i].key >> shift) & (kBuckets - 1);
+      const uint32_t d = (uint32_t)(rec_key(e[i]) >> shift) & (kBuckets - 1);
       const uint64_t mt = match_digit8(d, __ballot(valid));
       const uint32_t below = mbcnt(mt);
       const uint32_t pre = wcnt[w][d];
@@ -979,8 +1021,8 @@
       if (valid && below == 0) wcnt[w][d] = (WC)(pre + (uint32_t)__popcll(mt));
       if (C16) {
         const int li = wbase + i * 64;
-        if (li == 0) tile_lo[0] = (uint32_t)(e[i].key >> shift16) & 0xFFu;
-        if (li == nvalid - 1) tile_lo[1] = (uint32_t)(e[i].key >> shift16) & 0xFFu;
+        if (li == 0) tile_lo[0] = (uint32_t)(rec_key(e[i]) >> shift16) & 0xFFu;
+        if (li == nvalid - 1) tile_lo[1] = (uint32_t)(rec_key(e[i]) >> shift16) & 0xFFu;
       }
     }
     __syncthreads();
@@ -1026,12 +1068,16 @@
 #pragma unroll
       for (int i = 0; i < IPT; ++i) {
         if (wbase + i * 64 < nvalid) {
-          const uint32_t d = (uint32_t)(e[i].key >> shift) & (kBuckets - 1);
-          if (HALVES == 1) {
-            stage[wcnt[w][d] + rk[i]] = e[i];
+          const uint32_t d = (uint32_t)(rec_key(e[i]) >> shift) & (kBuckets - 1);
+          if (POUT) {
+            const uint32_t p = wcnt[w][d] + rk[i];
+            skey[p] = rec_key(e[i]);
+            sval[p] = (uint32_t)rec_val(e[i]);
+          } else if (HALVES == 1) {
+            stage[wcnt[w][d] + rk[i]] = make_rec<Elem>(rec_key(e[i]), rec_val(e[i]));
           } else {
             if (h == 0) rk[i] += wcnt[w][d];
-            if ((int)(rk[i] / HT) == h) stage[rk[i] - h * HT] = e[i];
+            if ((int)(rk[i] / HT) == h) stage[rk[i] - h * HT] = make_rec<Elem>(rec_key(e[i]), rec_val(e[i]));
           }
         }
       }
@@ -1107,14 +1153,14 @@
       grab(nxt_tile, nxt_sub);
     }
 
-    auto emit = [&](auto skew_tag, const Elem& v, int j, int64_t g, uint32_t c) {
+    auto emit = [&](auto skew_tag, const ROut& v, int j, int64_t g, uint32_t c) {
       constexpr bool kSkew = decltype(skew_tag)::value;
       LSB_DASSERT(g >= 0 && g < mcap);
       const uint64_t gs = (uint64_t)g < (uint64_t)(mcap - 1) ? (uint64_t)g : (uint64_t)(mcap - 1);
       store_elem(out + gs, v);
       if (NEXT) {
         const uint32_t xs = (uint32_t)j >= (c & 0xFFFFu) ? (c >> 24) : ((c >> 16) & 0xFFu);
-        const uint32_t dn = (uint32_t)(v.key >> next_shift) & (kBuckets - 1);
+        const uint32_t dn = (uint32_t)(rec_key(v) >> next_shift) & (kBuckets - 1);
         const uint32_t slot = xs * kBuckets + dn;
         if (kSkew) {
           const uint64_t act = __ballot(1);
@@ -1207,33 +1253,44 @@
         constexpr int G = SEG && LSB_SEG_BATCH > 0 && LSB_SEG_BATCH < HT / BLOCK ? LSB_SEG_BATCH : HT / BLOCK;
 #pragma unroll
         for (int k0 = 0; k0 < HT / BLOCK; k0 += G) {
-          Elem v[G];
+          ROut v[G];
           int64_t dl[G];
           uint32_t ct[G];
-#pragma unroll
-          for (int k = 0; k < G; ++k) v[k] = stage[(k0 + k) * BLOCK + t];
+          if constexpr (POUT) {
+            uint64_t kk[G];
+#pragma unroll
+            for (int k = 0; k < G; ++k) kk[k] = skey[(k0 + k) * BLOCK + t];
+#pragma unroll
+            for (int k = 0; k < G; ++k) v[k] = make_rec<Packed>(kk[k], sval[(k0 + k) * BLOCK + t]);
+          } else {
+#pragma unroll
+            for (int k = 0; k < G; ++k) v[k] = stage[(k0 + k) * BLOCK + t];
+          }
 #pragma unroll
           for (int k = 0; k < G; ++k) {
-            const uint32_t d = (uint32_t)(v[k].key >> shift) & (kBuckets - 1);
+            const uint32_t d = (uint32_t)(rec_key(v[k]) >> shift) & (kBuckets - 1);
             dl[k] = delta[d];
             ct[k] = NEXT ? cut[d] : 0u;
           }
 #pragma unroll
           for (int k = 0; k < G; ++k) {
             const int j = (k0 + k) * BLOCK + t;
-            emit(skew_tag, v[k], j, dl[k] + (SEG ? seg_pos(v[k], j, jend) : j), ct[k]);
+            if constexpr (SEG) emit(skew_tag, v[k], j, dl[k] + seg_pos(v[k], j, jend), ct[k]);
+            else emit(skew_tag, v[k], j, dl[k] + j, ct[k]);
           }
         }
         return;
       }
       for (int j = h * HT + t; j < jend; j += BLOCK) {
-        const Elem v = stage[j - h * HT];
+        ROut v;
+        if constexpr (POUT) v = make_rec<Packed>(skey[j], sval[j]);
+        else v = stage[j - h * HT];
         int pos = j;
-        if (SEG) pos = seg_pos(v, j, jend);
-        const uint32_t d = (uint32_t)(v.key >> shift) & (kBuckets - 1);
+        if constexpr (SEG) pos = seg_pos(v, j, jend);
+        const uint32_t d = (uint32_t)(rec_key(v) >> shift) & (kBuckets - 1);
         emit(skew_tag, v, j, delta[d] + pos, NEXT ? cut[d] : 0u);
         if (C16 && mixed16) {
-          const uint32_t s16 = (d << 8) | ((uint32_t)(v.key >> shift16) & 0xFFu);
+          const uint32_t s16 = (d << 8) | ((uint32_t)(rec_key(v) >> shift16) & 0xFFu);
           const uint64_t act = __ballot(1);
           const uint32_t prev = (uint32_t)__builtin_amdgcn_update_dpp((int)~s16, (int)s16, 0x138, 0xf, 0xf, false);
           const bool head = prev != s16;
@@ -1268,18 +1325,20 @@
       if (nh[i]) atomicAdd(&next_hist[i], nh[i]);
   }
   if (RG == 1 && bkt && cur_sub >= 0 && racc) atomicAdd(&rg.counts[t * kSub + cur_sub], racc);
-}
-
-template <int BLOCK, int IPT, bool NEXT, bool C16, int HALVES, bool SEG = false, bool GATHER = false, int RG = 0>
+  if (!PIN && POUT && __ballot(vhi != 0) != 0 && lane == 0) atomicOr(rg.wide, 1u);
+}
+
+template <int BLOCK, int IPT, bool NEXT, bool C16, int HALVES, bool SEG = false, bool GATHER = false, int RG = 0,
+          bool PIN = false, bool POUT = false>
 __global__ __launch_bounds__(BLOCK, (HALVES == 1 ? 2 : 3) * BLOCK / 256) void k_onesweep(
     const Elem* __restrict__ in, Elem* __restrict__ out, int64_t m, int shift, int next_shift,
     const uint32_t* __restrict__ sub_hist, uint32_t* __restrict__ next_hist,
     uint32_t* __restrict__ status, uint32_t* __restrict__ tile_ctr, uint32_t epoch,
     uint32_t* __restrict__ err, uint64_t* __restrict__ totals,
     unsigned long long* __restrict__ count16, SegPass seg, GatherSrc gs, RegionPass rg) {
-  onesweep_body<BLOCK, IPT, NEXT, C16, HALVES, SEG, GATHER, RG>(in, out, m, shift, next_shift, sub_hist,
-                                                                next_hist, status, tile_ctr, epoch, err, totals,
-                                                                count16, seg, gs, rg);
+  onesweep_body<BLOCK, IPT, NEXT, C16, HALVES, SEG, GATHER, RG, PIN, POUT>(in, out, m, shift, next_shift, sub_hist,
+                                                                           next_hist, status, tile_ctr, epoch, err,
+                                                                           totals, count16, seg, gs, rg);
 }
 
 __global__ __launch_bounds__(kOsBlock, 2 * kOsBlock / 256) void k_onesweep_probe(
@@ -1288,9 +1347,9 @@
     uint32_t* __restrict__ status, uint32_t* __restrict__ tile_ctr, uint32_t epoch,
     uint32_t* __restrict__ err, uint64_t* __restrict__ totals,
     unsigned long long* __restrict__ count16, SegPass seg, GatherSrc gs) {
-  onesweep_body<kOsBlock, kOsIpt, true, false, 1, false, false, 0>(in, out, m, shift, next_shift, sub_hist,
-                                                                   next_hist, status, tile_ctr, epoch, err,
-                                                                   totals, count16, seg, gs, RegionPass());
+  onesweep_body<kOsBlock, kOsIpt, true, false, 1, false, false, 0, false, false>(
+      in, out, m, shift, next_shift, sub_hist, next_hist, status, tile_ctr, epoch, err, totals, count16, seg, gs,
+      RegionPass());
 }
 
 constexpr int kPlaceBlock = 256;
@@ -1695,6 +1754,14 @@
     store_elem(dst + i, load_elem_nt(src + i));
 }
 
+__global__ __launch_bounds__(256) void k_unpack(Elem* __restrict__ dst, const Packed* __restrict__ src, int64_t cnt) {
+  const int64_t stride = (int64_t)gridDim.x * 256;
+  for (int64_t i = (int64_t)blockIdx.x * 256 + threadIdx.x; i < cnt; i += stride) {
+    const Packed p = load_elem_nt(src + i);
+    store_elem(dst + i, Elem{rec_key(p), rec_val(p)});
+  }
+}
+
 __global__ __launch_bounds__(256) void k_verify(const Elem* __restrict__ A, int64_t here,
                                                 int64_t gbase, int64_t n, int64_t per, KeyGen gen,
                                                 unsigned long long* first_bad) {
@@ -1858,15 +1925,17 @@
   return hipGetLastError();
 }
 
-hipError_t launch_sample(const Elem* A, int64_t m, int shift, uint32_t* hist, uint64_t* span, hipStream_t s) {
-  if (shift < 0 || shift > 56) return hipErrorInvalidValue;
+hipError_t launch_sample(const Elem* A, int64_t m, int shift, uint32_t* hist, uint64_t* span, uint32_t* wide,
+                         hipStream_t s) {
+  if (shift < 0 || shift > 56 || !wide) return hipErrorInvalidValue;
   hipError_t e = hipMemsetAsync(hist, 0, sizeof(uint32_t) * kBuckets, s);
   if (e == hipSuccess) e = hipMemsetAsync(span, 0, 2 * sizeof(uint64_t), s);
+  if (e == hipSuccess) e = hipMemsetAsync(wide, 0, sizeof(uint32_t), s);
   if (e != hipSuccess || m <= 0) return e;
   const int64_t TT = (m + kTile - 1) / kTile;
   const unsigned g = (unsigned)(TT < kSampleTiles ? TT : kSampleTiles);
   hipLaunchKernelGGL(k_sample, dim3(g), dim3(kSampleBlock), 0, s, A, m, shift, hist,
-                     reinterpret_cast<unsigned long long*>(span));
+                     reinterpret_cast<unsigned long long*>(span), wide);
   return hipGetLastError();
 }
 
@@ -1913,6 +1982,9 @@
   if (rm != 0) {
     if (c16 || extra.halves != 1 || extra.seg || gat || extra.probe || extra.totals) return hipErrorInvalidValue;
     if (rm == 1 && (next_shift < 0 || !rp.ovf)) return hipErrorInvalidValue;
+    if (rm == 1 ? (extra.pack_in || (extra.pack_out && !rp.wide))
+                : (extra.pack_in != extra.pack_out || (extra.pack_in && next_shift < 0)))
+      return hipErrorInvalidValue;
     if (next_shift >= 0) {
       e = hipMemsetAsync(next_hist, 0, sizeof(uint32_t) * kSub * kBuckets, s);
       if (e != hipSuccess) return e;
@@ -1920,10 +1992,20 @@
     if (rm == 1) {
       e = hipMemsetAsync(rp.counts, 0, sizeof(uint32_t) * kRegions, s);
       if (e == hipSuccess) e = hipMemsetAsync(rp.ovf, 0, sizeof(uint32_t), s);
+      if (e == hipSuccess && extra.pack_out) e = hipMemsetAsync(rp.wide, 0, sizeof(uint32_t), s);
       if (e != hipSuccess) return e;
-      hipLaunchKernelGGL((k_onesweep<kOsBlock, kOsIpt, true, false, 1, false, false, 1>), gd, bd, 0, s, in, out,
-                         m, shift, next_shift, sub_hist, next_hist, st, tile_ctr, epoch, err, nullptr, nullptr,
-                         SegPass(), gsrc, rp);
+      if (extra.pack_out)
+        hipLaunchKernelGGL((k_onesweep<kOsBlock, kOsIpt, true, false, 1, false, false, 1, false, true>), gd, bd, 0, s,
+                           in, out, m, shift, next_shift, sub_hist, next_hist, st, tile_ctr, epoch, err, nullptr,
+                           nullptr, SegPass(), gsrc, rp);
+      else
+        hipLaunchKernelGGL((k_onesweep<kOsBlock, kOsIpt, true, false, 1, false, false, 1>), gd, bd, 0, s, in, out,
+                           m, shift, next_shift, sub_hist, next_hist, st, tile_ctr, epoch, err, nullptr, nullptr,
+                           SegPass(), gsrc, rp);
+    } else if (next_shift >= 0 && extra.pack_in) {
+      hipLaunchKernelGGL((k_onesweep<kOsBlock, kOsIpt, true, false, 1, false, false, 2, true, true>), gd, bd, 0, s,
+                         in, out, m, shift, next_shift, sub_hist, next_hist, st, tile_ctr, epoch, err, nullptr,
+                         nullptr, SegPass(), gsrc, rp);
     } else if (next_shift >= 0) {
       hipLaunchKernelGGL((k_onesweep<kOsBlock, kOsIpt, true, false, 1, false, false, 2>), gd, bd, 0, s, in, out,
                          m, shift, next_shift, sub_hist, next_hist, st, tile_ctr, epoch, err, nullptr, nullptr,
@@ -1933,6 +2015,23 @@
                          m, shift, 0, sub_hist, nullptr, st, tile_ctr, epoch, err, nullptr, nullptr, SegPass(),
                          gsrc, rp);
     }
+  } else if (extra.pack_in) {
+    if (c16 || extra.halves != 1 || extra.seg || gat || extra.probe || extra.totals ||
+        extra.pack_out != (next_shift >= 0))
+      return hipErrorInvalidValue;
+    if (next_shift >= 0) {
+      e = hipMemsetAsync(next_hist, 0, sizeof(uint32_t) * kSub * kBuckets, s);
+      if (e != hipSuccess) return e;
+      hipLaunchKernelGGL((k_onesweep<kOsBlock, kOsIpt, true, false, 1, false, false, 0, true, true>), gd, bd, 0, s,
+                         in, out, m, shift, next_shift, sub_hist, next_hist, st, tile_ctr, epoch, err, nullptr,
+                         nullptr, SegPass(), gsrc, RegionPass());
+    } else {
+      hipLaunchKernelGGL((k_onesweep<kOsBlock, kOsIpt, false, false, 1, false, false, 0, true, false>), gd, bd, 0, s,
+                         in, out, m, shift, 0, sub_hist, nullptr, st, tile_ctr, epoch, err, nullptr, nullptr,
+                         SegPass(), gsrc, RegionPass());
+    }
+  } else if (extra.pack_out) {
+    return hipErrorInvalidValue;
   } else if (extra.probe) {
     if (next_shift < 0 || !next_hist || c16 || extra.halves != 1 || extra.seg || gat) return hipErrorInvalidValue;
     e = hipMemsetAsync(next_hist, 0, sizeof(uint32_t) * kSub * kBuckets, s);
@@ -2086,6 +2185,12 @@
   return hipGetLastError();
 }
 
+hipError_t launch_unpack(Elem* dst, const Packed* src, int64_t cnt, hipStream_t s) {
+  if (cnt <= 0) return hipSuccess;
+  hipLaunchKernelGGL(k_unpack, dim3(grid_for(cnt, 256, 8192)), dim3(256), 0, s, dst, src, cnt);
+  return hipGetLastError();
+}
+
 hipError_t launch_verify(const Elem* A, int64_t here, int64_t gbase, int64_t n, int64_t per,
                          KeyGen gen, unsigned long long* first_bad, hipStream_t s) {
   if (here <= 0) return hipSuccess;
diff --git a/distributed-lsb_amd/csrc/lsb_passes.cpp b/distributed-lsb_amd/csrc/lsb_passes.cpp
--- a/distributed-lsb_amd/csrc/lsb_passes.cpp
+++ b/distributed-lsb_amd/csrc/lsb_passes.cpp
@@ -57,8 +57,8 @@
          c->ranks[0].here <= lsb::kOnesweepMaxElems;
 }
 
-constexpr int kRgCounts = 0, kRgHist = lsb::kRegions, kRgOvf = kRgHist + lsb::kBuckets,
-              kRgSpan = kRgOvf + 2, kRgWords = kRgSpan + 4;
+constexpr int kRgCounts = 0, kRgHist = lsb::kRegions, kRgOvf = kRgHist + lsb::kBuckets, kRgWide = kRgOvf + 1,
+              kRgSpan = kRgOvf + 2, kRgSampleWide = kRgSpan + 4, kRgWords = kRgSampleWide + 1;
 
 int onesweep_ensure(Rank& r) {
   if (r.os_status) return LSB_OK;
@@ -161,7 +161,7 @@
 }
 
 int onesweep_digits(lsb_ctx* c, Rank& r, const std::vector<int>& digits, int* passes, size_t from = 0,
-                    const lsb::RegionPass* rp = nullptr, bool* disarm = nullptr) {
+                    const lsb::RegionPass* rp = nullptr, bool* disarm = nullptr, bool packed = false) {
   uint32_t* hist[2] = {r.os_hist, r.os_hist + lsb::kOnesweepSubs * lsb::kBuckets};
   for (size_t i = from; i < digits.size(); ++i) {
     const int shift = digits[i] * lsb::kDigitBits;
@@ -173,7 +173,22 @@
       x.region = rp;
       x.region_mode = 2;
     }
-    LSB_TRY(onesweep_launch(c, r, shift, next, hist[i & 1], hist[(i + 1) & 1], x));
+    x.pack_in = packed;
+    x.pack_out = packed && next >= 0;
+    const int rc = onesweep_launch(c, r, shift, next, hist[i & 1], hist[(i + 1) & 1], x);
+    if (rc != LSB_OK) {
+      if (packed && i > from) {
+        const hipError_t e =
+            lsb::launch_unpack(r.B, reinterpret_cast<const lsb::Packed*>(r.A), r.here, r.stream);
+        if (e == hipSuccess) {
+          std::swap(r.A, r.B);
+        } else {
+          (void)hipGetLastError();
+          c->broken = true;
+        }
+      }
+      return rc;
+    }
     ++*passes;
     if (disarm) *disarm = false;
   }
@@ -192,6 +207,7 @@
   rp.cap = r.rg_cap;
   rp.counts = r.rg_buf + kRgCounts;
   rp.ovf = r.rg_buf + kRgOvf;
+  rp.wide = r.rg_buf + kRgWide;
   return rp;
 }
 
@@ -201,7 +217,7 @@
   {
     Timer t(c, &r, LSB_K_UPSWEEP);
     HIP_TRY(lsb::launch_sample(r.A, r.here, byte * lsb::kDigitBits, r.rg_buf + kRgHist,
-                               reinterpret_cast<uint64_t*>(r.rg_buf + kRgSpan), r.stream));
+                               reinterpret_cast<uint64_t*>(r.rg_buf + kRgSpan), r.rg_buf + kRgSampleWide, r.stream));
   }
   HIP_TRY(hipMemcpyAsync(r.rg_h + kRgHist, r.rg_buf + kRgHist, (size_t)(kRgWords - kRgHist) * sizeof(uint32_t),
                          hipMemcpyDeviceToHost, r.stream));
@@ -224,15 +240,18 @@
   return LSB_OK;
 }
 
-int region_first(lsb_ctx* c, Rank& r, int shift, int next_shift, int* passes) {
+int region_first(lsb_ctx* c, Rank& r, int shift, int next_shift, int* passes, bool pack = false) {
   const lsb::RegionPass rp = region_pass(r);
   begin_pass(c, shift);
   lsb::OnesweepExtra x;
   x.region = &rp;
   x.region_mode = 1;
+  x.pack_out = pack;
   LSB_TRY(onesweep_launch(c, r, shift, next_shift, nullptr, r.os_hist + lsb::kOnesweepSubs * lsb::kBuckets, x));
   ++*passes;
-  HIP_TRY(hipMemcpyAsync(r.rg_h + kRgOvf, r.rg_buf + kRgOvf, sizeof(uint32_t), hipMemcpyDeviceToHost, r.stream));
+  r.rg_h[kRgWide] = 0;
+  HIP_TRY(hipMemcpyAsync(r.rg_h + kRgOvf, r.rg_buf + kRgOvf, (pack ? 2 : 1) * sizeof(uint32_t),
+                         hipMemcpyDeviceToHost, r.stream));
   return LSB_OK;
 }
 
@@ -264,6 +283,7 @@
   std::vector<int> digits, msd;
   bool fuse = false;
   bool region = false;
+  bool pack = false;
   Elem *X0 = nullptr, *X1 = nullptr, *X2 = nullptr;
   bool armed = false;
   uint64_t pmask = 0;
@@ -298,6 +318,7 @@
   int hybrid_passes(size_t from);
   int classic();
   int first_hist(int byte, bool* skewed, bool* constant);
+  int restart_counted();
   int queue_err_word() {
     HIP_TRY(hipMemcpyAsync(r.os_err_h, r.os_ctr + lsb::kOnesweepSubs, sizeof(uint32_t),
                            hipMemcpyDeviceToHost, r.stream));
@@ -371,7 +392,9 @@
       X1 = r.B;
       X2 = r.R;
       armed = true;
-      return region_first(c, r, 0, lsb::kDigitBits, &passes);
+      pack = c->pack_values == 2 ||
+             (c->pack_values == 1 && !c->pack_wide && r.rg_h[kRgSampleWide] == 0);
+      return region_first(c, r, 0, lsb::kDigitBits, &passes, pack);
     }
     varying = ~0ull;
     LSB_TRY(count_byte(c, r, 0, c->skip_constant));
@@ -415,30 +438,18 @@
     region = false;
     HIP_TRY(hipStreamSynchronize(r.stream));
     digits = varying_bytes(~0ull);
-    if (r.rg_h[kRgOvf] == 0) {
+    const bool wide = pack && r.rg_h[kRgWide] != 0;
+    if (wide) c->pack_wide = true;
+    if (r.rg_h[kRgOvf] == 0 && !wide) {
       r.os_halves = 1;
       const lsb::RegionPass rp = region_pass(r);
-      LSB_TRY(onesweep_digits(c, r, digits, &passes, 1, &rp, &armed));
+      if (pack) c->last_records = LSB_RECORDS_PACKED;
+      LSB_TRY(onesweep_digits(c, r, digits, &passes, 1, &rp, &armed, pack));
       kind = kDone;
       return queue_err_word();
     }
-    c->last_first = LSB_FIRST_REGIONAL_REDONE;
-    std::swap(r.A, r.B);
-    armed = false;
-    passes = 0;
-    c->pass_cursor = 0;
-    c->cur_pass = 0;
-    HIP_TRY(hipMemsetAsync(r.span, 0, 2 * sizeof(uint64_t), r.stream));
-    LSB_TRY(count_byte(c, r, 0, c->skip_constant));
-    LSB_TRY(queue_halves(c, r, r.os_hist));
-    HIP_TRY(hipMemcpyAsync(r.span_h, r.span, 2 * sizeof(uint64_t), hipMemcpyDeviceToHost, r.stream));
-    HIP_TRY(hipStreamSynchronize(r.stream));
-    varying = c->skip_constant ? r.span_h[0] & r.span_h[1] : ~0ull;
-    digits = varying_bytes(varying);
-    LSB_TRY(choose_halves(c, r, true));
-    LSB_TRY(onesweep_digits(c, r, digits, &passes));
-    kind = kDone;
-    return queue_err_word();
+    if (wide) c->last_records = LSB_RECORDS_PACKED_REDONE;
+    return restart_counted();
   }
   if (kind == kHybrid && region) {
     region = false;
@@ -497,6 +508,26 @@
   return hybrid_passes(0);
 }
 
+int LocalSort::restart_counted() {
+  c->last_first = LSB_FIRST_REGIONAL_REDONE;
+  std::swap(r.A, r.B);
+  armed = false;
+  passes = 0;
+  c->pass_cursor = 0;
+  c->cur_pass = 0;
+  HIP_TRY(hipMemsetAsync(r.span, 0, 2 * sizeof(uint64_t), r.stream));
+  LSB_TRY(count_byte(c, r, 0, c->skip_constant));
+  LSB_TRY(queue_halves(c, r, r.os_hist));
+  HIP_TRY(hipMemcpyAsync(r.span_h, r.span, 2 * sizeof(uint64_t), hipMemcpyDeviceToHost, r.stream));
+  HIP_TRY(hipStreamSynchronize(r.stream));
+  varying = c->skip_constant ? r.span_h[0] & r.span_h[1] : ~0ull;
+  digits = varying_bytes(varying);
+  LSB_TRY(choose_halves(c, r, true));
+  LSB_TRY(onesweep_digits(c, r, digits, &passes));
+  kind = kDone;
+  return queue_err_word();
+}
+
 int LocalSort::hybrid_passes(size_t from) {
   const int64_t m = r.here;
   if (from == 0) {
diff --git a/distributed-lsb_amd/csrc/lsb_rt.h b/distributed-lsb_amd/csrc/lsb_rt.h
--- a/distributed-lsb_amd/csrc/lsb_rt.h
+++ b/distributed-lsb_amd/csrc/lsb_rt.h
@@ -138,12 +138,16 @@
   bool gather = true;
   int os_split = 0;
   int fail_onesweep = 0;
+  int pack_values = 1;
+  bool pack_wide = false;
+  bool broken = false;
   int hybrid = 0;
   int64_t coll_calls = 0, coll_bytes = 0, coll_max = 0;
   int last_local_passes = 0;
   int last_exchanges = 0;
   uint64_t last_varying = 0;
   int last_first = 0;
+  int last_records = 0;
   lsb::KeyGen keygen;
   std::vector<lsb_rt::PendingEvent> pending;
   std::vector<std::pair<int, hipEvent_t>> event_pool;
diff --git a/distributed-lsb_amd/lsbsort/__init__.py b/distributed-lsb_amd/lsbsort/__init__.py
--- a/distributed-lsb_amd/lsbsort/__init__.py
+++ b/distributed-lsb_amd/lsbsort/__init__.py
@@ -32,6 +32,8 @@
 OPT_FAIL_ONESWEEP = 11
 OPT_REGION_FIRST = 12
 OPT_EXCHANGE_CHUNKS = 13
+OPT_PACK_VALUES = 14
+RECORDS_FULL, RECORDS_PACKED, RECORDS_PACKED_REDONE = 0, 1, 2
 FIRST_COUNT, FIRST_REGIONAL, FIRST_REGIONAL_REDONE = 0, 1, 2
 MAX_PASSES = 16
 
@@ -133,6 +135,7 @@
             "lsb_set_option": (i32, [vp, i32, i64]),
             "lsb_get_last_sort": (i32, [vp, vp, vp, vp]),
             "lsb_get_first_pass": (i32, [vp, vp]),
+            "lsb_get_last_records": (i32, [vp, vp]),
             "lsb_local_ranks": (i32, [vp, ctypes.POINTER(ctypes.c_int), ctypes.POINTER(ctypes.c_int)]),
             "lsb_generate": (i32, [vp]),
             "lsb_generate_ex": (i32, [vp, i32, ctypes.c_double]),
@@ -423,6 +426,11 @@
         _check(_lib().lsb_get_first_pass(self._h, ctypes.byref(f)), "lsb_get_first_pass")
         return int(f.value)
 
+    def last_records(self) -> int:
+        f = ctypes.c_int()
+        _check(_lib().lsb_get_last_records(self._h, ctypes.byref(f)), "lsb_get_last_records")
+        return int(f.value)
+
     def kernel_stats(self) -> dict:
         out = {}
         for kid, name in enumerate(KERNEL_NAMES):
diff --git a/include/lsb.h b/include/lsb.h
--- a/include/lsb.h
+++ b/include/lsb.h
@@ -53,6 +53,8 @@
 #define LSB_OPT_REGION_FIRST    12
 #define LSB_OPT_EXCHANGE_CHUNKS 13
 
+#define LSB_OPT_PACK_VALUES     14
+
 int64_t lsb_per_rank(int64_t n_total, int num_ranks);
 int64_t lsb_here(int64_t n_total, int num_ranks, int rank);
 
@@ -92,6 +94,10 @@
 #define LSB_FIRST_REGIONAL        1
 #define LSB_FIRST_REGIONAL_REDONE 2
 int  lsb_get_first_pass(lsb_ctx_t* ctx, int* form);
+#define LSB_RECORDS_FULL          0
+#define LSB_RECORDS_PACKED        1
+#define LSB_RECORDS_PACKED_REDONE 2
+int  lsb_get_last_records(lsb_ctx_t* ctx, int* form);
 int  lsb_pass(lsb_ctx_t* ctx, int digit);
 int  lsb_sync(lsb_ctx_t* ctx);
 int  lsb_barrier(lsb_ctx_t* ctx);
```

After: 22150, median of 6. 1.11x the previous value.
